# TrevorS/qwen3-tts-rs

Hardware: AMD Instinct MI355X
Metric: acoustic_frames_per_sec (higher is better)
Workload: dtype bf16

## Files before the change

include/q3tts.h:

```cpp
#ifndef Q3TTS_H
#define Q3TTS_H

#include <stddef.h>
#include <stdint.h>

#ifdef __cplusplus
extern "C" {
#endif

#define Q3_ABI_VERSION 1
#define Q3_MAX_BATCH 64

typedef enum q3_status {
    Q3_OK = 0,
    Q3_INVALID_ARG = 1,
    Q3_IO = 2,
    Q3_MISSING_WEIGHT = 3,
    Q3_KV_OVERFLOW = 4,
    Q3_HIP_ERROR = 5,
    Q3_RCCL_ERROR = 6,
    Q3_UNSUPPORTED = 7,
    Q3_OOM = 8
} q3_status;

// ... 209 lines not shown
int         q3_conv_path(int cout, int cin, int L, int k, int dil, int phases, int packed, int has_resid, int planes, int aligned16);
int         q3_resunit_path(int C, int L, int dil, int packed, int ya_is_xa, int planes);
const char* q3_conv_path_name(int code);
typedef struct q3_conv_ex_args {
    int kind, cin, cout, L, k, dil, stride;
    int act, planes, packed, resid_in_place, snake_raw, y2_is_x;
    int y_front, y_elems;
    int* path;
    const float* x; const float* w; const float* b;
    const float* snake_a; const float* snake_b; const float* resid; const float* scale;
    const float* post_a; const float* post_ib;
    const float* w2; const float* b2; const float* mid_a; const float* mid_ib;
    float* y; float* y2;
} q3_conv_ex_args;
q3_status q3_conv_ex(int device, const q3_conv_ex_args* args);
q3_status q3_test_conv_resident(int device, const q3_conv_ex_args* args, int resident, int* lds_bytes);
int q3_gemm_path(int M, int N, int K, int epi, int norm, int w2, int planes, int* path);
typedef struct q3_gemm_ex_args {
    int M, N, K, ldx, ldy, ldr, M_alloc;
    int epi, geometry, k_split, sup_m, sup_n;
    float eps;
    int* path;
    const float* x; const uint16_t* w; const uint16_t* w2;
    const float* bias; const float* norm_w; const float* resid;
    float* y;
} q3_gemm_ex_args;
q3_status q3_gemm_ex(int device, const q3_gemm_ex_args* args);
int q3_attn_prefill_path(int nh, int nkv, int use_planes, int halves, int* path);
typedef struct q3_attn_prefill_ex_args {
    int n_seq, rps, base_pos, nh, nkv, max_seq, ld_qkv, ld_out;
    int kernel, halves, use_planes;
    float eps;
    int* path;
    const float* qkv; const float* q_norm_w; const float* k_norm_w;
    const float* rope_cos; const float* rope_sin;
    float* kcache; float* vcache; float* out;
    int layout, n_layers, layer, n_slabs;
    const int* page_slots; int* rot_used; long long* stray;
} q3_attn_prefill_ex_args;
q3_status q3_attn_prefill_ex(int device, const q3_attn_prefill_ex_args* args);
typedef struct q3_attn_prefill_packed_ex_args {
    int n_seq, nh, nkv, max_seq, ld_qkv, ld_out;
    int kernel;
    float eps;
    const int* seq_len;
    int* path; long long* plane_tail;
    const float* qkv; const float* q_norm_w; const float* k_norm_w;
    const float* rope_cos; const float* rope_sin;
    float* kcache; float* vcache; float* out;
    int layout, n_layers, layer, n_slabs;
    const int* page_slots; int* rot_used; long long* stray;
} q3_attn_prefill_packed_ex_args;
q3_status q3_attn_prefill_packed_ex(int device, const q3_attn_prefill_packed_ex_args* args);
q3_status q3_prefill_pack_plan(const int32_t* lengths, const int32_t* hit_pages, int32_t n, int32_t row_budget, int32_t gemm_ok,
                               int32_t* pass, int32_t* row0, int32_t* n_passes);
q3_status q3_session_prefill_info(const q3_session* s, int32_t info[8]);
typedef struct q3_prompt_rows_ex_args {
    int mode, n, cols, n_table, n_rows, n_ref, cp_vocab, lds, ldd, reserved;
    const uint16_t* table; const uint32_t* ids; const float* src;
    const int* text_row; const int* codec_id; const float* xvec;
    const uint32_t* ref_codes; const uint16_t* cp_embs;
    const int* dst_row; const int* ent;
    float* out; int* trail_len; int* text_ready; int* limit;
} q3_prompt_rows_ex_args;
q3_status q3_prompt_rows_ex(int device, const q3_prompt_rows_ex_args* args);
int q3_attn_c_path(int hd, int kernel);
typedef struct q3_attn_c_ex_args {
    int mode, nh, hd, L, kernel, window;
    int N, n_rows, layers, layer, cap, n_blocks, n_tabs;
    float scale;
    const float* q; const float* k; const float* v;
    const int* rows; const float* caches;
    const int* tabs; const int* tab0; const int* tab_n;
    float* o;
} q3_attn_c_ex_args;
q3_status q3_attn_c_ex(int device, const q3_attn_c_ex_args* args);
q3_status q3_rope_c_ex(int device, float* q, float* k, const float* cs, const float* sn, const int* pos, int nh, int hd, int L, int n_pos);
q3_status q3_copy_cols_ex(int device, const float* src, size_t src_elems, float* dst, size_t dst_elems, int n, int C, const long long* s_off,
                          const long long* d_off, const int* sp, const int* dp, size_t src_off, size_t dst_off);
q3_status q3_copy_segs_ex(int device, const float* src, size_t src_elems, float* dst, size_t dst_elems, int n_segs, const unsigned long long* segs);
q3_status q3_gather_frames_ex(int device, const uint32_t* src, size_t src_elems, const long long* s_off, int n, uint32_t* dst, size_t dst_elems);
q3_status q3_rvq_embed_ex(int device, const uint32_t* frames, int n_frames, const float* first_cb, const float* rest_cbs, int cb_dim, int cb_size,
                          float* first_out, float* rest_out, int out_front, int out_elems);
q3_status q3_silu_mul_ex(int device, const float* g, const float* u, float* y, long long n, long long y_elems);
typedef struct q3_spk_op_ex_args {
    int op, C, T, pl, Tp, ld, off, reserved;
    long long a_elems, b_elems, out_front, out_elems;
    const float* a; const float* b; float* out;
} q3_spk_op_ex_args;
q3_status q3_spk_op_ex(int device, const q3_spk_op_ex_args* args);
typedef struct q3_mimi_op_ex_args {
    int op, C, L, r, Lf, elu, replicate, reserved;
    long long a_elems, b_elems, out_front, out_elems;
    const float* a; const float* b; float* out;
} q3_mimi_op_ex_args;
q3_status q3_mimi_op_ex(int device, const q3_mimi_op_ex_args* args);
q3_status q3_mimi_rvq_ex(int device, const float* proj, int T, const float* books, int n_layers, int CB, int CD, uint32_t* codes, int n_q,
                         int q0);
typedef struct q3_sample_rec {
    float inv_temp; int apply_temp, greedy;
    int top_k; float top_p; int use_top_p;
    float rep_pen, rep_inv; int use_rep;
    int eos_id, min_new_tokens, pad;
} q3_sample_rec;
q3_status q3_sample_row(const q3_options* opts, q3_sample_rec* out);
typedef struct q3_prompt_shape_rec {
    int32_t icl, n_ins, n_ref_text, n_icl, overlay;
    int32_t prefill_len, n_rows;
    int32_t trailing_len, n_trail;
    int32_t limit, open_need, prefix_pages;
    int32_t r_role, r_pad, r_bos, r_text, r_eos, trail_base;
} q3_prompt_shape_rec;
q3_status q3_prompt_shape(const q3_request* req, int n_text, q3_prompt_shape_rec* out, int* text_row, int* codec_id, int cap_positions);
typedef struct q3_sample_ex_args {
    int B, vocab, ld, u_stride, u_elems, advance, token_count_static, hist_stride_b, hist_cap, codec_eos, use_suppress, guard;
    q3_sample_rec scalar;
    const float* logits; const float* u; const int* draw_idx; const q3_sample_rec* rows;
    const int* limit; const int* text_ready;
    uint32_t* tok; uint8_t* seen; int* token_count; int* frame_idx; int* pos; float* logits_hist;
} q3_sample_ex_args;
q3_status q3_sample_ex(int device, const q3_sample_ex_args* args);
typedef struct q3_frame_embed_ex_args {
    int B, H, n_sem, cp_vocab, max_frames, n_text_rows, guard, reserved;
    const uint16_t* codec_emb; const uint16_t* cp_embs; const uint32_t* tok; const float* cp_logits_last;
    const int* frame_idx; const float* text_rows; const int* trail_base; const int* trail_len; const int* pad_row; const int* text_ready;
    uint32_t* codes; float* out;
} q3_frame_embed_ex_args;
q3_status q3_frame_embed_ex(int device, const q3_frame_embed_ex_args* args);
typedef struct q3_cp_gather_ex_args {
    int pass, B, H, n_sem, cp_vocab, max_frames, proj_dim, qkv_dim, ld_out, ld_qkv_out, guard, reserved;
    const float* last_hidden; const uint16_t* codec_emb; const uint32_t* tok; const uint16_t* cp_emb; const float* cp_logits;
    const float* proj_tab; const float* qkv_tab; const int* frame_idx;
    uint32_t* codes; float* out; float* qkv_out;
} q3_cp_gather_ex_args;
q3_status q3_cp_gather_ex(int device, const q3_cp_gather_ex_args* args);
q3_status q3_rmsnorm_ex(int device, const float* x, long long x_elems, long long x_off, int ldx, const float* w, float* y, long long y_elems,
                        long long y_front, int ldy, int rows, int cols, float eps, const int* frame_idx, const int* text_ready);
q3_status q3_norm_c(int device, int layernorm, const float* x, const float* w, const float* b, int C, int L, float eps,
                    float* y, int y_front, int y_elems);
q3_status q3_dwconv7(int device, const float* x, const float* w, const float* b, int C, int L, float* y, int y_front, int y_elems);
q3_status q3_row_move(int device, void* src_host, size_t src_bytes, void* dst_host, size_t dst_bytes, int n_segs, const size_t* src_off,
                      const size_t* dst_off, const size_t* seg_bytes, const int* mode);
enum { Q3_DEC_QUANT = 0, Q3_DEC_PRECONV = 1, Q3_DEC_PRETRANS = 2, Q3_DEC_UP0 = 3, Q3_DEC_UP1 = 4,
       Q3_DEC_INIT = 5, Q3_DEC_BLK0 = 6, Q3_DEC_BLK1 = 7, Q3_DEC_BLK2 = 8, Q3_DEC_BLK3 = 9, Q3_DEC_N = 10 };
q3_status q3_decode_codes(q3_model* m, const uint32_t* frames_host, int n_frames, float* pcm_host,
                          float** taps_host);
typedef struct q3_codec_stream q3_codec_stream;
q3_status q3_codec_stream_create(q3_model* m, int rows, int max_frames, q3_codec_stream** out);
void      q3_codec_stream_free(q3_codec_stream* cs);
q3_status q3_codec_stream_reset(q3_codec_stream* cs, int row);
q3_status q3_codec_stream_pos(q3_codec_stream* cs, int row, int* n_frames);
q3_status q3_codec_stream_push(q3_codec_stream* cs, int n_rows, const int* rows, const uint32_t* const* frames_host,
                               const int* n_frames, float* const* pcm_host, const size_t* cap);
q3_status q3_codec_stream_create_blocked(q3_model* m, int rows, int max_frames, int block_frames, int max_blocks, q3_codec_stream** out);
q3_status q3_codec_stream_info(q3_codec_stream* cs, int* block_frames, size_t* block_bytes, int* blocks_total, int* blocks_in_use,
                               int* blocks_peak);
q3_status q3_codec_stream_prime(q3_codec_stream* cs, int row, const uint32_t* frames_host, int n_frames);
enum { Q3_PCM_F32 = 0, Q3_PCM_S16 = 1, Q3_PCM_ULAW = 2, Q3_PCM_ALAW = 3 };
typedef struct q3_pcm_stage q3_pcm_stage;
q3_status q3_pcm_stage_create(int device, int rows, size_t max_push_samples, q3_pcm_stage** out);
void      q3_pcm_stage_free(q3_pcm_stage* ps);
q3_status q3_pcm_stage_set(q3_pcm_stage* ps, int row, uint32_t sample_rate, int format);
q3_status q3_pcm_stage_reset(q3_pcm_stage* ps, int row);
q3_status q3_pcm_stage_push(q3_pcm_stage* ps, int n_rows, const int* rows, const float* const* in_host, const size_t* n_in,
                            const int* last, void* const* out_host, const size_t* cap_samples, size_t* n_samples);
q3_status q3_pcm_stage_bound(uint32_t sample_rate, size_t n_in, size_t* n_out_max);
q3_status q3_pcm_stage_taps(uint32_t sample_rate, float* taps_host, size_t cap_floats, int* L, int* M);
q3_status q3_codec_stream_push_out(q3_codec_stream* cs, int n_rows, const int* rows, const uint32_t* const* frames_host, const int* n_frames,
                                   q3_pcm_stage* ps, const int* ps_rows, const int* last,
                                   void* const* out_host, const size_t* cap_samples, size_t* n_samples);
q3_status q3_session_set_output(q3_session* s, uint32_t sample_rate, int format);
q3_status q3_session_next_chunks_out(q3_session* s, void* const* out_host, const size_t* cap_samples, size_t* n_samples, int* done);
q3_status q3_batcher_ticket_output(q3_batcher* b, int64_t ticket, uint32_t sample_rate, int format);
q3_status q3_batcher_read_out(q3_batcher* b, int64_t ticket, void* out_host, size_t cap_samples, size_t* n_samples, int* done);
q3_status q3_pcm_stage_set_tempo(q3_pcm_stage* ps, int row, int tempo_permille);
q3_status q3_pcm_stage_tempo_count(int tempo_permille, size_t n_in_total, int ended, size_t* frames, size_t* samples_24k);
q3_status q3_pcm_stage_bound_tempo(uint32_t sample_rate, int tempo_permille, size_t n_in, size_t* n_out_max);
q3_status q3_pcm_stage_tempo_lags(q3_pcm_stage* ps, int row, int64_t* k0, int* lags, size_t cap, size_t* n);
q3_status q3_session_set_tempo(q3_session* s, int b, int tempo_permille);
q3_status q3_batcher_ticket_tempo(q3_batcher* b, int64_t ticket, int tempo_permille);
q3_status q3_pcm_stage_set_level(q3_pcm_stage* ps, int row, int gain_mB, int ceiling_mB);
q3_status q3_pcm_stage_level_coeffs(int gain_mB, int ceiling_mB, float* g, float* c);
q3_status q3_pcm_stage_level_count(size_t n_in_total, int ended, size_t* n_out);
q3_status q3_pcm_stage_bound_level(uint32_t sample_rate, int tempo_permille, size_t n_in, size_t* n_out_max);
q3_status q3_session_set_level(q3_session* s, int b, int gain_mB, int ceiling_mB);
q3_status q3_batcher_ticket_level(q3_batcher* b, int64_t ticket, int gain_mB, int ceiling_mB);
enum { Q3_LOUD_OFF = 0, Q3_LOUD_METER = 1, Q3_LOUD_NORMALIZE = 2 };
q3_status q3_loudness_kweight(uint32_t sample_rate, double* shelf_ba, double* highpass_ba);
q3_status q3_pcm_stage_loudness_consts(int target_mB, int prior_mB, float* T, float* P, float* gate_abs, float* a_lo, float* a_hi);
q3_status q3_pcm_stage_set_loudness(q3_pcm_stage* ps, int row, int mode, int target_mB, int prior_mB);
q3_status q3_pcm_stage_loudness(q3_pcm_stage* ps, int row, float* mean_square, float* gain, int* blocks, int* gated);
q3_status q3_pcm_stage_loudness_blocks(q3_pcm_stage* ps, int row, float* z, size_t cap, size_t* n);
q3_status q3_session_set_loudness(q3_session* s, int b, int mode, int target_mB, int prior_mB);
q3_status q3_session_loudness(q3_session* s, int b, float* mean_square, float* gain, int* blocks, int* gated);
q3_status q3_batcher_ticket_loudness(q3_batcher* b, int64_t ticket, int mode, int target_mB, int prior_mB);
q3_status q3_batcher_ticket_loudness_read(q3_batcher* b, int64_t ticket, float* mean_square, float* gain, int* blocks, int* gated);
q3_status q3_pcm_stage_set_pitch(q3_pcm_stage* ps, int row, int cents);
q3_status q3_pcm_stage_pitch_plan(int tempo_permille, int cents, int* tempo_eff, double* cents_realized);
q3_status q3_pcm_stage_pitch_tables(float* sinc, size_t cap1, float* win, size_t cap2, int* S1, int* S2);
q3_status q3_pcm_stage_pitch_count(int tempo_permille, int cents, size_t n_in_total, int ended, size_t* samples_24k);
q3_status q3_pcm_stage_bound_pitch(uint32_t sample_rate, int tempo_permille, int cents, int with_level, size_t n_in, size_t* n_out_max);
q3_status q3_session_set_pitch(q3_session* s, int b, int cents);
q3_status q3_batcher_ticket_pitch(q3_batcher* b, int64_t ticket, int cents);
q3_status q3_pcm_stage_set_silence(q3_pcm_stage* ps, int row, int threshold_mB, int edge_ms, int pause_ms);
q3_status q3_pcm_stage_silence(q3_pcm_stage* ps, int row, int64_t* n_in, int64_t* n_out, int64_t* lead_cut, int64_t* pause_cut, int64_t* trail_cut);
q3_status q3_pcm_stage_silence_hold(int edge_ms, int pause_ms, size_t* samples);
q3_status q3_pcm_stage_bound_silence(uint32_t sample_rate, int tempo_permille, int cents, int with_level, int edge_ms, int pause_ms, size_t n_in,
                                     size_t* n_out_max);
q3_status q3_silence_trim(const float* x, size_t n, int threshold_mB, int edge_ms, int pause_ms, float* y, size_t cap, size_t* n_y, int64_t* counts);
q3_status q3_session_set_silence(q3_session* s, int b, int threshold_mB, int edge_ms, int pause_ms);
q3_status q3_session_silence(q3_session* s, int b, int64_t* n_in, int64_t* n_out, int64_t* lead_cut, int64_t* pause_cut, int64_t* trail_cut);
q3_status q3_batcher_ticket_silence(q3_batcher* b, int64_t ticket, int threshold_mB, int edge_ms, int pause_ms);
q3_status q3_batcher_ticket_silence_read(q3_batcher* b, int64_t ticket, int64_t* n_in, int64_t* n_out, int64_t* lead_cut, int64_t* pause_cut, int64_t* trail_cut);
void      q3_codes_to_tensor(const uint32_t* frames, int n_frames, int64_t* out);

q3_status q3_session_set_profile(q3_session* s, int enable);
q3_status q3_session_profile_read(q3_session* s, double* ms, double* bytes, long* launches, int reset);
q3_status q3_session_profile_shapes(q3_session* s, int* rows, int cap_rows, int* n_rows, int reset);
q3_status q3_bench_linear(int device, int M, int N, int K, int epi, int rms, int tiled, int iters, int n_copies,
                          double* avg_us);
q3_status q3_session_stream(q3_session* s, void** stream);
q3_status q3_session_submit_info(q3_session* s, int* path, int* nodes);
q3_status q3_session_submit_fences(q3_session* s, int* acquire_free, int* release_free);
q3_status q3_session_frame_bytes(q3_session* s, int kv_len, double* weight_bytes, double* kv_bytes);

enum { Q3_MODEL_UNKNOWN = -1, Q3_MODEL_BASE = 0, Q3_MODEL_CUSTOM_VOICE = 1, Q3_MODEL_VOICE_DESIGN = 2 };
q3_status q3_config_default(int variant, q3_config* out);
q3_status q3_config_from_json(const char* path, q3_config* out, int* model_type);
q3_status q3_model_load(const char* model_dir, int device, q3_model** out, int* model_type);
q3_status q3_model_load_safetensors(q3_model* m, const char* path, int* n_loaded);
q3_status q3_safetensors_info(const char* path, const char* name, int* dtype, int64_t* shape, int cap_dims, int* n_dims);
q3_status q3_pcm16_from_f32(const float* samples_host, int64_t n, int16_t* out_host);
q3_status q3_wav_write_pcm16(const char* path, const float* samples_host, int64_t n, uint32_t sample_rate);
q3_status q3_g711_from_pcm16(const int16_t* in_host, int64_t n, int law, uint8_t* out_host);
q3_status q3_wav_write_g711(const char* path, const uint8_t* bytes_host, int64_t n, uint32_t sample_rate, int law);
q3_status q3_wav_read(const char* path, float* out_host, int64_t cap, int64_t* n_samples, uint32_t* sample_rate);
q3_status q3_codes_write_bin(const char* path, const uint32_t* codes_host, int n_frames, int n_groups);
q3_status q3_codes_read_bin(const char* path, uint32_t* codes_host, int cap_frames, int n_groups, int* n_frames);
q3_status q3_audio_write_bin(const char* path, const float* samples_host, int64_t n);
q3_status q3_audio_read_bin(const char* path, float* out_host, int64_t cap, int64_t* n_samples);
q3_status q3_resample(const float* in_host, int64_t n, uint32_t sr_in, uint32_t sr_out, float* out_host, int64_t cap, int64_t* n_out);

typedef struct q3_spk_config {
    int32_t mel_dim;
    int32_t enc_dim;
    int32_t channels[5];
    int32_t kernel_sizes[5];
    int32_t dilations[5];
    int32_t attention_channels;
    int32_t res2net_scale;
    int32_t se_channels;
    int32_t sample_rate;
} q3_spk_config;
typedef struct q3_speaker_encoder q3_speaker_encoder;
q3_status q3_spk_config_default(q3_spk_config* out);
q3_status q3_spk_config_from_json(const char* path, q3_spk_config* out, int* present);
q3_status q3_spk_create(const q3_spk_config* cfg, int device, q3_speaker_encoder** out);
void q3_spk_free(q3_speaker_encoder* e);
q3_status q3_spk_get_config(const q3_speaker_encoder* e, q3_spk_config* out);
int q3_spk_n_tensors(const q3_speaker_encoder* e);
q3_status q3_spk_tensor_info(const q3_speaker_encoder* e, int i, const char** name, int64_t* n);
q3_status q3_spk_set_tensor(q3_speaker_encoder* e, const char* name, const void* data_host, int src_dtype, int64_t n);
q3_status q3_spk_finalize(q3_speaker_encoder* e);
q3_status q3_spk_load_safetensors(q3_speaker_encoder* e, const char* path);
int q3_spk_mel_frames(int64_t n_samples);
q3_status q3_spk_mel(q3_speaker_encoder* e, const float* samples_host, int64_t n, float* mel_host, int64_t cap_floats, int* n_frames);
q3_status q3_spk_tables(q3_speaker_encoder* e, float* win_host, float* fb_host);
q3_status q3_spk_forward(q3_speaker_encoder* e, const float* mel_host, int T, float* out_host, float** taps_host);
q3_status q3_spk_encode(q3_speaker_encoder* e, const float* samples_host, int64_t n, uint32_t sample_rate, float* out_host);

typedef struct q3_mimi_config {
    int32_t n_filters;
    int32_t hidden;
    int32_t ratios[4];
    int32_t kernel;
    int32_t res_kernel;
    int32_t last_kernel;
    int32_t compress;
    int32_t n_layers;
    int32_t n_heads;
    int32_t head_dim;
    int32_t inter;
    int32_t window;
    int32_t cb_size;
    int32_t cb_dim;
    int32_t n_q;
    int32_t n_sem;
    float norm_eps;
    float rope_theta;
} q3_mimi_config;
typedef struct q3_speech_encoder q3_speech_encoder;
q3_status q3_mimi_config_default(q3_mimi_config* out);
q3_status q3_mimi_create(const q3_mimi_config* cfg, int device, q3_speech_encoder** out);
void q3_mimi_free(q3_speech_encoder* e);
q3_status q3_mimi_get_config(const q3_speech_encoder* e, q3_mimi_config* out);
int q3_mimi_n_tensors(const q3_speech_encoder* e);
q3_status q3_mimi_tensor_info(const q3_speech_encoder* e, int i, const char** name, int64_t* n);
q3_status q3_mimi_set_tensor(q3_speech_encoder* e, const char* name, const void* data_host, int src_dtype, int64_t n);
q3_status q3_mimi_finalize(q3_speech_encoder* e);
q3_status q3_mimi_load_safetensors(q3_speech_encoder* e, const char* path);
int q3_mimi_frames(const q3_mimi_config* cfg, int64_t n_samples);
q3_status q3_mimi_encode(q3_speech_encoder* e, const float* samples_host, int64_t n, uint32_t sample_rate, uint32_t* codes_host,
                         int cap_frames, int* n_frames, float** taps_host);

enum { Q3_SRC_U8 = 0, Q3_SRC_S16 = 1, Q3_SRC_S24 = 2, Q3_SRC_S32 = 3, Q3_SRC_F32 = 4, Q3_SRC_ULAW = 5, Q3_SRC_ALAW = 6 };
typedef struct q3_clip { const void* data; int64_t frames; int32_t channels; uint32_t sample_rate; int32_t format; } q3_clip;
// ... 37 lines not shown
```

qwen3_tts_rs_amd/_lib.py:

```python
import ctypes
import os

from .config import CConfig

_HERE = os.path.dirname(os.path.abspath(__file__))
LIB_PATH = os.environ.get("Q3TTS_LIB") or os.path.join(_HERE, "libq3tts.so")

if not os.path.exists(LIB_PATH):
    raise ImportError(
        f"{LIB_PATH} not found: the gfx950 HIP library is not built. Run "
        "`python -c 'import __graft_entry__ as g; g.build()'` (or qwen3_tts_rs_amd/csrc/build.sh).")

lib = ctypes.CDLL(LIB_PATH)


class COptions(ctypes.Structure):
    _fields_ = [
        ("temperature", ctypes.c_double), ("top_p", ctypes.c_double), ("repetition_penalty", ctypes.c_double),
        ("seed", ctypes.c_uint64), ("max_length", ctypes.c_int32), ("top_k", ctypes.c_int32),
        ("eos_token_id", ctypes.c_int32), ("chunk_frames", ctypes.c_int32), ("min_new_tokens", ctypes.c_int32),
        ("has_seed", ctypes.c_int32),
    ]


# ... 43 lines not shown
               [("eps", ctypes.c_float), ("qkv_eps", ctypes.c_float), ("reserved", ctypes.c_int32)] + \
               [(n, ctypes.c_void_p) for n in ("pos", "qkv", "q_norm_w", "k_norm_w", "rope_cos", "rope_sin", "kcache", "vcache", "out", "page_slots",
                                               "rot_used", "stray", "qkv_part", "qkv_ssq", "g_logits", "g_tok", "g_qkv_tab", "g_proj_tab", "g_x",
                                               "g_codes", "g_frame_idx", "zero_buf")]


class CConvEx(ctypes.Structure):
    _fields_ = [(n, ctypes.c_int32) for n in ("kind", "cin", "cout", "L", "k", "dil", "stride", "act", "planes", "packed", "resid_in_place",
                                              "snake_raw", "y2_is_x", "y_front", "y_elems")] + [("path", ctypes.POINTER(ctypes.c_int32))] + \
               [(n, ctypes.c_void_p) for n in ("x", "w", "b", "snake_a", "snake_b", "resid", "scale", "post_a", "post_ib", "w2", "b2", "mid_a",
                                               "mid_ib", "y", "y2")]


class CGemmEx(ctypes.Structure):
    _fields_ = [(n, ctypes.c_int32) for n in ("M", "N", "K", "ldx", "ldy", "ldr", "M_alloc", "epi", "geometry", "k_split", "sup_m",
                                              "sup_n")] + [("eps", ctypes.c_float), ("path", ctypes.POINTER(ctypes.c_int32))] + \
               [(n, ctypes.c_void_p) for n in ("x", "w", "w2", "bias", "norm_w", "resid", "y")]


class CAttnPrefillEx(ctypes.Structure):
    _fields_ = [(n, ctypes.c_int32) for n in ("n_seq", "rps", "base_pos", "nh", "nkv", "max_seq", "ld_qkv", "ld_out", "kernel", "halves",
                                              "use_planes")] + [("eps", ctypes.c_float), ("path", ctypes.POINTER(ctypes.c_int32))] + \
               [(n, ctypes.c_void_p) for n in ("qkv", "q_norm_w", "k_norm_w", "rope_cos", "rope_sin", "kcache", "vcache", "out")] + \
               [(n, ctypes.c_int32) for n in ("layout", "n_layers", "layer", "n_slabs")] + \
               [(n, ctypes.c_void_p) for n in ("page_slots", "rot_used", "stray")]


class CAttnPrefillPackedEx(ctypes.Structure):
    _fields_ = [(n, ctypes.c_int32) for n in ("n_seq", "nh", "nkv", "max_seq", "ld_qkv", "ld_out", "kernel")] + [("eps", ctypes.c_float)] + \
               [(n, ctypes.c_void_p) for n in ("seq_len", "path", "plane_tail", "qkv", "q_norm_w", "k_norm_w", "rope_cos", "rope_sin", "kcache", "vcache",
                                               "out")] + \
               [(n, ctypes.c_int32) for n in ("layout", "n_layers", "layer", "n_slabs")] + \
               [(n, ctypes.c_void_p) for n in ("page_slots", "rot_used", "stray")]


class CPromptRowsEx(ctypes.Structure):
    _fields_ = [(n, ctypes.c_int32) for n in ("mode", "n", "cols", "n_table", "n_rows", "n_ref", "cp_vocab", "lds", "ldd", "reserved")] + \
               [(n, ctypes.c_void_p) for n in ("table", "ids", "src", "text_row", "codec_id", "xvec", "ref_codes", "cp_embs", "dst_row", "ent", "out",
                                               "trail_len", "text_ready", "limit")]


class CAttnCEx(ctypes.Structure):
    _fields_ = [(n, ctypes.c_int32) for n in ("mode", "nh", "hd", "L", "kernel", "window", "N", "n_rows", "layers", "layer", "cap", "n_blocks",
                                              "n_tabs")] + [("scale", ctypes.c_float)] + \
               [(n, ctypes.c_void_p) for n in ("q", "k", "v", "rows", "caches", "tabs", "tab0", "tab_n", "o")]


class CSpkOpEx(ctypes.Structure):
    _fields_ = [(n, ctypes.c_int32) for n in ("op", "C", "T", "pl", "Tp", "ld", "off", "reserved")] + \
               [(n, ctypes.c_longlong) for n in ("a_elems", "b_elems", "out_front", "out_elems")] + \
               [(n, ctypes.c_void_p) for n in ("a", "b", "out")]


class CMimiOpEx(ctypes.Structure):
    _fields_ = [(n, ctypes.c_int32) for n in ("op", "C", "L", "r", "Lf", "elu", "replicate", "reserved")] + \
               [(n, ctypes.c_longlong) for n in ("a_elems", "b_elems", "out_front", "out_elems")] + \
               [(n, ctypes.c_void_p) for n in ("a", "b", "out")]


class CSampleRow(ctypes.Structure):
    _fields_ = [("inv_temp", ctypes.c_float), ("apply_temp", ctypes.c_int32), ("greedy", ctypes.c_int32), ("top_k", ctypes.c_int32),
                ("top_p", ctypes.c_float), ("use_top_p", ctypes.c_int32), ("rep_pen", ctypes.c_float), ("rep_inv", ctypes.c_float),
                ("use_rep", ctypes.c_int32), ("eos_id", ctypes.c_int32), ("min_new_tokens", ctypes.c_int32), ("pad", ctypes.c_int32)]


class CPromptShape(ctypes.Structure):
    _fields_ = [(n, ctypes.c_int32) for n in ("icl", "n_ins", "n_ref_text", "n_icl", "overlay", "prefill_len", "n_rows", "trailing_len", "n_trail",
                                              "limit", "open_need", "prefix_pages", "r_role", "r_pad", "r_bos", "r_text", "r_eos", "trail_base")]


class CSampleEx(ctypes.Structure):
    _fields_ = [(n, ctypes.c_int32) for n in ("B", "vocab", "ld", "u_stride", "u_elems", "advance", "token_count_static", "hist_stride_b",
                                              "hist_cap", "codec_eos", "use_suppress", "guard")] + [("scalar", CSampleRow)] + \
               [(n, ctypes.c_void_p) for n in ("logits", "u", "draw_idx", "rows", "limit", "text_ready", "tok", "seen", "token_count",
                                               "frame_idx", "pos", "logits_hist")]


class CFrameEmbedEx(ctypes.Structure):
    _fields_ = [(n, ctypes.c_int32) for n in ("B", "H", "n_sem", "cp_vocab", "max_frames", "n_text_rows", "guard", "reserved")] + \
               [(n, ctypes.c_void_p) for n in ("codec_emb", "cp_embs", "tok", "cp_logits_last", "frame_idx", "text_rows", "trail_base",
                                               "trail_len", "pad_row", "text_ready", "codes", "out")]


class CCpGatherEx(ctypes.Structure):
    _fields_ = [(n, ctypes.c_int32) for n in ("pass_", "B", "H", "n_sem", "cp_vocab", "max_frames", "proj_dim", "qkv_dim", "ld_out",
                                              "ld_qkv_out", "guard", "reserved")] + \
               [(n, ctypes.c_void_p) for n in ("last_hidden", "codec_emb", "tok", "cp_emb", "cp_logits", "proj_tab", "qkv_tab", "frame_idx",
                                               "codes", "out", "qkv_out")]


class CClip(ctypes.Structure):
    _fields_ = [("data", ctypes.c_void_p), ("frames", ctypes.c_int64), ("channels", ctypes.c_int32), ("sample_rate", ctypes.c_uint32),
                ("format", ctypes.c_int32)]


class CMimiPackClip(ctypes.Structure):
    _fields_ = [("frames", ctypes.c_int32), ("pass_", ctypes.c_int32), ("start", ctypes.c_int64)]


class CWavDesc(ctypes.Structure):
    _fields_ = [("format", ctypes.c_int32), ("channels", ctypes.c_int32), ("bits", ctypes.c_int32), ("sample_rate", ctypes.c_uint32),
                ("frames", ctypes.c_int64), ("data_offset", ctypes.c_int64), ("data_bytes", ctypes.c_int64)]


class CTiming(ctypes.Structure):
    _fields_ = [("prefill_ms", ctypes.c_double), ("generation_ms", ctypes.c_double), ("decode_ms", ctypes.c_double),
                ("generation_frames", ctypes.c_int32)]


c_void_p, c_int, c_char_p = ctypes.c_void_p, ctypes.c_int, ctypes.c_char_p
P = ctypes.POINTER

SYMBOLS = {
    "q3_abi_version": (c_int, []),
    "q3_last_error": (c_char_p, []),
    "q3_device_count": (c_int, []),
    "q3_model_create": (c_int, [P(CConfig), c_int, P(c_void_p)]),
    "q3_model_free": (None, [c_void_p]),
    "q3_model_set_tensor": (c_int, [c_void_p, c_char_p, c_int, c_void_p, ctypes.c_int64]),
    "q3_model_n_tensors": (c_int, [c_void_p]),
    "q3_model_tensor_info": (c_int, [c_void_p, c_int, P(c_char_p), P(ctypes.c_int64), P(c_int)]),
    "q3_model_arena": (c_int, [c_void_p, P(c_void_p), P(ctypes.c_size_t)]),
    "q3_model_kv_pool_limit": (c_int, [c_void_p, c_int]),
    "q3_model_set_codec_planes": (c_int, [c_void_p, c_int]),
    "q3_model_kv_pool_trim": (c_int, [c_void_p, P(ctypes.c_size_t)]),
    "q3_model_kv_pool_info": (c_int, [c_void_p, P(c_int), P(ctypes.c_size_t), P(c_int), P(c_int), P(c_int)]),
    "q3_model_prefix_cache": (c_int, [c_void_p, c_int]),
    "q3_model_prefix_cache_info": (c_int, [c_void_p, P(c_int), P(c_int), P(c_int), P(ctypes.c_longlong), P(ctypes.c_longlong), P(ctypes.c_longlong)]),
    "q3_session_prefix_info": (c_int, [c_void_p, c_int, P(c_int)]),
    "q3_model_mark_loaded": (c_int, [c_void_p]),
    "q3_model_finalize": (c_int, [c_void_p]),
    "q3_synth_fill": (c_int, [ctypes.c_uint64, c_char_p, c_int, ctypes.c_float, ctypes.c_float, ctypes.c_int64, c_void_p]),
    "q3_session_create": (c_int, [c_void_p, P(CRequest), c_int, P(c_void_p)]),
    "q3_session_create_reserved": (c_int, [c_void_p, P(CRequest), c_int, c_int, c_int, P(c_void_p)]),
    "q3_session_free": (None, [c_void_p]),
    "q3_session_prefill": (c_int, [c_void_p]),
    "q3_session_generate": (c_int, [c_void_p, c_int, c_int]),
    "q3_session_frames": (c_int, [c_void_p, c_int, P(c_int), P(c_int)]),
    "q3_session_codes": (c_int, [c_void_p, c_int, c_void_p, c_int, P(c_int)]),
    "q3_session_decode": (c_int, [c_void_p, c_int, c_int, c_int, c_void_p, ctypes.c_size_t, P(ctypes.c_size_t)]),
    "q3_session_set_kv_dtype": (c_int, [c_void_p, c_int]),
    "q3_session_run": (c_int, [c_void_p, c_int, P(c_void_p), P(ctypes.c_size_t), P(ctypes.c_size_t), P(CTiming)]),
    "q3_session_next_chunk": (c_int, [c_void_p, c_void_p, ctypes.c_size_t, P(ctypes.c_size_t), P(c_int)]),
    "q3_session_next_chunk_row": (c_int, [c_void_p, c_int, c_void_p, ctypes.c_size_t, P(ctypes.c_size_t), P(c_int)]),
    "q3_session_next_chunks": (c_int, [c_void_p, P(c_void_p), P(ctypes.c_size_t), P(ctypes.c_size_t), P(c_int)]),
    "q3_codec_stream_create": (c_int, [c_void_p, c_int, c_int, P(c_void_p)]),
    "q3_codec_stream_create_blocked": (c_int, [c_void_p, c_int, c_int, c_int, c_int, P(c_void_p)]),
    "q3_codec_stream_info": (c_int, [c_void_p, P(c_int), P(ctypes.c_size_t), P(c_int), P(c_int), P(c_int)]),
    "q3_codec_stream_prime": (c_int, [c_void_p, c_int, c_void_p, c_int]),
    "q3_codec_stream_free": (None, [c_void_p]),
    "q3_codec_stream_reset": (c_int, [c_void_p, c_int]),
    "q3_codec_stream_pos": (c_int, [c_void_p, c_int, P(c_int)]),
    "q3_codec_stream_push": (c_int, [c_void_p, c_int, P(c_int), P(c_void_p), P(c_int), P(c_void_p), P(ctypes.c_size_t)]),
    "q3_pcm_stage_create": (c_int, [c_int, c_int, ctypes.c_size_t, P(c_void_p)]),
    "q3_pcm_stage_free": (None, [c_void_p]),
    "q3_pcm_stage_set": (c_int, [c_void_p, c_int, ctypes.c_uint32, c_int]),
    "q3_pcm_stage_reset": (c_int, [c_void_p, c_int]),
    "q3_pcm_stage_push": (c_int, [c_void_p, c_int, P(c_int), P(c_void_p), P(ctypes.c_size_t), P(c_int), P(c_void_p), P(ctypes.c_size_t),
                                  P(ctypes.c_size_t)]),
    "q3_pcm_stage_bound": (c_int, [ctypes.c_uint32, ctypes.c_size_t, P(ctypes.c_size_t)]),
    "q3_pcm_stage_taps": (c_int, [ctypes.c_uint32, c_void_p, ctypes.c_size_t, P(c_int), P(c_int)]),
    "q3_pcm_stage_set_tempo": (c_int, [c_void_p, c_int, c_int]),
    "q3_pcm_stage_tempo_count": (c_int, [c_int, ctypes.c_size_t, c_int, P(ctypes.c_size_t), P(ctypes.c_size_t)]),
    "q3_pcm_stage_bound_tempo": (c_int, [ctypes.c_uint32, c_int, ctypes.c_size_t, P(ctypes.c_size_t)]),
    "q3_pcm_stage_tempo_lags": (c_int, [c_void_p, c_int, P(ctypes.c_int64), c_void_p, ctypes.c_size_t, P(ctypes.c_size_t)]),
    "q3_session_set_tempo": (c_int, [c_void_p, c_int, c_int]),
    "q3_batcher_ticket_tempo": (c_int, [c_void_p, ctypes.c_int64, c_int]),
    "q3_pcm_stage_set_pitch": (c_int, [c_void_p, c_int, c_int]),
    "q3_pcm_stage_pitch_plan": (c_int, [c_int, c_int, P(c_int), P(ctypes.c_double)]),
    "q3_pcm_stage_pitch_tables": (c_int, [c_void_p, ctypes.c_size_t, c_void_p, ctypes.c_size_t, P(c_int), P(c_int)]),
    "q3_pcm_stage_pitch_count": (c_int, [c_int, c_int, ctypes.c_size_t, c_int, P(ctypes.c_size_t)]),
    "q3_pcm_stage_bound_pitch": (c_int, [ctypes.c_uint32, c_int, c_int, c_int, ctypes.c_size_t, P(ctypes.c_size_t)]),
    "q3_session_set_pitch": (c_int, [c_void_p, c_int, c_int]),
    "q3_batcher_ticket_pitch": (c_int, [c_void_p, ctypes.c_int64, c_int]),
    "q3_pcm_stage_set_silence": (c_int, [c_void_p, c_int, c_int, c_int, c_int]),
    "q3_pcm_stage_silence": (c_int, [c_void_p, c_int] + [P(ctypes.c_int64)] * 5),
    "q3_pcm_stage_silence_hold": (c_int, [c_int, c_int, P(ctypes.c_size_t)]),
    "q3_pcm_stage_bound_silence": (c_int, [ctypes.c_uint32, c_int, c_int, c_int, c_int, c_int, ctypes.c_size_t, P(ctypes.c_size_t)]),
    "q3_silence_trim": (c_int, [c_void_p, ctypes.c_size_t, c_int, c_int, c_int, c_void_p, ctypes.c_size_t, P(ctypes.c_size_t), P(ctypes.c_int64)]),
    "q3_session_set_silence": (c_int, [c_void_p, c_int, c_int, c_int, c_int]),
    "q3_session_silence": (c_int, [c_void_p, c_int] + [P(ctypes.c_int64)] * 5),
    "q3_batcher_ticket_silence": (c_int, [c_void_p, ctypes.c_int64, c_int, c_int, c_int]),
    "q3_batcher_ticket_silence_read": (c_int, [c_void_p, ctypes.c_int64] + [P(ctypes.c_int64)] * 5),
    "q3_pcm_stage_set_level": (c_int, [c_void_p, c_int, c_int, c_int]),
    "q3_pcm_stage_level_coeffs": (c_int, [c_int, c_int, P(ctypes.c_float), P(ctypes.c_float)]),
    "q3_pcm_stage_level_count": (c_int, [ctypes.c_size_t, c_int, P(ctypes.c_size_t)]),
    "q3_pcm_stage_bound_level": (c_int, [ctypes.c_uint32, c_int, ctypes.c_size_t, P(ctypes.c_size_t)]),
    "q3_session_set_level": (c_int, [c_void_p, c_int, c_int, c_int]),
    "q3_batcher_ticket_level": (c_int, [c_void_p, ctypes.c_int64, c_int, c_int]),
    "q3_loudness_kweight": (c_int, [ctypes.c_uint32, P(ctypes.c_double), P(ctypes.c_double)]),
    "q3_pcm_stage_loudness_consts": (c_int, [c_int, c_int, P(ctypes.c_float), P(ctypes.c_float), P(ctypes.c_float), P(ctypes.c_float), P(ctypes.c_float)]),
    "q3_pcm_stage_set_loudness": (c_int, [c_void_p, c_int, c_int, c_int, c_int]),
    "q3_pcm_stage_loudness": (c_int, [c_void_p, c_int, P(ctypes.c_float), P(ctypes.c_float), P(c_int), P(c_int)]),
    "q3_pcm_stage_loudness_blocks": (c_int, [c_void_p, c_int, c_void_p, ctypes.c_size_t, P(ctypes.c_size_t)]),
    "q3_session_set_loudness": (c_int, [c_void_p, c_int, c_int, c_int, c_int]),
    "q3_session_loudness": (c_int, [c_void_p, c_int, P(ctypes.c_float), P(ctypes.c_float), P(c_int), P(c_int)]),
    "q3_batcher_ticket_loudness": (c_int, [c_void_p, ctypes.c_int64, c_int, c_int, c_int]),
    "q3_batcher_ticket_loudness_read": (c_int, [c_void_p, ctypes.c_int64, P(ctypes.c_float), P(ctypes.c_float), P(c_int), P(c_int)]),
    "q3_codec_stream_push_out": (c_int, [c_void_p, c_int, P(c_int), P(c_void_p), P(c_int), c_void_p, P(c_int), P(c_int), P(c_void_p),
                                         P(ctypes.c_size_t), P(ctypes.c_size_t)]),
    "q3_session_set_output": (c_int, [c_void_p, ctypes.c_uint32, c_int]),
    "q3_session_next_chunks_out": (c_int, [c_void_p, P(c_void_p), P(ctypes.c_size_t), P(ctypes.c_size_t), P(c_int)]),
    "q3_batcher_ticket_output": (c_int, [c_void_p, ctypes.c_int64, ctypes.c_uint32, c_int]),
    "q3_batcher_read_out": (c_int, [c_void_p, ctypes.c_int64, c_void_p, ctypes.c_size_t, P(ctypes.c_size_t), P(c_int)]),
    "q3_session_replace": (c_int, [c_void_p, c_int, c_void_p]),
    "q3_session_park_row": (c_int, [c_void_p, c_int, P(c_void_p)]),
    "q3_session_resume_row": (c_int, [c_void_p, c_int, c_void_p]),
    "q3_parked_free": (None, [c_void_p]),
    "q3_parked_info": (c_int, [c_void_p, P(c_int), P(c_int), P(c_int), P(c_int), P(ctypes.c_size_t)]),
    "q3_row_move": (c_int, [c_int, c_void_p, ctypes.c_size_t, c_void_p, ctypes.c_size_t, c_int, P(ctypes.c_size_t), P(ctypes.c_size_t),
                            P(ctypes.c_size_t), P(c_int)]),
    "q3_batcher_create": (c_int, [c_void_p, c_int, c_int, c_int, P(c_void_p)]),
    "q3_batcher_free": (None, [c_void_p]),
    "q3_batcher_submit": (c_int, [c_void_p, c_void_p, c_int, P(ctypes.c_int64)]),
    "q3_batcher_submit_streamed": (c_int, [c_void_p, c_void_p, P(ctypes.c_int64)]),
    "q3_batcher_read": (c_int, [c_void_p, ctypes.c_int64, c_void_p, ctypes.c_size_t, P(ctypes.c_size_t), P(c_int)]),
    "q3_batcher_stream_info": (c_int, [c_void_p, P(c_int), P(ctypes.c_size_t), P(c_int), P(c_int), P(c_int)]),
    "q3_batcher_submit_open": (c_int, [c_void_p, c_void_p, c_int, P(ctypes.c_int64)]),
    "q3_batcher_append_text": (c_int, [c_void_p, ctypes.c_int64, c_void_p, c_int, c_int]),
    "q3_batcher_text_state": (c_int, [c_void_p, ctypes.c_int64, P(c_int), P(c_int), P(c_int), P(c_int)]),
    "q3_batcher_cancel": (c_int, [c_void_p, ctypes.c_int64]),
    "q3_batcher_set_parking": (c_int, [c_void_p, c_int, c_int, c_int]),
    "q3_batcher_park": (c_int, [c_void_p, ctypes.c_int64]),
    "q3_batcher_unpark": (c_int, [c_void_p, ctypes.c_int64]),
    "q3_batcher_park_info": (c_int, [c_void_p, P(c_int), P(c_int), P(ctypes.c_longlong), P(ctypes.c_longlong), P(ctypes.c_longlong), P(c_int)]),
    "q3_batcher_step": (c_int, [c_void_p, c_int, c_int, P(c_int), P(c_int), P(c_int)]),
    "q3_batcher_poll": (c_int, [c_void_p, ctypes.c_int64, P(c_int), P(c_int), P(ctypes.c_size_t)]),
    "q3_batcher_fetch": (c_int, [c_void_p, ctypes.c_int64, c_void_p, c_int, c_void_p, ctypes.c_size_t]),
    "q3_session_set_debug": (c_int, [c_void_p, c_int]),
    "q3_session_prefill_len": (c_int, [c_void_p, c_int, P(c_int), P(c_int)]),
    "q3_session_get": (c_int, [c_void_p, c_int, c_int, c_void_p, ctypes.c_size_t]),
    "q3_talker_step": (c_int, [c_void_p, c_void_p, c_void_p, c_void_p]),
    "q3_cp_generate": (c_int, [c_void_p, c_void_p, c_void_p, c_void_p, c_void_p]),
    "q3_frame_embed": (c_int, [c_void_p, ctypes.c_uint32, c_void_p, c_void_p, c_void_p]),
    "q3_sample": (c_int, [c_int, c_void_p, c_void_p, c_void_p, c_int, c_int, P(COptions), c_int, c_void_p]),
    "q3_rng_seed": (None, [ctypes.c_uint64, P(ctypes.c_uint64)]),
    "q3_rng_next": (ctypes.c_float, [P(ctypes.c_uint64)]),
    "q3_fused_residual_rmsnorm": (c_int, [c_int, c_int, c_void_p, c_void_p, c_void_p, c_int, c_int, ctypes.c_float, c_void_p, c_void_p]),
    "q3_linear": (c_int, [c_int, c_void_p, c_void_p, c_void_p, c_int, c_int, c_int, c_void_p]),
    "q3_linear_ex": (c_int, [c_int, P(CLinearEx)]),
    "q3_attn_step": (c_int, [c_int, P(CAttnStep)]),
    "q3_attn_step_ex": (c_int, [c_int, P(CAttnStepEx)]),
    "q3_kv_pages_to_bf16_ex": (c_int, [c_int] * 4 + [c_void_p] * 6),
    "q3_conv_path": (c_int, [c_int] * 10),
    "q3_resunit_path": (c_int, [c_int] * 6),
    "q3_conv_path_name": (c_char_p, [c_int]),
    "q3_conv_ex": (c_int, [c_int, P(CConvEx)]),
    "q3_test_conv_resident": (c_int, [c_int, P(CConvEx), c_int, P(ctypes.c_int32)]),
    "q3_gemm_path": (c_int, [c_int] * 7 + [P(ctypes.c_int32)]),
    "q3_gemm_ex": (c_int, [c_int, P(CGemmEx)]),
    "q3_attn_prefill_path": (c_int, [c_int] * 4 + [P(ctypes.c_int32)]),
    "q3_attn_prefill_ex": (c_int, [c_int, P(CAttnPrefillEx)]),
    "q3_attn_prefill_packed_ex": (c_int, [c_int, P(CAttnPrefillPackedEx)]),
    "q3_prefill_pack_plan": (c_int, [P(ctypes.c_int32), P(ctypes.c_int32), ctypes.c_int32, ctypes.c_int32, ctypes.c_int32, P(ctypes.c_int32),
                                     P(ctypes.c_int32), P(ctypes.c_int32)]),
    "q3_session_prefill_info": (c_int, [c_void_p, P(ctypes.c_int32)]),
    "q3_prompt_rows_ex": (c_int, [c_int, P(CPromptRowsEx)]),
    "q3_attn_c_path": (c_int, [c_int, c_int]),
    "q3_attn_c_ex": (c_int, [c_int, P(CAttnCEx)]),
    "q3_rope_c_ex": (c_int, [c_int, c_void_p, c_void_p, c_void_p, c_void_p, c_void_p, c_int, c_int, c_int, c_int]),
    "q3_copy_cols_ex": (c_int, [c_int, c_void_p, ctypes.c_size_t, c_void_p, ctypes.c_size_t, c_int, c_int, c_void_p, c_void_p, c_void_p, c_void_p,
                                ctypes.c_size_t, ctypes.c_size_t]),
    "q3_copy_segs_ex": (c_int, [c_int, c_void_p, ctypes.c_size_t, c_void_p, ctypes.c_size_t, c_int, c_void_p]),
    "q3_gather_frames_ex": (c_int, [c_int, c_void_p, ctypes.c_size_t, c_void_p, c_int, c_void_p, ctypes.c_size_t]),
    "q3_rvq_embed_ex": (c_int, [c_int, c_void_p, c_int, c_void_p, c_void_p, c_int, c_int, c_void_p, c_void_p, c_int, c_int]),
    "q3_silu_mul_ex": (c_int, [c_int, c_void_p, c_void_p, c_void_p, ctypes.c_longlong, ctypes.c_longlong]),
    "q3_spk_op_ex": (c_int, [c_int, P(CSpkOpEx)]),
    "q3_mimi_op_ex": (c_int, [c_int, P(CMimiOpEx)]),
    "q3_mimi_rvq_ex": (c_int, [c_int, c_void_p, c_int, c_void_p, c_int, c_int, c_int, c_void_p, c_int, c_int]),
    "q3_spk_tables": (c_int, [c_void_p, c_void_p, c_void_p]),
    "q3_sample_row": (c_int, [P(COptions), P(CSampleRow)]),
    "q3_prompt_shape": (c_int, [P(CRequest), c_int, P(CPromptShape), c_void_p, c_void_p, c_int]),
    "q3_sample_ex": (c_int, [c_int, P(CSampleEx)]),
    "q3_frame_embed_ex": (c_int, [c_int, P(CFrameEmbedEx)]),
    "q3_cp_gather_ex": (c_int, [c_int, P(CCpGatherEx)]),
    "q3_rmsnorm_ex": (c_int, [c_int, c_void_p, ctypes.c_longlong, ctypes.c_longlong, c_int, c_void_p, c_void_p, ctypes.c_longlong,
                              ctypes.c_longlong, c_int, c_int, c_int, ctypes.c_float, c_void_p, c_void_p]),
    "q3_norm_c": (c_int, [c_int, c_int, c_void_p, c_void_p, c_void_p, c_int, c_int, ctypes.c_float, c_void_p, c_int, c_int]),
    "q3_dwconv7": (c_int, [c_int, c_void_p, c_void_p, c_void_p, c_int, c_int, c_void_p, c_int, c_int]),
    "q3_decode_codes": (c_int, [c_void_p, c_void_p, c_int, c_void_p, P(c_void_p)]),
    "q3_codes_to_tensor": (None, [c_void_p, c_int, c_void_p]),
    "q3_session_set_profile": (c_int, [c_void_p, c_int]),
    "q3_session_profile_read": (c_int, [c_void_p, P(ctypes.c_double), P(ctypes.c_double), P(ctypes.c_long), c_int]),
    "q3_session_profile_shapes": (c_int, [c_void_p, P(c_int), c_int, P(c_int), c_int]),
    "q3_bench_linear": (c_int, [c_int] * 9 + [P(ctypes.c_double)]),
    "q3_session_stream": (c_int, [c_void_p, P(c_void_p)]),
    "q3_session_frame_bytes": (c_int, [c_void_p, c_int, P(ctypes.c_double), P(ctypes.c_double)]),
    "q3_session_submit_info": (c_int, [c_void_p, P(c_int), P(c_int)]),
    "q3_session_submit_fences": (c_int, [c_void_p, P(c_int), P(c_int)]),
    "q3_session_set_stream_mode": (c_int, [c_void_p, c_int]),
    "q3_session_open_text": (c_int, [c_void_p, c_int]),
    "q3_session_append_text": (c_int, [c_void_p, c_int, c_void_p, c_int, c_int]),
    "q3_session_text_state": (c_int, [c_void_p, c_int, P(c_int), P(c_int), P(c_int), P(c_int), P(c_int)]),
    "q3_model_config": (c_int, [c_void_p, P(CConfig)]),
    "q3_config_default": (c_int, [c_int, P(CConfig)]),
    "q3_config_from_json": (c_int, [c_char_p, P(CConfig), P(c_int)]),
    "q3_model_load": (c_int, [c_char_p, c_int, P(c_void_p), P(c_int)]),
    "q3_model_load_safetensors": (c_int, [c_void_p, c_char_p, P(c_int)]),
    "q3_safetensors_info": (c_int, [c_char_p, c_char_p, P(c_int), P(ctypes.c_int64), c_int, P(c_int)]),
    "q3_pcm16_from_f32": (c_int, [c_void_p, ctypes.c_int64, c_void_p]),
    "q3_wav_write_pcm16": (c_int, [c_char_p, c_void_p, ctypes.c_int64, ctypes.c_uint32]),
    "q3_g711_from_pcm16": (c_int, [c_void_p, ctypes.c_int64, c_int, c_void_p]),
    "q3_wav_write_g711": (c_int, [c_char_p, c_void_p, ctypes.c_int64, ctypes.c_uint32, c_int]),
    "q3_wav_read": (c_int, [c_char_p, c_void_p, ctypes.c_int64, P(ctypes.c_int64), P(ctypes.c_uint32)]),
    "q3_codes_write_bin": (c_int, [c_char_p, c_void_p, c_int, c_int]),
    "q3_codes_read_bin": (c_int, [c_char_p, c_void_p, c_int, c_int, P(c_int)]),
# ... 67 lines not shown
```

qwen3_tts_rs_amd/api.py:

```python
import ctypes
import enum
from dataclasses import dataclass
from typing import List, NamedTuple, Optional, Sequence, Tuple

import numpy as np

from . import _lib
from ._lib import lib, check, COptions, CRequest, CTiming
from .config import Q3Config
from . import synth

MAX_BATCH = 64
CODEC_EOS_TOKEN_ID = 2150
SAMPLES_PER_FRAME = 1920


class Language(enum.Enum):
    Chinese = 2055
    English = 2050
    Japanese = 2058
    Korean = 2064
    German = 2053
    French = 2061
    Russian = 2069
# ... 992 lines not shown
        s = Session(self, utts[:n0], o, frame_budget=budget, prompt_budget=prompt)
        owner = list(range(n0)); nxt = n0
        codes: List[Optional[np.ndarray]] = [None] * len(utts); pcm: List[Optional[np.ndarray]] = [None] * len(utts)
        frames = 0
        t0 = _time.perf_counter()
        try:
            s.prefill()
            while any(i is not None for i in owner):
                s.generate(poll_frames, use_graph=use_graph)
                for b in range(n0):
                    i = owner[b]
                    if i is None:
                        continue
                    n, done = s.frames(b)
                    if not done:
                        continue
                    codes[i] = s.codes(b); frames += int(codes[i].shape[0])
                    if decode:
                        pcm[i] = s.decode(b)
                    if nxt < len(utts):
                        s.replace(b, utts[nxt]); owner[b] = nxt; nxt += 1
                    else:
                        owner[b] = None
            wall = _time.perf_counter() - t0
        finally:
            s.close()
        return codes, pcm, frames, wall

    def synthesize_continuous_streaming(self, utts: Sequence[Utterance], options=None, slots: int = 8, poll_frames: int = 10,
                                        on_audio=None, use_graph: bool = True):
        o = options or SynthesisOptions()
        utts = list(utts)
        budget = max((u.max_length if u.max_length is not None else (u.options or o).max_length) for u in utts)
        prompt = max((0 if u.instruct_ids is None else len(u.instruct_ids)) + (0 if u.ref_codes is None else int(np.asarray(u.ref_codes).reshape(-1, 16).shape[0])) + 16 for u in utts)
        bt = Batcher(self, slots=min(slots, max(len(utts), 1)), frame_budget=budget, prompt_budget=prompt, options=o)
        try:
            tickets = [bt.submit_streamed(u) for u in utts]
            open_ = set(range(len(utts)))

            def drain():
                for i in sorted(open_):
                    samples, done = bt.read(tickets[i])
                    if samples.size or done:
                        if on_audio is not None:
                            on_audio(i, samples, done)
                    if done:
                        open_.discard(i)
            while True:
                running, queued, _ = bt.step(poll_frames, use_graph)
                drain()
                if running == 0 and queued == 0:
                    break
            drain()
            return [bt.fetch(t)[0] for t in tickets]
        finally:
            bt.close()

    def synthesize_streaming(self, text_ids, speaker: Speaker, language: Language, options=None,
                             continuous: bool = False) -> StreamingSession:
        return StreamingSession(self, Utterance(text_ids, speaker, language), options or SynthesisOptions(), continuous)

    def synthesize_voice_design_streaming(self, text_ids, instruct_ids, language: Language, options=None,
                                          continuous: bool = False) -> StreamingSession:
        return StreamingSession(self, Utterance(text_ids, language=language, instruct_ids=instruct_ids), options or SynthesisOptions(), continuous)

    def synthesize_streaming_text(self, first_ids, speaker: Speaker, language: Language, options=None,
                                  continuous: bool = False) -> "TextStreamingSession":
        return TextStreamingSession(self, Utterance(list(first_ids), speaker, language), options or SynthesisOptions(), continuous)

    def synthesize_voice_clone_debug(self, text_ids, prompt, language: Language, options=None):
        return self.synthesize_voice_clone(text_ids, prompt.speaker_embedding, language, options,
                                           ref_codes=prompt.ref_codes, ref_text_ids=prompt.ref_text_ids)

    def device(self) -> str:
        return f"hip:{self.device_index}"

    @classmethod
    def from_pretrained_with_tokenizer(cls, model_dir: str, tokenizer_dir: Optional[str], device: int = 0):
        from .text import TextTokenizer
        return cls.from_pretrained(model_dir, device), TextTokenizer.from_pretrained(model_dir, tokenizer_dir)

    def decode_codes(self, codes: np.ndarray, taps=None) -> AudioBuffer:
        c = np.ascontiguousarray(codes, dtype=np.uint32).reshape(-1, 16)
        out = np.zeros(c.shape[0] * self.config.samples_per_frame, dtype=np.float32)
        tp = None
        if taps is not None:
            tp = (ctypes.c_void_p * 10)(*[t.ctypes.data_as(ctypes.c_void_p) if t is not None else None for t in taps])
        check(lib.q3_decode_codes(self._h, c.ctypes.data_as(ctypes.c_void_p), c.shape[0], out.ctypes.data_as(ctypes.c_void_p), tp))
        return AudioBuffer(out)

    def codec_stream(self, rows: int, max_frames: int, block_frames: int = 0, max_blocks: int = 0) -> "CodecStream":
        return CodecStream(self, rows, max_frames, block_frames, max_blocks)

    def pcm_stage(self, rows: int, max_push_samples: int) -> "PcmStage":
        return PcmStage(self, rows, max_push_samples)

    def frame_embed(self, sem_token: int, codes15, text_add: np.ndarray) -> np.ndarray:
        c = np.ascontiguousarray(codes15, dtype=np.uint32); t = np.ascontiguousarray(text_add, dtype=np.float32)
        out = np.zeros(self.config.hidden, dtype=np.float32)
        check(lib.q3_frame_embed(self._h, int(sem_token), c.ctypes.data_as(ctypes.c_void_p), t.ctypes.data_as(ctypes.c_void_p),
                                 out.ctypes.data_as(ctypes.c_void_p)))
        return out


class CodecStream:
    def __init__(self, model: "Qwen3TTS", rows: int, max_frames: int, block_frames: int = 0, max_blocks: int = 0):
        self.model = model; self.rows = int(rows); self.max_frames = int(max_frames)
        self._h = ctypes.c_void_p()
        if block_frames or max_blocks:
            check(lib.q3_codec_stream_create_blocked(model._h, self.rows, self.max_frames, int(block_frames), int(max_blocks),
                                                     ctypes.byref(self._h)))
        else:
            check(lib.q3_codec_stream_create(model._h, self.rows, self.max_frames, ctypes.byref(self._h)))

    def prime(self, row: int, codes: np.ndarray):
        c = np.ascontiguousarray(codes, dtype=np.uint32).reshape(-1, 16)
        check(lib.q3_codec_stream_prime(self._h, int(row), c.ctypes.data_as(ctypes.c_void_p), c.shape[0]))

    def info(self) -> dict:
        bf = ctypes.c_int(); bb = ctypes.c_size_t(); tot = ctypes.c_int(); use = ctypes.c_int(); peak = ctypes.c_int()
        check(lib.q3_codec_stream_info(self._h, ctypes.byref(bf), ctypes.byref(bb), ctypes.byref(tot), ctypes.byref(use), ctypes.byref(peak)))
        return {"block_frames": bf.value, "block_bytes": bb.value, "blocks_total": tot.value, "blocks_in_use": use.value,
                "blocks_peak": peak.value}

    def push(self, frames: dict, stage: Optional["PcmStage"] = None, stage_rows: Optional[dict] = None, last=()) -> dict:
        if stage is None:
            return self._push_lists(list(frames.keys()), list(frames.values()))
        rows = list(frames.keys()); n = len(rows); spf = self.model.config.samples_per_frame
        cs = [np.ascontiguousarray(frames[r], dtype=np.uint32).reshape(-1, 16) for r in rows]
        srows = [int((stage_rows or {}).get(r, r)) for r in rows]
        outs = [np.zeros(stage.bound(sr, c.shape[0] * spf), dtype=stage.dtype(sr)) for sr, c in zip(srows, cs)]
        r_ = (ctypes.c_int * n)(*[int(x) for x in rows])
        fp = (ctypes.c_void_p * n)(*[c.ctypes.data_as(ctypes.c_void_p) for c in cs])
        nf = (ctypes.c_int * n)(*[c.shape[0] for c in cs])
        sr_ = (ctypes.c_int * n)(*srows)
        ls = (ctypes.c_int * n)(*[1 if r in last else 0 for r in rows])
        op = (ctypes.c_void_p * n)(*[o.ctypes.data_as(ctypes.c_void_p) for o in outs])
        cp = (ctypes.c_size_t * n)(*[o.size for o in outs])
        ns = (ctypes.c_size_t * n)()
        check(lib.q3_codec_stream_push_out(self._h, n, r_, fp, nf, stage._h, sr_, ls, op, cp, ns))
        return {int(rows[i]): outs[i][:ns[i]].copy() for i in range(n)}

    def _push_lists(self, rows: Sequence[int], codes: Sequence[np.ndarray], cap: Optional[Sequence[int]] = None) -> dict:
        n = len(rows); spf = self.model.config.samples_per_frame
        cs = [np.ascontiguousarray(c, dtype=np.uint32).reshape(-1, 16) for c in codes]
        outs = [np.zeros(c.shape[0] * spf, dtype=np.float32) for c in cs]
        r = (ctypes.c_int * n)(*[int(x) for x in rows])
        fp = (ctypes.c_void_p * n)(*[c.ctypes.data_as(ctypes.c_void_p) for c in cs])
        nf = (ctypes.c_int * n)(*[c.shape[0] for c in cs])
        op = (ctypes.c_void_p * n)(*[o.ctypes.data_as(ctypes.c_void_p) for o in outs])
        cp = (ctypes.c_size_t * n)(*[int(x) for x in (cap if cap is not None else [o.size for o in outs])])
        check(lib.q3_codec_stream_push(self._h, n, r, fp, nf, op, cp))
        return {int(rows[i]): outs[i] for i in range(n)}

    def reset(self, row: int):
        check(lib.q3_codec_stream_reset(self._h, int(row)))

    def pos(self, row: int) -> int:
        n = ctypes.c_int()
        check(lib.q3_codec_stream_pos(self._h, int(row), ctypes.byref(n)))
        return n.value

    def close(self):
        if getattr(self, "_h", None):
            lib.q3_codec_stream_free(self._h); self._h = None

    __del__ = close


PCM_F32, PCM_S16, PCM_ULAW, PCM_ALAW = 0, 1, 2, 3
PCM_NAMES = ("f32", "s16", "ulaw", "alaw")
PCM_DTYPE = (np.float32, np.int16, np.uint8, np.uint8)


def pcm_format(pcm16: bool = False, fmt: Optional[str] = None) -> int:
    if fmt is None:
        return PCM_S16 if pcm16 else PCM_F32
    if pcm16:
        raise ValueError("give pcm16= or fmt=, not both")
    if fmt not in PCM_NAMES:
        raise ValueError(f"fmt must be one of {list(PCM_NAMES)}, not {fmt!r}")
    return PCM_NAMES.index(fmt)


def pcm_stage_taps(rate: int) -> Tuple[np.ndarray, int, int]:
    L = ctypes.c_int(); M = ctypes.c_int()
    check(lib.q3_pcm_stage_taps(int(rate), None, 0, ctypes.byref(L), ctypes.byref(M)))
    t = np.zeros((L.value, 128), np.float32)
    check(lib.q3_pcm_stage_taps(int(rate), t.ctypes.data_as(ctypes.c_void_p), t.size, ctypes.byref(L), ctypes.byref(M)))
    return t, L.value, M.value


def pcm_stage_bound(rate: int, n_in: int, tempo_permille: int = 1000, level: bool = False, pitch_cents: int = 0, silence=None) -> int:
    n = ctypes.c_size_t()
    if silence is not None:
        check(lib.q3_pcm_stage_bound_silence(int(rate), int(tempo_permille), int(pitch_cents), 1 if level else 0, int(silence[0]), int(silence[1]),
                                             int(n_in), ctypes.byref(n)))
    elif int(pitch_cents):
        check(lib.q3_pcm_stage_bound_pitch(int(rate), int(tempo_permille), int(pitch_cents), 1 if level else 0, int(n_in), ctypes.byref(n)))
    elif level:
        check(lib.q3_pcm_stage_bound_level(int(rate), int(tempo_permille), int(n_in), ctypes.byref(n)))
    elif int(tempo_permille) == 1000:
        check(lib.q3_pcm_stage_bound(int(rate), int(n_in), ctypes.byref(n)))
    else:
        check(lib.q3_pcm_stage_bound_tempo(int(rate), int(tempo_permille), int(n_in), ctypes.byref(n)))
    return int(n.value)


def pcm_stage_tempo_count(tempo_permille: int, n_in_total: int, ended: bool = False) -> Tuple[int, int]:
    f = ctypes.c_size_t(); y = ctypes.c_size_t()
    check(lib.q3_pcm_stage_tempo_count(int(tempo_permille), int(n_in_total), 1 if ended else 0, ctypes.byref(f), ctypes.byref(y)))
    return int(f.value), int(y.value)


def pcm_stage_pitch_plan(tempo_permille: int, cents: int) -> Tuple[int, float]:
    te = ctypes.c_int(); c = ctypes.c_double()
    check(lib.q3_pcm_stage_pitch_plan(int(tempo_permille), int(cents), ctypes.byref(te), ctypes.byref(c)))
    return int(te.value), float(c.value)


def pcm_stage_pitch_tables() -> Tuple[np.ndarray, np.ndarray, int, int]:
    s1 = ctypes.c_int(); s2 = ctypes.c_int()
    check(lib.q3_pcm_stage_pitch_tables(None, 0, None, 0, ctypes.byref(s1), ctypes.byref(s2)))
    sc = np.zeros(61 * s1.value + 2, np.float32); w2 = np.zeros(64 * s2.value + 2, np.float32)
    check(lib.q3_pcm_stage_pitch_tables(sc.ctypes.data_as(ctypes.c_void_p), sc.size, w2.ctypes.data_as(ctypes.c_void_p), w2.size,
                                        ctypes.byref(s1), ctypes.byref(s2)))
    return sc, w2, s1.value, s2.value


def pcm_stage_pitch_count(tempo_permille: int, cents: int, n_in_total: int, ended: bool = False) -> int:
    n = ctypes.c_size_t()
    check(lib.q3_pcm_stage_pitch_count(int(tempo_permille), int(cents), int(n_in_total), 1 if ended else 0, ctypes.byref(n)))
    return int(n.value)


def pcm_stage_level_coeffs(gain_mb: int, ceiling_mb: int) -> Tuple[np.float32, np.float32]:
    g = ctypes.c_float(); c = ctypes.c_float()
    check(lib.q3_pcm_stage_level_coeffs(int(gain_mb), int(ceiling_mb), ctypes.byref(g), ctypes.byref(c)))
    return np.float32(g.value), np.float32(c.value)


def pcm_stage_level_count(n_in_total: int, ended: bool = False) -> int:
    n = ctypes.c_size_t()
    check(lib.q3_pcm_stage_level_count(int(n_in_total), 1 if ended else 0, ctypes.byref(n)))
    return int(n.value)


LOUD_OFF, LOUD_METER, LOUD_NORMALIZE = 0, 1, 2


class Loudness(NamedTuple):
    lufs: float
    mean_square: float
    gain: float
    gain_db: float
    blocks: int
    gated: int

    @classmethod
    def of(cls, m, g, blocks, gated):
        m = float(np.float32(m)); g = float(np.float32(g))
        return cls(-0.691 + 10.0 * float(np.log10(m)) if m > 0.0 else float("-inf"), m, g, 20.0 * float(np.log10(g)) if g > 0.0 else float("-inf"),
                   int(blocks), int(gated))


def loudness_kweight(rate: int) -> Tuple[np.ndarray, np.ndarray]:
    sh = np.zeros(6, np.float64); hp = np.zeros(6, np.float64)
    check(lib.q3_loudness_kweight(int(rate), sh.ctypes.data_as(ctypes.POINTER(ctypes.c_double)), hp.ctypes.data_as(ctypes.POINTER(ctypes.c_double))))
    return sh, hp


def pcm_stage_loudness_consts(target_mb: int = -1900, prior_mb: int = 0) -> Tuple[np.float32, ...]:
    v = [ctypes.c_float() for _ in range(5)]
    check(lib.q3_pcm_stage_loudness_consts(int(target_mb), int(prior_mb), *[ctypes.byref(x) for x in v]))
    return tuple(np.float32(x.value) for x in v)


class Silence(NamedTuple):
    n_in: int
    n_out: int
    lead_cut: int
    pause_cut: int
    trail_cut: int


def silence_mb(threshold_db) -> int:
    return 0 if threshold_db is None else int(round(float(threshold_db) * 100.0))


def pcm_stage_silence_hold(edge_ms: int, pause_ms: int) -> int:
    n = ctypes.c_size_t()
    check(lib.q3_pcm_stage_silence_hold(int(edge_ms), int(pause_ms), ctypes.byref(n)))
    return int(n.value)


def trim_silence(samples, threshold_db: float, edge_ms: int = 50, pause_ms: int = 400, counts: bool = False):
    x = np.ascontiguousarray(samples.samples if isinstance(samples, AudioBuffer) else samples, dtype=np.float32).reshape(-1)
    if isinstance(samples, AudioBuffer) and samples.sample_rate != 24000:
        raise ValueError(f"trim_silence takes 24 kHz audio, not {samples.sample_rate} Hz")
    y = np.zeros(max(x.size, 1), np.float32)
    n = ctypes.c_size_t(); c = (ctypes.c_int64 * 5)()
    check(lib.q3_silence_trim(x.ctypes.data_as(ctypes.c_void_p), x.size, silence_mb(threshold_db), int(edge_ms), int(pause_ms),
                              y.ctypes.data_as(ctypes.c_void_p), y.size, ctypes.byref(n), c))
    y = y[:int(n.value)].copy()
    out = AudioBuffer(y, 24000) if isinstance(samples, AudioBuffer) else y
    return (out, Silence(*[int(v) for v in c])) if counts else out
# ... 1070 lines not shown
```

qwen3_tts_rs_amd/csrc/q3_codec_stream.hip:

```cpp
#include "q3_engine.h"

struct CsRow { int pos = 0; float* kv = nullptr; float* lat = nullptr; float* hist = nullptr; std::vector<float*> blocks; };
struct q3_codec_stream {
    q3_model* m = nullptr; int R = 0, cap = 0;
    int bf = 0, max_blocks = 0;
    std::vector<float*> free_blocks; int blocks_total = 0, blocks_in_use = 0, blocks_peak = 0;
    hipStream_t st = nullptr; bool owns_stream = false;
    std::vector<CsRow> rows;
    CodecWS ws;
    float *cs = nullptr, *sn = nullptr;
    char* desc = nullptr; size_t desc_cap = 0;
    float* stage = nullptr; float* stage_host = nullptr; size_t stage_cap = 0;
};

static size_t kv_floats(const q3_codec_stream* cs) {
    const q3_config& c = cs->m->cfg;
    return (size_t)c.dec_layers * 2 * c.dec_heads * c.dec_head_dim * cs->cap;
}

static size_t block_floats(const q3_codec_stream* cs) {
    const q3_config& c = cs->m->cfg;
    return ((size_t)c.dec_layers * 2 * c.dec_heads * c.dec_head_dim + c.dec_latent) * cs->bf;
}

q3_status codec_stream_create(q3_model* m, int rows, int max_frames, hipStream_t st, q3_codec_stream** out, int block_frames, int max_blocks) {
    if (!m || !m->finalized) return set_err(Q3_INVALID_ARG, "model not finalized");
    if (!out || rows < 1 || max_frames < 1) return set_err(Q3_INVALID_ARG, "q3_codec_stream_create: rows and max_frames must be positive");
    if (m->device < 0) return set_err(Q3_INVALID_ARG, "q3_codec_stream_create: the model has no device (manifest-only): the vocoder runs on the GPU");
    if (m->cfg.dec_head_dim != 64) return set_err(Q3_INVALID_ARG, "q3_codec_stream_create: decoder head dim must be 64");
    HIPC(hipSetDevice(m->device));
    std::unique_ptr<q3_codec_stream> cs(new q3_codec_stream());
    cs->m = m; cs->R = rows; cs->cap = max_frames; cs->rows.resize(rows);
    cs->bf = block_frames; cs->max_blocks = max_blocks;
    m->refs.fetch_add(1);
    auto fail = [&](q3_status s) { q3_codec_stream_free(cs.release()); return s; };
    if (st) cs->st = st;
    else {
        q3_relax_capture_mode();
        const hipError_t e = hipStreamCreateWithFlags(&cs->st, hipStreamNonBlocking);
        if (e != hipSuccess) { cs->st = nullptr; return fail(set_err(Q3_HIP_ERROR, "hipStreamCreateWithFlags: %s", hipGetErrorString(e))); }
        cs->owns_stream = true;
    }
    if (dev_malloc((void**)&cs->cs, (size_t)max_frames * 32 * 4) != hipSuccess || dev_malloc((void**)&cs->sn, (size_t)max_frames * 32 * 4) != hipSuccess)
        return fail(set_err(Q3_OOM, "q3_codec_stream_create: RoPE table of %d frames", max_frames));
    const q3_status s = codec_rope_table(m->cfg, max_frames, cs->cs, cs->sn);
    if (s != Q3_OK) return fail(s);
    *out = cs.release();
    return Q3_OK;
}

extern "C" q3_status q3_codec_stream_create(q3_model* m, int rows, int max_frames, q3_codec_stream** out) {
    return codec_stream_create(m, rows, max_frames, nullptr, out);
}

extern "C" q3_status q3_codec_stream_create_blocked(q3_model* m, int rows, int max_frames, int block_frames, int max_blocks, q3_codec_stream** out) {
    if (block_frames < 32 || block_frames % 32 != 0)
        return set_err(Q3_INVALID_ARG, "q3_codec_stream_create_blocked: block_frames %d is not a positive multiple of 32 (a 32-key attention tile must lie inside one block)", block_frames);
    if (max_blocks < 0) return set_err(Q3_INVALID_ARG, "q3_codec_stream_create_blocked: negative max_blocks");
    return codec_stream_create(m, rows, max_frames, nullptr, out, block_frames, max_blocks);
}
extern "C" q3_status q3_codec_stream_info(q3_codec_stream* cs, int* block_frames, size_t* block_bytes, int* blocks_total, int* blocks_in_use, int* blocks_peak) {
    if (!cs) return set_err(Q3_INVALID_ARG, "q3_codec_stream_info: null stream");
    if (block_frames) *block_frames = cs->bf;
    if (block_bytes) *block_bytes = block_floats(cs) * 4;
    if (blocks_total) *blocks_total = cs->blocks_total;
    if (blocks_in_use) *blocks_in_use = cs->blocks_in_use;
    if (blocks_peak) *blocks_peak = cs->blocks_peak;
    return Q3_OK;
}

extern "C" void q3_codec_stream_free(q3_codec_stream* cs) {
    if (!cs) return;
    q3_model* m = cs->m;
    (void)hipSetDevice(m->device);
    if (cs->st) (void)hipStreamSynchronize(cs->st);
    for (CsRow& r : cs->rows) { dev_free(r.kv); dev_free(r.lat); dev_free(r.hist); for (float* b : r.blocks) dev_free(b); }
    for (float* b : cs->free_blocks) dev_free(b);
    cs->ws.release();
    dev_free(cs->cs); dev_free(cs->sn); dev_free(cs->desc); dev_free(cs->stage);
    if (cs->stage_host) (void)hipHostFree(cs->stage_host);
    if (cs->owns_stream && cs->st) (void)hipStreamDestroy(cs->st);
    delete cs;
    if (m->refs.fetch_sub(1) == 1) model_destroy(m);
}

int codec_stream_pos(const q3_codec_stream* cs, int row) { return cs->rows[row].pos; }
void codec_stream_blocks(const q3_codec_stream* cs, int row, int upto, int* held, int* need) {
    const CsRow& r = cs->rows[row];
    *held = (int)r.blocks.size();
    *need = cs->bf ? std::max(0, (upto + cs->bf - 1) / cs->bf - *held) : 0;
}
void codec_stream_reset(q3_codec_stream* cs, int row) {
    CsRow& r = cs->rows[row];
    r.pos = 0;
    cs->blocks_in_use -= (int)r.blocks.size();
    cs->free_blocks.insert(cs->free_blocks.end(), r.blocks.begin(), r.blocks.end());
    r.blocks.clear();
}

extern "C" q3_status q3_codec_stream_reset(q3_codec_stream* cs, int row) {
    if (!cs || row < 0 || row >= cs->R) return set_err(Q3_INVALID_ARG, "q3_codec_stream_reset: bad row");
    codec_stream_reset(cs, row);
    return Q3_OK;
}
extern "C" q3_status q3_codec_stream_pos(q3_codec_stream* cs, int row, int* n_frames) {
    if (!cs || row < 0 || row >= cs->R || !n_frames) return set_err(Q3_INVALID_ARG, "q3_codec_stream_pos: bad row");
    *n_frames = cs->rows[row].pos;
    return Q3_OK;
}

namespace {
struct DescBlock {
    std::vector<char> host;
    template <typename T> size_t add(const std::vector<T>& v) {
        const size_t off = (host.size() + 15) & ~(size_t)15;
        host.resize(off + v.size() * sizeof(T));
        if (!v.empty()) memcpy(host.data() + off, v.data(), v.size() * sizeof(T));
        return off;
    }
};
}

q3_status codec_stream_push(q3_codec_stream* cs, const std::vector<CsPush>& all) {
    q3_model* m = cs->m;
    const q3_config& c = m->cfg;
    std::vector<CsPush> P;
    for (const CsPush& p : all) if (p.n > 0) P.push_back(p);
    q3_pcm_stage* ps = nullptr;
    std::vector<const CsPush*> flush;
    for (const CsPush& p : all) {
        if (p.ps) ps = p.ps;
        if (p.n_out) *p.n_out = 0;
        if (p.n <= 0 && p.ps && p.last) flush.push_back(&p);
    }
    if (P.empty()) {
        if (flush.empty()) return Q3_OK;
        std::vector<PsSeg> segs; std::vector<void*> outs; std::vector<size_t> cnt(flush.size(), 0);
        for (const CsPush* f : flush) { segs.push_back({f->ps_row, nullptr, 0, 1}); outs.push_back(f->out_host); }
        Q3C(pcm_stage_push_dev(ps, segs, cs->st, outs.data(), cnt.data()));
        for (size_t k = 0; k < flush.size(); ++k) if (flush[k]->n_out) *flush[k]->n_out = cnt[k];
        return Q3_OK;
    }
    HIPC(hipSetDevice(m->device));
    hipStream_t st = cs->st;
    const int Q = c.dec_q_dim, LAT = c.dec_latent, QD = c.dec_heads * c.dec_head_dim, cap = cs->cap, spf = samples_per_frame(c);
    const int nP = (int)P.size();
    const bool on_dev = P[0].dev != nullptr;
    const int bf = cs->bf, kp = bf ? bf : cap;
    const size_t lat_off = (size_t)c.dec_layers * 2 * QD * bf;
    struct Untake {
        q3_codec_stream* cs; const std::vector<CsPush>& P; bool armed = true;
        ~Untake() {
            if (!armed || !cs->bf) return;
            for (const CsPush& p : P) {
                CsRow& r = cs->rows[p.row];
                while ((int)r.blocks.size() > (r.pos + cs->bf - 1) / cs->bf) { cs->free_blocks.push_back(r.blocks.back()); r.blocks.pop_back(); cs->blocks_in_use--; }
            }
        }
    } untake{cs, P};
    if (bf) {
        int need = 0;
        for (const CsPush& p : P) {
            const CsRow& r = cs->rows[p.row];
            need += std::max(0, (r.pos + p.n + bf - 1) / bf - (int)r.blocks.size());
        }
        if (cs->max_blocks > 0 && cs->blocks_in_use + need > cs->max_blocks)
            return set_err(Q3_OOM, "codec stream: block pool exhausted: the push needs %d more block(s) of %d frames, %d of %d are in use",
                           need, bf, cs->blocks_in_use, cs->max_blocks);
        while ((int)cs->free_blocks.size() < need) {
            float* b = nullptr;
            if (dev_malloc((void**)&b, block_floats(cs) * 4) != hipSuccess) {
                (void)hipGetLastError();
                return set_err(Q3_OOM, "codec stream: block %d (%zu KB each)", cs->blocks_total, block_floats(cs) * 4 >> 10);
            }
            cs->free_blocks.push_back(b); cs->blocks_total++;
        }
        for (const CsPush& p : P) {
            CsRow& r = cs->rows[p.row];
            if (!r.hist && dev_malloc((void**)&r.hist, (size_t)Q * 2 * 4) != hipSuccess) {
                (void)hipGetLastError(); r.hist = nullptr;
                return set_err(Q3_OOM, "codec stream: history columns of row %d", p.row);
            }
        }
        for (const CsPush& p : P) {
            CsRow& r = cs->rows[p.row];
            while ((int)r.blocks.size() * bf < r.pos + p.n) { r.blocks.push_back(cs->free_blocks.back()); cs->free_blocks.pop_back(); cs->blocks_in_use++; }
        }
    }
    for (const CsPush& p : P) {
        CsRow& r = cs->rows[p.row];
        if (bf || r.kv) continue;
        if (dev_malloc((void**)&r.kv, kv_floats(cs) * 4) != hipSuccess || dev_malloc((void**)&r.lat, (size_t)LAT * cap * 4) != hipSuccess ||
            dev_malloc((void**)&r.hist, (size_t)Q * 2 * 4) != hipSuccess) {
            (void)hipGetLastError();
            dev_free(r.kv); dev_free(r.lat); dev_free(r.hist); r.kv = r.lat = r.hist = nullptr;
            return set_err(Q3_OOM, "codec stream: state of row %d (%zu MB)", p.row, (kv_floats(cs) + (size_t)LAT * cap) * 4 >> 20);
        }
    }
    int N = 0, W = 0, Lc = 0, solo_max = 0, max_tiles = 0;
    std::vector<int> col0(nP), out0(nP), conc, solo;
    for (int i = 0; i < nP; ++i) {
        const int f0 = cs->rows[P[i].row].pos, a0 = f0 + P[i].skip, e = f0 + P[i].n;
        col0[i] = N; N += P[i].n;
        out0[i] = W; W += e - a0;
        if (e > a0) {
            if (a0 > CODEC_CTX_FRAMES) { conc.push_back(i); Lc += e - a0 + CODEC_CTX_FRAMES; }
            else { solo.push_back(i); solo_max = std::max(solo_max, e); }
        }
        max_tiles = std::max(max_tiles, ((e - 1) >> 5) - (f0 >> 5) + 1);
    }
    const int Np = N + 2 * nP;
    {
        const int CS_WIDE = 2048;
        int max_n = 0; for (const CsPush& p : P) max_n = std::max(max_n, p.n);
        const int T = std::max(1, std::max(Lc, solo_max));
        const long long Tw = (long long)cs->R * (max_n + CODEC_CTX_FRAMES), Fw = (long long)cs->R * (max_n + 2);
        Q3C(codec_reserve(m, cs->ws, (int)std::max<long long>(T, std::min<long long>(Tw, CS_WIDE)),
                          (int)std::max<long long>(Np, std::min<long long>(Fw, CS_WIDE))));
    }
    CodecWS& ws = cs->ws;
    if ((size_t)W * spf > cs->stage_cap) {
        HIPC(hipStreamSynchronize(st));
        dev_free(cs->stage); cs->stage = nullptr;
        if (cs->stage_host) { (void)hipHostFree(cs->stage_host); cs->stage_host = nullptr; }
        cs->stage_cap = 0;
        HIPC(dev_malloc((void**)&cs->stage, (size_t)W * spf * 4));
        HIPC(hipHostMalloc((void**)&cs->stage_host, (size_t)W * spf * 4, hipHostMallocDefault));
        cs->stage_cap = (size_t)W * spf;
    }
    std::vector<PsSeg> psegs; std::vector<const CsPush*> pseg_of; std::vector<void*> pouts; PsPlan plan;
    if (ps) {
        for (int i = 0; i < nP; ++i)
            if (P[i].ps) { psegs.push_back({P[i].ps_row, cs->stage + (size_t)out0[i] * spf, (size_t)(P[i].n - P[i].skip) * spf, P[i].last}); pseg_of.push_back(&P[i]); }
        for (const CsPush* f : flush) { psegs.push_back({f->ps_row, nullptr, 0, 1}); pseg_of.push_back(f); }
        for (const CsPush* p : pseg_of) pouts.push_back(p->out_host);
        Q3C(pcm_stage_begin(ps, psegs, plan));
    }
    float *A = ws.bufA, *B = ws.bufB, *C = ws.bufC, *F = ws.bufF;
    float* knew = A + (size_t)QD * N;
    std::vector<int> pos(N);
    std::vector<AttnCsRow> arows(nP);
    std::vector<ColCopy> xin(Np), hist(2 * nP), compact(N), kvsc(N), latsc(N), latg(Lc), solog;
    std::vector<SegCopy> segs;
    std::vector<AttnCbRow> brows(bf ? nP : 0);
    std::vector<const float*> tabs;
    auto kv_col = [&](const CsRow& r, int f) { return bf ? r.blocks[f / bf] + f % bf : r.kv + f; };
    auto lat_col = [&](const CsRow& r, int f) { return bf ? r.blocks[f / bf] + lat_off + f % bf : r.lat + f; };
    std::vector<const uint32_t*> fsrc(on_dev ? N : 0);
    std::vector<uint32_t> fhost(on_dev ? 0 : (size_t)N * 16);
    for (int i = 0; i < nP; ++i) {
        const CsRow& r = cs->rows[P[i].row];
        const int f0 = r.pos, n = P[i].n, x0 = col0[i] + 2 * i;
        arows[i] = {r.kv, f0, f0 + n, col0[i]};
        if (bf) { brows[i] = {(int)tabs.size(), f0, f0 + n, col0[i]}; tabs.insert(tabs.end(), r.blocks.begin(), r.blocks.end()); }
        for (int h = 0; h < 2; ++h) xin[x0 + h] = {f0 - 2 + h >= 0 ? r.hist + h : nullptr, A + x0 + h, 2, Np};
        for (int h = 0; h < 2; ++h) hist[2 * i + h] = {A + x0 + n + h, r.hist + h, Np, 2};
        for (int j = 0; j < n; ++j) {
            const int col = col0[i] + j;
            pos[col] = f0 + j;
            xin[x0 + 2 + j] = {B + col, A + x0 + 2 + j, N, Np};
            compact[col] = {B + x0 + 2 + j, C + col, Np, N};
            kvsc[col] = {knew + col, kv_col(r, f0 + j), N, kp};
            latsc[col] = {C + col, lat_col(r, f0 + j), N, kp};
            if (on_dev) fsrc[col] = P[i].dev + (size_t)j * 16;
            else memcpy(&fhost[(size_t)col * 16], P[i].host + (size_t)j * 16, 64);
        }
    }
    {
        int l0 = 0;
        for (int i : conc) {
            const CsRow& r = cs->rows[P[i].row];
            const int a0 = r.pos + P[i].skip, c0 = a0 - CODEC_CTX_FRAMES, len = P[i].n - P[i].skip + CODEC_CTX_FRAMES;
            for (int j = 0; j < len; ++j) latg[l0 + j] = {lat_col(r, c0 + j), F + l0 + j, kp, Lc};
            segs.push_back({(unsigned long long)(l0 + CODEC_CTX_FRAMES) * spf, (unsigned long long)out0[i] * spf, (unsigned long long)(P[i].n - P[i].skip) * spf});
            l0 += len;
        }
        for (int i : solo) {
            const CsRow& r = cs->rows[P[i].row];
            const int e = r.pos + P[i].n;
            if (bf) for (int f = 0; f < e; ++f) solog.push_back({lat_col(r, f), F + f, kp, e});
            segs.push_back({(unsigned long long)(cs->rows[P[i].row].pos + P[i].skip) * spf, (unsigned long long)out0[i] * spf,
                            (unsigned long long)(P[i].n - P[i].skip) * spf});
        }
    }
    DescBlock db;
    const size_t o_pos = db.add(pos), o_arows = db.add(arows), o_xin = db.add(xin), o_hist = db.add(hist), o_compact = db.add(compact),
                 o_kvsc = db.add(kvsc), o_latsc = db.add(latsc), o_latg = db.add(latg), o_segs = db.add(segs), o_fsrc = db.add(fsrc),
                 o_brows = db.add(brows), o_tabs = db.add(tabs), o_solog = db.add(solog), o_ps = db.add(plan.desc);
    if (db.host.size() > cs->desc_cap) {
        HIPC(hipStreamSynchronize(st));
        dev_free(cs->desc); cs->desc = nullptr; cs->desc_cap = 0;
        HIPC(dev_malloc((void**)&cs->desc, db.host.size() * 2));
        cs->desc_cap = db.host.size() * 2;
    }
    struct Failed {
        q3_codec_stream* cs; const std::vector<CsPush>& P; bool armed = true;
        ~Failed() {
            if (!armed) return;
            (void)hipStreamSynchronize(cs->st);
            for (const CsPush& p : P) codec_stream_reset(cs, p.row);
        }
    } failed{cs, P};
    HIPC(q3_hipMemcpy(cs->desc, db.host.data(), db.host.size(), hipMemcpyHostToDevice));
    auto D = [&](size_t off) { return (const void*)(cs->desc + off); };
    if (on_dev) HIPC(launch_gather_frames((const uint32_t* const*)D(o_fsrc), ws.frames, N, st));
    else HIPC(q3_hipMemcpy(ws.frames, fhost.data(), fhost.size() * 4, hipMemcpyHostToDevice));

    const CodecScope scope(m);
    Q3C(codec_front_quant(m, ws, N, st));
    HIPC(launch_copy_cols((const ColCopy*)D(o_xin), Np, Q, 0, 0, st));
    HIPC(launch_copy_cols((const ColCopy*)D(o_hist), 2 * nP, Q, 0, 0, st));
    Q3C(codec_front_preconv(m, A, B, Np, st));
    HIPC(launch_copy_cols((const ColCopy*)D(o_compact), N, LAT, 0, 0, st));
    const float scale = (float)pow((double)c.dec_head_dim, -0.5);
    Q3C(codec_front_transformer(m, ws, N, st, [&](int l, float* q, float* k, float*, float* ao) -> q3_status {
        const size_t layer_off = (size_t)l * 2 * QD * kp;
        HIPC(launch_rope_c_pos(q, k, cs->cs, cs->sn, (const int*)D(o_pos), c.dec_heads, c.dec_head_dim, N, st));
        HIPC(launch_copy_cols((const ColCopy*)D(o_kvsc), N, 2 * QD, 0, layer_off, st));
        if (bf) HIPC(launch_attn_cb(q, ao, (const AttnCbRow*)D(o_brows), (const float* const*)D(o_tabs), nP, max_tiles, layer_off, c.dec_heads, c.dec_head_dim, N, bf, scale, st));
        else HIPC(launch_attn_cs(q, ao, (const AttnCsRow*)D(o_arows), nP, max_tiles, layer_off, c.dec_heads, c.dec_head_dim, N, cap, scale, st));
        return Q3_OK;
    }));
    HIPC(launch_copy_cols((const ColCopy*)D(o_latsc), N, LAT, 0, 0, st));
    const SegCopy* dsegs = (const SegCopy*)D(o_segs);
    if (!conc.empty()) {
        size_t max_n = 0; for (int i : conc) max_n = std::max(max_n, (size_t)(P[i].n - P[i].skip) * spf);
        HIPC(launch_copy_cols((const ColCopy*)D(o_latg), Lc, LAT, 0, 0, st));
        Q3C(codec_stack_dev(m, ws, F, Lc, st, nullptr, scope));
        HIPC(launch_copy_segs(ws.pcm, cs->stage, dsegs, (int)conc.size(), max_n, st));
    }
    for (size_t k = 0, g0 = 0; k < solo.size(); ++k) {
        const int i = solo[k]; const CsRow& r = cs->rows[P[i].row];
        const int e = r.pos + P[i].n;
        if (bf) { HIPC(launch_copy_cols((const ColCopy*)D(o_solog) + g0, e, LAT, 0, 0, st)); g0 += (size_t)e; }
        else HIPC(launch_copy_rows(r.lat, cap, F, e, LAT, e, st));
        Q3C(codec_stack_dev(m, ws, F, e, st, nullptr, scope));
        HIPC(launch_copy_segs(ws.pcm, cs->stage, dsegs + conc.size() + k, 1, (size_t)(P[i].n - P[i].skip) * spf, st));
    }
    bool raw = false;
    for (int i = 0; i < nP; ++i) raw = raw || !P[i].ps;
    if (W > 0 && raw) HIPC(hipMemcpyAsync(cs->stage_host, cs->stage, (size_t)W * spf * 4, hipMemcpyDeviceToHost, st));
    if (ps) Q3C(pcm_stage_run(ps, psegs, plan, (const PsDesc*)D(o_ps), st));
    HIPC(hipStreamSynchronize(st));
    if (ps) pcm_stage_finish(ps, psegs, plan, pouts.data(), nullptr);
    for (size_t k = 0; k < psegs.size(); ++k) if (pseg_of[k]->n_out) *pseg_of[k]->n_out = plan.count[k];
    for (int i = 0; i < nP; ++i) {
        if (P[i].pcm_host && !P[i].ps) memcpy(P[i].pcm_host, cs->stage_host + (size_t)out0[i] * spf, (size_t)(P[i].n - P[i].skip) * spf * 4);
        cs->rows[P[i].row].pos += P[i].n;
    }
    failed.armed = false; untake.armed = false;
    cs->blocks_peak = std::max(cs->blocks_peak, cs->blocks_in_use);
    return Q3_OK;
}

extern "C" q3_status q3_codec_stream_push(q3_codec_stream* cs, int n_rows, const int* rows, const uint32_t* const* frames_host,
                                          const int* n_frames, float* const* pcm_host, const size_t* cap) {
    if (!cs) return set_err(Q3_INVALID_ARG, "q3_codec_stream_push: null stream");
    if (n_rows < 0 || (n_rows > 0 && (!rows || !frames_host || !n_frames || !pcm_host || !cap)))
        return set_err(Q3_INVALID_ARG, "q3_codec_stream_push: null argument");
    const int spf = samples_per_frame(cs->m->cfg);
    std::vector<char> seen(cs->R, 0);
    std::vector<CsPush> P;
    for (int i = 0; i < n_rows; ++i) {
        const int r = rows[i], n = n_frames[i];
        if (r < 0 || r >= cs->R) return set_err(Q3_INVALID_ARG, "q3_codec_stream_push: row %d out of range (%d rows)", r, cs->R);
        if (seen[r]) return set_err(Q3_INVALID_ARG, "q3_codec_stream_push: row %d listed twice", r);
        seen[r] = 1;
        if (n < 0) return set_err(Q3_INVALID_ARG, "q3_codec_stream_push: negative frame count for row %d", r);
        if (n == 0) continue;
        if (cs->rows[r].pos + n > cs->cap)
            return set_err(Q3_INVALID_ARG, "q3_codec_stream_push: row %d would reach %d frames, the stream holds %d", r, cs->rows[r].pos + n, cs->cap);
        if (!frames_host[i] || !pcm_host[i]) return set_err(Q3_INVALID_ARG, "q3_codec_stream_push: null frames or pcm pointer for row %d", r);
        if (cap[i] < (size_t)n * spf) return set_err(Q3_INVALID_ARG, "q3_codec_stream_push: pcm buffer of row %d too small (%zu < %zu samples)", r, cap[i], (size_t)n * spf);
        for (int f = 0; f < n; ++f)
            for (int g = 1; g < 16; ++g)
                if (frames_host[i][(size_t)f * 16 + g] >= (uint32_t)cs->m->cfg.dec_cb_size)
                    return set_err(Q3_INVALID_ARG, "code %u out of range for codebook %d (row %d, frame %d)", frames_host[i][(size_t)f * 16 + g], g, r, f);
        P.push_back({r, n, 0, frames_host[i], nullptr, pcm_host[i]});
    }
    return codec_stream_push(cs, P);
}

extern "C" q3_status q3_codec_stream_push_out(q3_codec_stream* cs, int n_rows, const int* rows, const uint32_t* const* frames_host, const int* n_frames,
                                              q3_pcm_stage* ps, const int* ps_rows, const int* last,
                                              void* const* out_host, const size_t* cap_samples, size_t* n_samples) {
    if (!cs) return set_err(Q3_INVALID_ARG, "q3_codec_stream_push_out: null stream");
    if (!ps) return set_err(Q3_INVALID_ARG, "q3_codec_stream_push_out: null stage");
    if (n_rows < 0 || (n_rows > 0 && (!rows || !frames_host || !n_frames || !ps_rows || !out_host || !cap_samples || !n_samples)))
        return set_err(Q3_INVALID_ARG, "q3_codec_stream_push_out: null argument");
    Q3C(pcm_stage_check_rows(ps, "q3_codec_stream_push_out", n_rows, ps_rows));
    const int spf = samples_per_frame(cs->m->cfg);
    std::vector<char> seen(cs->R, 0);
    std::vector<CsPush> P;
    for (int i = 0; i < n_rows; ++i) {
        const int r = rows[i], n = n_frames[i], lst = last ? last[i] : 0;
        if (r < 0 || r >= cs->R) return set_err(Q3_INVALID_ARG, "q3_codec_stream_push_out: row %d out of range (%d rows)", r, cs->R);
        if (seen[r]) return set_err(Q3_INVALID_ARG, "q3_codec_stream_push_out: row %d listed twice", r);
        seen[r] = 1;
        n_samples[i] = 0;
        if (n < 0) return set_err(Q3_INVALID_ARG, "q3_codec_stream_push_out: negative frame count for row %d", r);
        if (n == 0 && !lst) continue;
        if (cs->rows[r].pos + n > cs->cap)
            return set_err(Q3_INVALID_ARG, "q3_codec_stream_push_out: row %d would reach %d frames, the stream holds %d", r, cs->rows[r].pos + n, cs->cap);
        if (n > 0 && !frames_host[i]) return set_err(Q3_INVALID_ARG, "q3_codec_stream_push_out: null frames pointer for row %d", r);
        const size_t cnt = pcm_stage_count(ps, ps_rows[i], (size_t)n * spf, lst);
        if (cap_samples[i] < cnt) return set_err(Q3_INVALID_ARG, "q3_codec_stream_push_out: output buffer of row %d too small (%zu < %zu samples)", r, cap_samples[i], cnt);
        if (cnt > 0 && !out_host[i]) return set_err(Q3_INVALID_ARG, "q3_codec_stream_push_out: null output pointer for row %d", r);
        for (int f = 0; f < n; ++f)
            for (int g = 1; g < 16; ++g)
                if (frames_host[i][(size_t)f * 16 + g] >= (uint32_t)cs->m->cfg.dec_cb_size)
                    return set_err(Q3_INVALID_ARG, "code %u out of range for codebook %d (row %d, frame %d)", frames_host[i][(size_t)f * 16 + g], g, r, f);
        CsPush p{r, n, 0, frames_host[i], nullptr, nullptr};
        p.ps = ps; p.ps_row = ps_rows[i]; p.last = lst; p.out_host = out_host[i]; p.n_out = &n_samples[i];
        P.push_back(p);
    }
    return codec_stream_push(cs, P);
}

extern "C" q3_status q3_codec_stream_prime(q3_codec_stream* cs, int row, const uint32_t* frames_host, int n_frames) {
    if (!cs) return set_err(Q3_INVALID_ARG, "q3_codec_stream_prime: null stream");
    if (row < 0 || row >= cs->R) return set_err(Q3_INVALID_ARG, "q3_codec_stream_prime: row %d out of range (%d rows)", row, cs->R);
    if (cs->rows[row].pos != 0) return set_err(Q3_INVALID_ARG, "q3_codec_stream_prime: row %d is at frame %d, state-only frames come first", row, cs->rows[row].pos);
    if (n_frames < 0 || (n_frames > 0 && !frames_host)) return set_err(Q3_INVALID_ARG, "q3_codec_stream_prime: bad frames argument");
    if (n_frames > cs->cap) return set_err(Q3_INVALID_ARG, "q3_codec_stream_prime: %d frames, the stream holds %d", n_frames, cs->cap);
    for (int f = 0; f < n_frames; ++f)
        for (int g = 1; g < 16; ++g)
            if (frames_host[(size_t)f * 16 + g] >= (uint32_t)cs->m->cfg.dec_cb_size)
                return set_err(Q3_INVALID_ARG, "code %u out of range for codebook %d (row %d, frame %d)", frames_host[(size_t)f * 16 + g], g, row, f);
    return codec_stream_push(cs, {CsPush{row, n_frames, n_frames, frames_host, nullptr, nullptr}});
}
```

qwen3_tts_rs_amd/csrc/q3_engine.h:

```cpp
#pragma once
#include "../../include/q3tts.h"
#include "q3_kernels.h"

#include <math.h>
#include <stdarg.h>
#include <stdio.h>
#include <string.h>

#include <algorithm>
#include <atomic>
#include <chrono>
#include <functional>
#include <memory>
#include <string>
#include <thread>
#include <mutex>
#include <unordered_map>
#include <vector>

#include "q3_internal.h"
#include "q3_aql.h"

using namespace q3;
#define Q3_HIDDEN __attribute__((visibility("hidden")))
// ... 185 lines not shown
    if (no4 && w.t1 && M > 2) return 1;
    if (w.t2 && !short_k_wide(N, K) && (M <= 2 || (N <= 1024 && M <= 8))) return 2;
    return 1;
}
static inline void set_w(LinArgs& a, const TW& w, int M, int N, int K) {
    a.tiled = pick_mode(w, M, N, K); a.W = a.tiled == 2 ? w.t2 : w.t1; a.Kpad = kpad_for(a.tiled, K);
}
static inline void set_w2(LinArgs& a, const TW& w, const TW& w2, int M, int N, int K) {
    set_w(a, w, M, N, K); a.W2 = a.tiled == 2 ? w2.t2 : w2.t1;
}
Q3_HIDDEN hipError_t dev_malloc(void** p, size_t bytes);
Q3_HIDDEN void dev_free(void* p);

struct DevPool {
    std::vector<void*> ptrs;
    bool lazy = false;
    hipError_t settle() { return q3_null_stream_sync(); }
    template <typename T> hipError_t alloc(T** p, size_t count) {
        void* q = nullptr;
        hipError_t e = dev_malloc(&q, (count ? count : 1) * sizeof(T));
        if (e != hipSuccess) return e;
        ptrs.push_back(q); *p = (T*)q;
        return q3_null_stream_memset(q, (count ? count : 1) * sizeof(T), !lazy);
    }
    void release_all() {
        if (lazy) (void)q3_null_stream_sync();
        for (void* p : ptrs) dev_free(p);
        ptrs.clear(); lazy = false;
    }
    ~DevPool() { release_all(); }
};

constexpr int CODEC_CTX_FRAMES = 12;

struct CodecWS {
    int cap_frames = 0;
    int cap_front = 0;
    float *bufA = nullptr, *bufB = nullptr, *bufC = nullptr, *bufF = nullptr, *bufD = nullptr, *bufE = nullptr;
    float *cs = nullptr, *sn = nullptr;
    uint32_t* frames = nullptr; float* pcm = nullptr;
    void release() {
        dev_free(bufA); dev_free(bufB); dev_free(bufC); dev_free(bufF); dev_free(bufD); dev_free(bufE); dev_free(cs); dev_free(sn); dev_free(frames); dev_free(pcm);
        bufA = bufB = bufC = bufF = bufD = bufE = cs = sn = pcm = nullptr; frames = nullptr; cap_frames = 0; cap_front = 0;
    }
};

struct LmBuf { float *X, *SUM, *QKV, *Q, *ATT, *ACT, *PART; };
struct LmDims { int H, I, nh, nkv, layers; float eps; };

struct BatReq {
    q3_request r{}; std::vector<uint32_t> text, instruct, ref_codes, ref_text; std::vector<float> xvec;
    void own(const q3_request& q, int hidden) {
        r = q;
        text.assign(q.text_ids, q.text_ids + (q.text_ids ? q.n_text : 0));
        instruct.assign(q.instruct_ids, q.instruct_ids + (q.instruct_ids ? q.n_instruct : 0));
        ref_codes.assign(q.ref_codes, q.ref_codes + (q.ref_codes ? (size_t)q.n_ref * 16 : 0));
        ref_text.assign(q.ref_text_ids, q.ref_text_ids + (q.ref_text_ids ? q.n_ref_text : 0));
        if (q.xvector) xvec.assign(q.xvector, q.xvector + hidden);
        fix();
    }
    void fix() {
        r.text_ids = text.empty() ? nullptr : text.data(); r.n_text = (int32_t)text.size();
        r.instruct_ids = instruct.empty() ? nullptr : instruct.data(); r.n_instruct = (int32_t)instruct.size();
        r.ref_codes = ref_codes.empty() ? nullptr : ref_codes.data(); r.n_ref = (int32_t)(ref_codes.size() / 16);
        r.ref_text_ids = ref_text.empty() ? nullptr : ref_text.data(); r.n_ref_text = (int32_t)ref_text.size();
        r.xvector = xvec.empty() ? nullptr : xvec.data();
    }
};
struct SeqInfo {
    q3_request req; std::vector<uint32_t> text, instruct, ref_codes, ref_text; std::vector<float> xvec; bool icl = false;
    int prefill_len = 0, trailing_len = 0, row_base = 0, n_rows = 0, trail_base = 0, pad_row = 0;
    int n_frames = 0; bool done = false;
    int start_run = 0, limit = 0, stream_pos = 0;
    int reused = 0;
    bool idle = false;
    int max_length_req = 0;
    bool opened = false, text_closed = true;
    std::vector<uint32_t> text_all;
    int n_trail = 0, ready = 0x7fffffff, committed = 0;
    q3_request request() const {
        static const uint32_t none[1] = {0};
        q3_request r = req;
        r.text_ids = text.data(); r.n_text = (int32_t)text.size();
        r.instruct_ids = instruct.empty() ? nullptr : instruct.data(); r.n_instruct = (int32_t)instruct.size();
        r.ref_codes = ref_codes.empty() ? nullptr : ref_codes.data(); r.n_ref = (int32_t)(ref_codes.size() / 16);
        r.ref_text_ids = !ref_text.empty() ? ref_text.data() : icl ? none : nullptr; r.n_ref_text = (int32_t)ref_text.size();
        r.xvector = xvec.empty() ? nullptr : xvec.data();
        return r;
    }
};

struct ProfAcc { double ms = 0; double bytes = 0; long launches = 0; };
struct ParkShelf { std::mutex mu; bool alive = true; std::vector<std::pair<void*, size_t>> blocks; };
enum { PARK_MAX_SEGS = 24, PARK_PAYLOAD_INTS = 8 };
constexpr size_t PARK_DESC_BYTES = (size_t)PARK_MAX_SEGS * 32 + (size_t)PARK_PAYLOAD_INTS * 16;
struct ProfShape { int M, N, K, epi, rms, produce, tiled, count; };

struct OutSettings {
    uint32_t rate = 24000; int fmt = Q3_PCM_F32;
    int tempo = 1000, cents = 0;
    int gain_mB = 0, ceil_mB = 0;
    int loud = Q3_LOUD_OFF, target_mB = -1900, prior_mB = 0;
    int sil_mB = 0, edge_ms = 0, pause_ms = 20;
    bool plain() const {
        return rate == 24000 && fmt == Q3_PCM_F32 && tempo == 1000 && cents == 0 && gain_mB == 0 && ceil_mB == 0 && loud == Q3_LOUD_OFF && sil_mB == 0;
    }
    size_t sample_bytes() const { return fmt == Q3_PCM_F32 ? 4 : fmt == Q3_PCM_S16 ? 2 : 1; }
};

struct q3_session {
    q3_model* m = nullptr; int B = 0;
    hipStream_t stream = nullptr; bool owns_stream = true;
    DevPool pool;
    std::vector<SeqInfo> seq;
    q3_options opts{};
    int max_frames = 0, max_seq = 0, prefill_len = 0, n_splits = 1;
    int* limit = nullptr;
    SampleRow* sample_rows = nullptr;
    int row_cap = 0, repl_base = 0;
    LmBuf tb{}, cb{};
    float *LASTH = nullptr, *LOGITS = nullptr, *CP_IN = nullptr, *CP_LOGITS = nullptr;
    float* wide_ws = nullptr; size_t wide_ws_bytes = 0;
    float *kcache = nullptr, *vcache = nullptr, *ckcache = nullptr, *cvcache = nullptr;
    size_t kv_layer_stride = 0, ckv_layer_stride = 0;
    bool paged = false; unsigned long long* kv_table = nullptr; std::vector<std::vector<float*>> kv_rows;
    std::vector<BatReq> ragged;
    int prefill_info[8] = {0, 0, 0, 0, 0, 0, 0, 0};
    bool regrouped = false;
    bool prefix_common = false;
    int kv_overflow_row = -1;
    bool kv_bf16 = false, kv_in_bf16 = false; unsigned long long* kv_conv = nullptr;
    float *rows = nullptr, *embeds = nullptr, *xvec = nullptr; int n_rows_total = 0;
    uint32_t* ids_dev = nullptr; int *tr_dev = nullptr, *ci_dev = nullptr; float *proj_e = nullptr, *proj_h = nullptr;
    uint32_t* ref_codes_dev = nullptr;
    int *trail_base = nullptr, *trail_len = nullptr, *pad_row = nullptr;
    int* text_ready = nullptr;
    uint32_t* app_ids = nullptr; float *app_e = nullptr, *app_h = nullptr, *app_out = nullptr;
    int* flush_buf = nullptr; size_t flush_cap = 0;
    uint32_t* tok = nullptr; uint8_t* seen = nullptr; int *frame_idx = nullptr, *pos = nullptr, *token_count = nullptr;
    float* U = nullptr; uint32_t* codes = nullptr;
    float* logits_hist = nullptr; float* cp_logits_hist = nullptr; bool debug = false;
    bool prefilled = false; int frames_run = 0;
    uint64_t uid = 0; char* park_desc = nullptr; std::shared_ptr<ParkShelf> shelf;
    hipGraphExec_t graph_exec = nullptr; hipGraph_t graph = nullptr;
    q3::AqlProgram* aql = nullptr; int aql_mode = 0; bool aql_tried = false, aql_failed = false;
    bool precapture = false;
    CodecWS cws;
    q3_codec_stream* cstream = nullptr;
    q3_pcm_stage* ostage = nullptr; bool out_started = false;
    std::vector<OutSettings> out;
    hipStream_t dec_stream = nullptr; hipEvent_t dec_ev = nullptr;
    std::vector<CodecWS> par_ws; std::vector<hipStream_t> par_streams;
    CodecWS seg_ws;
    std::vector<uint32_t> codes_host; bool codes_host_valid = false;
    int stream_pos = 0;
    int stream_mode = 0;
    bool profile = false; ProfAcc prof_linear;
    bool legacy_attn = getenv("Q3_LEGACY_ATTN") != nullptr;
    bool proj_tables = getenv("Q3_NO_PROJ_TABLES") == nullptr;
    bool qkv_tables = getenv("Q3_NO_QKV_TABLES") == nullptr;
    bool ksplit = getenv("Q3_NO_KSPLIT") == nullptr;
    bool cp_attn = getenv("Q3_NO_CP_ATTN") == nullptr;
    bool no_chunk = getenv("Q3_NO_CHUNK") != nullptr;
    std::vector<std::pair<hipEvent_t, hipEvent_t>> prof_events; std::vector<double> prof_event_bytes;
    std::vector<hipEvent_t> prof_pool; size_t prof_pool_next = 0;
    std::vector<ProfShape> prof_shapes;
#ifdef Q3_TRACE
    unsigned long long* trace_buf = nullptr; int trace_node = 0, trace_cap = 0;
    struct TraceMeta { int kind, a, b, c, d, e, f; };
    std::vector<TraceMeta> trace_meta;
    unsigned long long* trace_next(int kind, int a, int b, int c, int d = 0, int e = 0, int f = 0) {
        if (!trace_buf || trace_node >= trace_cap) return nullptr;
        trace_meta.push_back({kind, a, b, c, d, e, f});
        return trace_buf + (size_t)(trace_node++) * TRACE_NODE;
    }
#endif
    ~q3_session();
};


Q3_HIDDEN void model_destroy(q3_model* m);
Q3_HIDDEN void retile_bf16(const uint16_t* src, int N, int K, uint16_t* dst, int mode);
Q3_HIDDEN q3_status codec_reserve(const q3_model* m, CodecWS& ws, int T, int Tf = 0);
Q3_HIDDEN int samples_per_frame(const q3_config& c);
Q3_HIDDEN q3_status codec_decode_dev(const q3_model* m, CodecWS& ws, int T, hipStream_t st, float** taps, int c0 = 0, int resident = 0);
struct Q3_HIDDEN CodecScope { int planes, resident; explicit CodecScope(const q3_model* m, int resident = 0); ~CodecScope(); CodecScope(const CodecScope&) = delete; };
using CodecAttnFn = std::function<q3_status(int layer, float* q, float* k, float* v, float* ao)>;
Q3_HIDDEN q3_status codec_rope_table(const q3_config& c, int n, float* cs_dev, float* sn_dev);
Q3_HIDDEN q3_status codec_front_quant(const q3_model* m, CodecWS& ws, int T, hipStream_t st);
Q3_HIDDEN q3_status codec_front_preconv(const q3_model* m, const float* x, float* y, int L, hipStream_t st);
Q3_HIDDEN q3_status codec_front_transformer(const q3_model* m, CodecWS& ws, int T, hipStream_t st, const CodecAttnFn& rope_attn);
Q3_HIDDEN q3_status codec_stack_dev(const q3_model* m, CodecWS& ws, float* cur, int L, hipStream_t st, float** taps, const CodecScope& scope);
struct CsPush {
    int row; int n; int skip; const uint32_t* host; const uint32_t* dev; float* pcm_host;
    q3_pcm_stage* ps = nullptr; int ps_row = -1; int last = 0; void* out_host = nullptr; size_t* n_out = nullptr;
};
Q3_HIDDEN q3_status codec_stream_create(q3_model* m, int rows, int max_frames, hipStream_t st, q3_codec_stream** out, int block_frames = 0,
                                        int max_blocks = 0);
Q3_HIDDEN q3_status codec_stream_push(q3_codec_stream* cs, const std::vector<CsPush>& pushes);
Q3_HIDDEN int codec_stream_pos(const q3_codec_stream* cs, int row);
Q3_HIDDEN void codec_stream_blocks(const q3_codec_stream* cs, int row, int upto, int* held, int* need);
Q3_HIDDEN void codec_stream_reset(q3_codec_stream* cs, int row);
struct PsSeg { int row; const float* dev; size_t n; int last; };
struct PsDesc {
    const float* src; const float* tail_in; float* tail_out; const float* taps; void* out;
    long long base, i0;
    int n_new, n_out, L, M, fmt, pad;
};
struct PsPlan { std::vector<PsDesc> desc; std::vector<size_t> off, count; size_t bytes = 0; bool late = false; };
Q3_HIDDEN void resampler_taps(int L, int M, std::vector<float>& out);
Q3_HIDDEN int pcm_stage_rows(const q3_pcm_stage* ps);
Q3_HIDDEN void pcm_stage_reset(q3_pcm_stage* ps, int row);
Q3_HIDDEN q3_status pcm_stage_check_rows(const q3_pcm_stage* ps, const char* who, int n_rows, const int* rows);
Q3_HIDDEN size_t pcm_stage_count(const q3_pcm_stage* ps, int row, size_t n, int last);
Q3_HIDDEN q3_status out_set_output(const char* who, OutSettings& o, uint32_t sample_rate, int format);
Q3_HIDDEN q3_status out_set_tempo(const char* who, OutSettings& o, int tempo_permille);
Q3_HIDDEN q3_status out_set_pitch(const char* who, OutSettings& o, int cents);
Q3_HIDDEN q3_status out_set_level(const char* who, OutSettings& o, int gain_mB, int ceiling_mB);
Q3_HIDDEN q3_status out_set_loudness(const char* who, OutSettings& o, int mode, int target_mB, int prior_mB);
Q3_HIDDEN q3_status out_set_silence(const char* who, OutSettings& o, int threshold_mB, int edge_ms, int pause_ms);
Q3_HIDDEN q3_status pcm_stage_apply(q3_pcm_stage* ps, int row, const char* who, const OutSettings& o);
Q3_HIDDEN const OutSettings& pcm_stage_settings(const q3_pcm_stage* ps, int row);
Q3_HIDDEN void out_loudness_at_rest(const OutSettings& o, float* mean_square, float* gain, int* blocks, int* gated);
Q3_HIDDEN void out_silence_at_rest(int64_t* n_in, int64_t* n_out, int64_t* lead_cut, int64_t* pause_cut, int64_t* trail_cut);
Q3_HIDDEN q3_status pcm_stage_begin(q3_pcm_stage* ps, const std::vector<PsSeg>& segs, PsPlan& plan);
Q3_HIDDEN q3_status pcm_stage_run(q3_pcm_stage* ps, const std::vector<PsSeg>& segs, PsPlan& plan, const PsDesc* desc_dev, hipStream_t st);
Q3_HIDDEN void pcm_stage_finish(q3_pcm_stage* ps, const std::vector<PsSeg>& segs, const PsPlan& plan, void* const* out_host, size_t* n_samples);
Q3_HIDDEN q3_status pcm_stage_push_dev(q3_pcm_stage* ps, const std::vector<PsSeg>& segs, hipStream_t st, void* const* out_host, size_t* n_samples);
Q3_HIDDEN hipError_t sync_frames(q3_session* s);
Q3_HIDDEN q3_status kv_reserve_row(q3_session* s, int b, int n_pos);
Q3_HIDDEN q3_status kv_reserve_frames(q3_session* s, int frames);
Q3_HIDDEN void kv_release_row(q3_session* s, int b);
Q3_HIDDEN LmDims talker_dims(const q3_config& c);
Q3_HIDDEN LmDims cp_dims(const q3_config& c);
Q3_HIDDEN q3_status talker_step(q3_session* s, const int* pos_dev, int pos_static, bool with_head, int rows_per_seq = 1,
                                const int* text_ready = nullptr);
Q3_HIDDEN SampleRow sample_row(const q3_options& o);
using PromptShape = q3_prompt_shape_rec;
Q3_HIDDEN int icl_frame_cap(int n_text);
Q3_HIDDEN PromptShape prompt_shape(const q3_request& r, int n_text);
static inline PromptShape prompt_shape(const q3_request& r) { return prompt_shape(r, r.n_text); }
Q3_HIDDEN void prompt_positions(const PromptShape& sh, const q3_request& r, int row_base, int* text_row, int* codec_id);
Q3_HIDDEN long row_worst_units(int prefill_len, int limit, bool bf16);
Q3_HIDDEN q3_request idle_request(int chunk_frames);
Q3_HIDDEN q3_status session_create(q3_model* m, const q3_request* reqs, int batch, int frame_budget, int prompt_budget, q3_session** out,
                                   hipStream_t borrow = nullptr);
Q3_HIDDEN q3_status lm_layer(q3_session* s, const LmDims& d, const LayerW& w, LmBuf& b, float* kc, float* vc, int max_seq,
                             const int* pos_dev, int pos_static, int n_splits, int rows_per_seq = 1, bool skip_qkv = false,
                             const CpGatherArgs* fold = nullptr, int paged_layer = -1);
struct TextPiece { int b; const uint32_t* ids; int n; bool last; };
Q3_HIDDEN q3_status session_text_enable(q3_session* s);
Q3_HIDDEN q3_status session_append_many(q3_session* s, const std::vector<TextPiece>& pieces);
Q3_HIDDEN int session_row_remaining(const q3_session* s, int b);
Q3_HIDDEN int session_row_committed(const q3_session* s, int b);
Q3_HIDDEN q3_status session_refresh_codes(q3_session* s);
enum { ROW_MOVE_COPY = 0, ROW_MOVE_EXCHANGE = 1 };
struct RowSeg { void* src; void* dst; unsigned long long bytes; int mode; int pad; };
Q3_HIDDEN hipError_t launch_row_move(const RowSeg* segs_dev, int n_segs, size_t max_bytes, hipStream_t st);
Q3_HIDDEN int parked_frames(const q3_parked* p, const uint32_t** codes);
Q3_HIDDEN int parked_committed(const q3_parked* p);
Q3_HIDDEN int parked_pages(const q3_parked* p);
Q3_HIDDEN bool parked_done(const q3_parked* p);
Q3_HIDDEN const SeqInfo& parked_seq(const q3_parked* p);
Q3_HIDDEN q3_status transplant_row(q3_session* s, int b, q3_session* side, int j, int limit);
Q3_HIDDEN q3_status side_prefill(q3_session* host, const q3_request* reqs, const int* limit_req, int n, bool open_text, bool closed,
                                 bool prefix_common, hipStream_t borrow, std::unique_ptr<q3_session>* side_out, int* limit_out,
                                 const std::function<void()>& created = nullptr, bool staged_only = false);
```

qwen3_tts_rs_amd/csrc/q3_session.hip:

```cpp
#include "q3_engine.h"
#include "q3_prefix_cache.h"

hipError_t sync_frames(q3_session* s) {
    if (s->aql) {
        std::string why;
        if (!q3::aql_wait(s->aql, &why)) { s->aql_failed = true; set_err(Q3_HIP_ERROR, "AQL frame submission: %s", why.c_str()); return hipErrorUnknown; }
    }
    return hipStreamSynchronize(s->stream);
}

static hipError_t run_linear(q3_session* s, const LinArgs& a_in) {
    LinArgs a = a_in;
    a.ws = s->wide_ws; a.ws_bytes = s->wide_ws_bytes;
#ifdef Q3_TRACE
    a.trace = s->trace_next(0, a.M, a.N, a.K, a.epi, a.norm_w ? 1 : 0, a.tiled);
#endif
    if (!s->profile) return launch_linear(a, s->stream);
    hipEvent_t e0, e1;
    if (s->prof_pool_next + 2 <= s->prof_pool.size()) { e0 = s->prof_pool[s->prof_pool_next++]; e1 = s->prof_pool[s->prof_pool_next++]; }
    else {
        hipError_t e = hipEventCreate(&e0); if (e != hipSuccess) return e;
        e = hipEventCreate(&e1); if (e != hipSuccess) return e;
        s->prof_pool.push_back(e0); s->prof_pool.push_back(e1); s->prof_pool_next = s->prof_pool.size();
    }
// ... 461 lines not shown
        }
        if (q.icl) {
            if (r.n_ref_text < 0) return set_err(Q3_INVALID_ARG, "bad reference text");
            q.ref_text.assign(r.ref_text_ids, r.ref_text_ids + r.n_ref_text);
            for (uint32_t id : q.ref_text) if (id >= (uint32_t)c.text_vocab) return set_err(Q3_INVALID_ARG, "reference text id %u out of range", id);
            q.req.opts.repetition_penalty = r.opts.repetition_penalty < 1.5 ? 1.5 : r.opts.repetition_penalty;
            q.req.opts.max_length = sh.limit;
            if (b == 0) s->opts = q.req.opts;
        }
        q.prefill_len = sh.prefill_len; q.trailing_len = sh.trailing_len;
        q.row_base = rows; q.n_rows = sh.n_rows;
        rows += q.n_rows;
        if (q.prefill_len != s->seq[0].prefill_len)
            return set_err(Q3_UNSUPPORTED, "all sequences of a batch must have the same prefill length (%d vs %d)", q.prefill_len, s->seq[0].prefill_len);
    }
    s->prefill_len = s->seq[0].prefill_len;
    s->n_rows_total = rows;
    s->max_frames = frame_budget > 1 ? frame_budget : 1;
    for (auto& q : s->seq) {
        if (q.req.opts.max_length < 1) return set_err(Q3_INVALID_ARG, "max_length must be at least 1");
        q.limit = q.req.opts.max_length; q.start_run = 0;
        if (q.limit > s->max_frames) s->max_frames = q.limit;
        if (q.n_rows > s->row_cap) s->row_cap = q.n_rows;
    }
    s->opts.max_length = s->max_frames;
    if (s->row_cap < 1024) s->row_cap = 1024;
    if (prompt_budget > 0 && s->row_cap < prompt_budget + 1024) s->row_cap = prompt_budget + 1024;
    s->repl_base = rows;
    s->max_seq = (prompt_budget > s->prefill_len ? prompt_budget : s->prefill_len) + s->max_frames + 1;
    if (s->max_seq > m->rope_len) return set_err(Q3_KV_OVERFLOW, "sequence length %d exceeds the RoPE table (%d)", s->max_seq, m->rope_len);
    {
        static const int ns_env = [] { const char* e = getenv("Q3_ATTN_SPLITS"); return e ? atoi(e) : 0; }();
        int ns = ns_env > 0 ? ns_env : (batch <= 2 ? 1024 : 512) / (batch * c.n_kv_heads);
        const int cap = ns_env > 0 ? MAX_SPLITS : (s->max_seq > 2048 ? MAX_SPLITS : 16);
        if (ns < 1) ns = 1; if (ns > cap) ns = cap; s->n_splits = ns;
    }
    {
        if (borrow) { s->stream = borrow; s->owns_stream = false; }
        else {
            {
                std::lock_guard<std::mutex> g(m->stream_mu);
                if (!m->idle_streams.empty()) { s->stream = m->idle_streams.back(); m->idle_streams.pop_back(); }
            }
            if (!s->stream) {
                int least = 0, greatest = 0;
                HIPC(hipDeviceGetStreamPriorityRange(&least, &greatest));
                HIPC(hipStreamCreateWithPriority(&s->stream, hipStreamNonBlocking, greatest));
            }
        }
    }
    const int B = batch, H = c.hidden, CH = c.cp_hidden;
    s->pool.lazy = true;
    auto alloc_lm = [&](LmBuf& b, const LmDims& d, int nsplit) -> hipError_t {
        const int QD = d.nh * HEAD_DIM, KD = d.nkv * HEAD_DIM;
        const size_t R = batch > 16 ? (size_t)up16(batch) : 16;
        hipError_t e;
        if ((e = s->pool.alloc(&b.X, R * d.H)) != hipSuccess) return e;
        if ((e = s->pool.alloc(&b.SUM, R * d.H)) != hipSuccess) return e;
        if ((e = s->pool.alloc(&b.QKV, R * (QD + 2 * KD))) != hipSuccess) return e;
        if ((e = s->pool.alloc(&b.Q, R * QD)) != hipSuccess) return e;
        if ((e = s->pool.alloc(&b.ATT, R * QD)) != hipSuccess) return e;
        if ((e = s->pool.alloc(&b.ACT, R * d.I)) != hipSuccess) return e;
        return s->pool.alloc(&b.PART, R * d.nh * nsplit * PART_STRIDE);
    };
    HIPC(alloc_lm(s->tb, talker_dims(c), s->n_splits));
    HIPC(alloc_lm(s->cb, cp_dims(c), 1));
    if (B > 16) {
        size_t need = 0;
        auto upd = [&](int N, int K, int epi) { if (N % 128 == 0 && K % 128 == 0) { const size_t b = gemm_wide_ws_bytes(B, N, K, epi); if (b > need) need = b; } };
        const int QDt = c.n_heads * HEAD_DIM, KDt = c.n_kv_heads * HEAD_DIM, QDc = c.cp_heads * HEAD_DIM, KDc = c.cp_kv_heads * HEAD_DIM;
        upd(QDt + 2 * KDt, H, EPI_NONE); upd(H, QDt, EPI_RESID); upd(c.inter, H, EPI_SWIGLU); upd(H, c.inter, EPI_RESID); upd(c.codec_vocab, H, EPI_NONE);
        upd(QDc + 2 * KDc, c.cp_hidden, EPI_NONE); upd(c.cp_hidden, QDc, EPI_RESID); upd(c.cp_inter, c.cp_hidden, EPI_SWIGLU); upd(c.cp_hidden, c.cp_inter, EPI_RESID);
        upd(c.cp_vocab, c.cp_hidden, EPI_NONE); upd(c.cp_hidden, H, EPI_NONE);
        if (need) { HIPC(s->pool.alloc(&s->wide_ws, need / 4)); s->wide_ws_bytes = need; }
    }
    HIPC(s->pool.alloc(&s->LASTH, (size_t)B * H));
    HIPC(s->pool.alloc(&s->LOGITS, (size_t)B * c.codec_vocab));
    HIPC(s->pool.alloc(&s->CP_IN, (size_t)(B > 16 ? up16(B) : 16) * H));
    HIPC(s->pool.alloc(&s->CP_LOGITS, (size_t)15 * B * c.cp_vocab));
    s->kv_layer_stride = (size_t)B * c.n_kv_heads * s->max_seq * HEAD_DIM;
    {
        const char* e = getenv("Q3_KV_CONTIGUOUS");
        s->paged = !(e && atoi(e) != 0);
        if (s->paged) {
            if (s->max_seq > KV_MAX_PAGES * KV_PAGE_POS) return set_err(Q3_KV_OVERFLOW, "sequence length %d exceeds a row's page table (%d)", s->max_seq, KV_MAX_PAGES * KV_PAGE_POS);
            HIPC(s->pool.alloc(&s->kv_table, (size_t)B * KV_MAX_PAGES));
            HIPC(s->pool.alloc(&s->kv_conv, (size_t)2 * B * KV_MAX_PAGES));
            HIPC(s->pool.alloc(&s->park_desc, PARK_DESC_BYTES));
            s->shelf = std::make_shared<ParkShelf>();
            s->kv_rows.resize((size_t)B);
            for (auto& r : s->kv_rows) r.reserve(KV_MAX_PAGES);
        } else {
            HIPC(s->pool.alloc(&s->kcache, s->kv_layer_stride * c.n_layers));
            HIPC(s->pool.alloc(&s->vcache, s->kv_layer_stride * c.n_layers));
        }
    }
    s->ckv_layer_stride = (size_t)B * c.cp_kv_heads * (c.n_groups + 1) * HEAD_DIM;
    HIPC(s->pool.alloc(&s->ckcache, 2 * s->ckv_layer_stride * c.cp_layers + 64));
    s->cvcache = s->ckcache + s->ckv_layer_stride * c.cp_layers + 64;
    HIPC(s->pool.alloc(&s->rows, ((size_t)rows + (size_t)B * s->row_cap) * H));
    HIPC(s->pool.alloc(&s->limit, B));
    HIPC(s->pool.alloc(&s->sample_rows, B));
    {
        std::vector<int> lim(B); std::vector<SampleRow> sr(B);
        for (int b = 0; b < B; ++b) { lim[b] = s->seq[b].limit; sr[b] = sample_row(s->seq[b].req.opts); }
        HIPC(q3_hipMemcpy(s->limit, lim.data(), B * 4, hipMemcpyHostToDevice));
        HIPC(q3_hipMemcpy(s->sample_rows, sr.data(), B * sizeof(SampleRow), hipMemcpyHostToDevice));
    }
    HIPC(s->pool.alloc(&s->embeds, (size_t)B * s->prefill_len * H));
    HIPC(s->pool.alloc(&s->xvec, (size_t)B * H));
    HIPC(s->pool.alloc(&s->ids_dev, (size_t)rows)); HIPC(s->pool.alloc(&s->tr_dev, (size_t)B * s->prefill_len)); HIPC(s->pool.alloc(&s->ci_dev, (size_t)B * s->prefill_len));
    HIPC(s->pool.alloc(&s->proj_e, (size_t)rows * c.text_dim)); HIPC(s->pool.alloc(&s->proj_h, (size_t)rows * c.text_dim));
    HIPC(s->pool.alloc(&s->trail_base, B)); HIPC(s->pool.alloc(&s->trail_len, B)); HIPC(s->pool.alloc(&s->pad_row, B));
    HIPC(s->pool.alloc(&s->tok, B)); HIPC(s->pool.alloc(&s->seen, (size_t)B * c.codec_vocab));
    HIPC(s->pool.alloc(&s->frame_idx, B)); HIPC(s->pool.alloc(&s->pos, B)); HIPC(s->pool.alloc(&s->token_count, B));
    HIPC(s->pool.alloc(&s->U, (size_t)B * (s->max_frames + 2)));
    HIPC(s->pool.alloc(&s->codes, (size_t)B * s->max_frames * 16));
    std::vector<float> U((size_t)B * (s->max_frames + 2), 0.0f);
    for (int b = 0; b < B; ++b) {
        uint64_t st;
        const q3_options& o = reqs[b].opts;
        uint64_t seed = o.seed;
        if (!o.has_seed) seed = (uint64_t)std::chrono::high_resolution_clock::now().time_since_epoch().count() + 0x9E37ULL * b;
        q3_rng_seed(seed, &st);
        for (int i = 0; i <= s->max_frames; ++i) U[(size_t)b * (s->max_frames + 2) + i] = q3_rng_next(&st);
    }
    HIPC(q3_hipMemcpy(s->U, U.data(), U.size() * 4, hipMemcpyHostToDevice));
    HIPC(s->pool.settle());
    s->pool.lazy = false;
    *out = s.release();
    return Q3_OK;
}

q3_session::~q3_session() {
    if (!m) return;
    (void)hipSetDevice(m->device);
    if (stream) (void)hipStreamSynchronize(stream);
    if (dec_stream) (void)hipStreamSynchronize(dec_stream);
    for (auto st : par_streams) (void)hipStreamSynchronize(st);
    if (aql) q3::aql_program_destroy(aql);
    for (int b = 0; b < (int)kv_rows.size(); ++b) kv_release_row(this, b);
    if (shelf) {
        std::lock_guard<std::mutex> g(shelf->mu);
        shelf->alive = false;
        for (auto& blk : shelf->blocks) dev_free(blk.first);
        shelf->blocks.clear();
    }
    if (graph_exec) (void)hipGraphExecDestroy(graph_exec);
    if (graph) (void)hipGraphDestroy(graph);
    for (auto& ev : prof_pool) (void)hipEventDestroy(ev);
    for (auto st : par_streams) (void)hipStreamDestroy(st);
    if (ostage) q3_pcm_stage_free(ostage);
    if (cstream) q3_codec_stream_free(cstream);
    cws.release(); seg_ws.release();
    for (auto& w : par_ws) w.release();
    if (dec_ev) (void)hipEventDestroy(dec_ev);
    if (dec_stream) (void)hipStreamDestroy(dec_stream);
    if (stream && owns_stream) {
        std::lock_guard<std::mutex> g(m->stream_mu);
        if (m->idle_streams.size() < 16) { m->idle_streams.push_back(stream); stream = nullptr; }
    }
    if (stream && owns_stream) (void)hipStreamDestroy(stream);
    pool.release_all();
    if (m->refs.fetch_sub(1) == 1) model_destroy(m);
}

extern "C" void q3_session_free(q3_session* s) { delete s; }

extern "C" q3_status q3_session_set_kv_dtype(q3_session* s, int dtype) {
    if (!s) return set_err(Q3_INVALID_ARG, "null session");
    if (s->prefilled) return set_err(Q3_INVALID_ARG, "q3_session_set_kv_dtype must be called before prefill");
    if (dtype != Q3_DTYPE_F32 && dtype != Q3_DTYPE_BF16) return set_err(Q3_INVALID_ARG, "q3_session_set_kv_dtype: unknown dtype %d", dtype);
    if (dtype == Q3_DTYPE_BF16 && !s->paged) return set_err(Q3_UNSUPPORTED, "bf16 K/V needs the paged cache (Q3_KV_CONTIGUOUS is set)");
    s->kv_bf16 = dtype == Q3_DTYPE_BF16;
    return Q3_OK;
}

extern "C" q3_status q3_session_set_debug(q3_session* s, int capture) {
    if (!s) return set_err(Q3_INVALID_ARG, "null session");
    if (s->prefilled) return set_err(Q3_INVALID_ARG, "set_debug must be called before prefill");
    if (capture && s->text_ready) return set_err(Q3_UNSUPPORTED, "set_debug: the session has open text rows");
    s->debug = capture != 0;
    if (s->debug && !s->logits_hist) {
        const q3_config& c = s->m->cfg;
        HIPC(hipSetDevice(s->m->device));
        HIPC(s->pool.alloc(&s->logits_hist, (size_t)s->B * (s->max_frames + 1) * c.codec_vocab));
        HIPC(s->pool.alloc(&s->cp_logits_hist, (size_t)s->max_frames * 15 * s->B * c.cp_vocab));
    }
    return Q3_OK;
}
extern "C" q3_status q3_session_set_profile(q3_session* s, int enable) {
    if (!s) return set_err(Q3_INVALID_ARG, "null session");
    if (enable && s->text_ready) return set_err(Q3_UNSUPPORTED, "set_profile: the session has open text rows");
    s->profile = enable != 0;
    return Q3_OK;
}
extern "C" q3_status q3_session_stream(q3_session* s, void** stream) {
    if (!s || !stream) return set_err(Q3_INVALID_ARG, "null argument");
    *stream = (void*)s->stream;
    return Q3_OK;
}
extern "C" q3_status q3_session_prefill_len(q3_session* s, int b, int* prefill_len, int* trailing_len) {
    if (!s || b < 0 || b >= s->B) return set_err(Q3_INVALID_ARG, "bad sequence index");
    if (!s->ragged.empty()) {
        if (prefill_len) *prefill_len = prompt_shape(s->ragged[(size_t)b].r).prefill_len;
        if (trailing_len) *trailing_len = -1;
        return Q3_OK;
    }
    if (prefill_len) *prefill_len = s->seq[b].prefill_len;
    if (trailing_len) *trailing_len = s->seq[b].trailing_len;
    return Q3_OK;
}

static q3_status text_project(q3_session* s, const uint32_t* ids_dev, int n, float* out_rows) {
    const q3_model* m = s->m; const q3_config& c = m->cfg;
    const int TD = c.text_dim, H = c.hidden;
    if (n > s->n_rows_total) return set_err(Q3_INVALID_ARG, "text_project: %d rows exceed the session's %d", n, s->n_rows_total);
    float *e = s->proj_e, *h = s->proj_h;
    q3_status st = Q3_OK;
    hipError_t er = launch_gather_rows_bf16(m->text_emb, ids_dev, e, n, TD, s->stream);
    if (er == hipSuccess && n >= 48 && TD % 64 == 0 && H % 64 == 0 && !s->no_chunk) {
        GemmArgs g1; g1.W = m->fc1w.t1; g1.x = e; g1.ldx = TD; g1.bias = m->fc1b; g1.y = h; g1.ldy = TD;
        g1.M = n; g1.N = TD; g1.K = TD; g1.Kpad = (TD + 31) / 32 * 32; g1.epi = EPI_SILU;
        er = launch_lm_gemm(g1, s->stream);
        if (er == hipSuccess) {
            GemmArgs g2; g2.W = m->fc2w.t1; g2.x = h; g2.ldx = TD; g2.bias = m->fc2b; g2.y = out_rows; g2.ldy = H;
            g2.M = n; g2.N = H; g2.K = TD; g2.Kpad = (TD + 31) / 32 * 32; g2.epi = EPI_NONE;
            er = launch_lm_gemm(g2, s->stream);
        }
    } else
    for (int r0 = 0; r0 < n && er == hipSuccess; r0 += 8) {
        const int M = (n - r0) < 8 ? (n - r0) : 8;
        LinArgs a;
        a.N = TD; a.K = TD; set_w(a, m->fc1w, M, TD, TD); a.x = e + (size_t)r0 * TD; a.ldx = TD; a.bias = m->fc1b; a.y = h + (size_t)r0 * TD; a.ldy = TD; a.M = M; a.epi = EPI_SILU;
        er = launch_linear(a, s->stream);
        if (er != hipSuccess) break;
        LinArgs b2;
        b2.N = H; b2.K = TD; set_w(b2, m->fc2w, M, H, TD); b2.x = h + (size_t)r0 * TD; b2.ldx = TD; b2.bias = m->fc2b; b2.y = out_rows + (size_t)r0 * H; b2.ldy = H; b2.M = M; b2.epi = EPI_NONE;
        er = launch_linear(b2, s->stream);
    }
    if (er != hipSuccess) st = set_err(Q3_HIP_ERROR, "text projection: %s", hipGetErrorString(er));
    return st;
}

static int slot_row0(const q3_session* s, int b) { return s->repl_base + b * s->row_cap; }
static int open_n_trail(const SeqInfo& q) { return prompt_shape(q.request(), (int)q.text_all.size()).n_trail; }
static void open_trailing_ids(const SeqInfo& q, std::vector<uint32_t>& out) {
    std::vector<uint32_t> all(q.ref_text);
    all.insert(all.end(), q.text_all.begin(), q.text_all.end());
    out.assign(all.end() - open_n_trail(q), all.end());
}
static void open_counts(SeqInfo& q) {
    q.n_trail = open_n_trail(q);
    q.trailing_len = q.n_trail + (q.text_closed ? 1 : 0);
    q.ready = q.text_closed ? 0x7fffffff : q.n_trail;
    if (q.icl && q.text_closed) q.limit = std::min(q.max_length_req, icl_frame_cap((int)q.text_all.size()));
}
static hipError_t project_group(q3_session* s, const uint32_t* ids_dev) {
    const q3_model* m = s->m; const q3_config& c = m->cfg;
    const int TD = c.text_dim, H = c.hidden;
    hipError_t er = launch_gather_rows_bf16(m->text_emb, ids_dev, s->app_e, 8, TD, s->stream);
    if (er != hipSuccess) return er;
    LinArgs a;
    a.N = TD; a.K = TD; set_w(a, m->fc1w, 8, TD, TD); a.x = s->app_e; a.ldx = TD; a.bias = m->fc1b; a.y = s->app_h; a.ldy = TD; a.M = 8; a.epi = EPI_SILU;
    er = launch_linear(a, s->stream);
    if (er != hipSuccess) return er;
    LinArgs b2;
    b2.N = H; b2.K = TD; set_w(b2, m->fc2w, 8, H, TD); b2.x = s->app_h; b2.ldx = TD; b2.bias = m->fc2b; b2.y = s->app_out; b2.ldy = H; b2.M = 8; b2.epi = EPI_NONE;
    return launch_linear(b2, s->stream);
}
static q3_status project_appended(q3_session* s, int b, const std::vector<uint32_t>& ids, int dst) {
    const int H = s->m->cfg.hidden, n = (int)ids.size(), row0 = slot_row0(s, b);
    if (n <= 0) return Q3_OK;
    std::vector<uint32_t> padded((size_t)(n + 7) / 8 * 8);
    for (size_t i = 0; i < padded.size(); ++i) padded[i] = ids[i < (size_t)n ? i : (size_t)n - 1];
    hipError_t er = hipSuccess;
    for (int r0 = 0; r0 < n && er == hipSuccess; r0 += 8) {
        const int k = (n - r0) < 8 ? (n - r0) : 8;
        er = hipMemcpyAsync(s->app_ids, padded.data() + r0, 8 * 4, hipMemcpyHostToDevice, s->stream);
        if (er == hipSuccess) er = project_group(s, s->app_ids);
        if (er == hipSuccess)
            er = hipMemcpyAsync(s->rows + (size_t)(row0 + dst + r0) * H, s->app_out, (size_t)k * H * 4, hipMemcpyDeviceToDevice, s->stream);
    }
    const hipError_t es = sync_frames(s);
    if (er == hipSuccess) er = es;
    if (er != hipSuccess) return set_err(Q3_HIP_ERROR, "appended text projection: %s", hipGetErrorString(er));
    return Q3_OK;
}
static q3_status publish_text(q3_session* s, int b) {
    const SeqInfo& q = s->seq[(size_t)b];
    const int v[3] = {q.trailing_len, q.ready, q.limit};
    HIPC(hipMemcpyAsync(s->trail_len + b, &v[0], 4, hipMemcpyHostToDevice, s->stream));
    HIPC(hipMemcpyAsync(s->text_ready + b, &v[1], 4, hipMemcpyHostToDevice, s->stream));
    HIPC(hipMemcpyAsync(s->limit + b, &v[2], 4, hipMemcpyHostToDevice, s->stream));
    HIPC(sync_frames(s));
    return Q3_OK;
}
static bool any_open_text(const q3_session* s) { for (const auto& q : s->seq) if (q.opened && !q.text_closed) return true; return false; }

static q3_status alloc_text_state(q3_session* s) {
    if (s->text_ready) return Q3_OK;
    const q3_config& c = s->m->cfg;
    HIPC(s->pool.alloc(&s->text_ready, (size_t)s->B));
    HIPC(s->pool.alloc(&s->app_ids, 8)); HIPC(s->pool.alloc(&s->app_e, (size_t)8 * c.text_dim));
    HIPC(s->pool.alloc(&s->app_h, (size_t)8 * c.text_dim)); HIPC(s->pool.alloc(&s->app_out, (size_t)8 * c.hidden));
    const std::vector<int> closed((size_t)s->B, 0x7fffffff);
// ... 963 lines not shown
}
extern "C" q3_status q3_session_next_chunks_out(q3_session* s, void* const* out_host, const size_t* cap_samples, size_t* n_samples, int* done) {
    if (!s) return set_err(Q3_INVALID_ARG, "q3_session_next_chunks_out: null session");
    if (!n_samples || !done || !out_host || !cap_samples) return set_err(Q3_INVALID_ARG, "q3_session_next_chunks_out: null argument");
    if (s->m->device < 0) return set_err(Q3_INVALID_ARG, "q3_session_next_chunks_out: the model has no device");
    if (!s->ostage) {
        const int chunk = s->opts.chunk_frames > 0 ? s->opts.chunk_frames : 10;
        Q3C(q3_pcm_stage_create(s->m->device, s->B, (size_t)chunk * samples_per_frame(s->m->cfg), &s->ostage));
        for (int b = 0; b < s->B; ++b) Q3C(pcm_stage_apply(s->ostage, b, "q3_session_next_chunks_out", s->out[(size_t)b]));
    }
    s->out_started = true;
    return next_chunks(s, nullptr, cap_samples, n_samples, done, true, out_host);
}
static q3_status next_chunks(q3_session* s, float* const* pcm_host, const size_t* cap, size_t* n_samples, int* done, bool out, void* const* out_host) {
    HIPC(hipSetDevice(s->m->device));
    if (!s->prefilled) Q3C(q3_session_prefill(s));
    Q3C(refresh_codes(s));
    const int chunk = s->opts.chunk_frames > 0 ? s->opts.chunk_frames : 10;
    const int spf = samples_per_frame(s->m->cfg);
    for (int b = 0; b < s->B; ++b) {
        SeqInfo& q = s->seq[b];
        while (!q.done && q.n_frames - q.stream_pos < chunk && (q.opened ? row_capacity(s, q) : session_remaining(s)) > 0) {
            Q3C(q3_session_generate(s, chunk - (q.n_frames - q.stream_pos), 1));
            Q3C(refresh_codes(s));
        }
    }
    std::vector<int> avail((size_t)s->B, 0);
    std::vector<char> held((size_t)s->B, 0), ends((size_t)s->B, 0);
    for (int b = 0; b < s->B; ++b) {
        const SeqInfo& q = s->seq[b];
        int a = std::min(q.n_frames - q.stream_pos, chunk);
        held[(size_t)b] = q.opened && !q.done && a < chunk;
        if (a < 0 || held[(size_t)b]) a = 0;
        avail[(size_t)b] = a;
        ends[(size_t)b] = held[(size_t)b] ? 0 : (a <= 0 || (q.done && q.stream_pos + a >= q.n_frames)) ? 1 : 0;
        if (out) {
            const size_t cnt = pcm_stage_count(s->ostage, b, (size_t)a * spf, ends[(size_t)b]);
            if (cnt > 0 && (!out_host[b] || cap[b] < cnt))
                return set_err(Q3_INVALID_ARG, "q3_session_next_chunks_out: output buffer of row %d too small (%zu samples needed)", b, cnt);
        } else if (a > 0 && pcm_host && pcm_host[b] && (!cap || cap[b] < (size_t)a * spf))
            return set_err(Q3_INVALID_ARG, "q3_session_next_chunks: pcm buffer of row %d too small", b);
    }
    std::vector<CsPush> pushes;
    std::vector<float> tmp;
    for (int b = 0; b < s->B; ++b) {
        SeqInfo& q = s->seq[b];
        const int a = avail[(size_t)b];
        n_samples[b] = out ? 0 : (size_t)a * spf;
        if (out) {
            const int last = ends[(size_t)b];
            if (a <= 0 && !last) continue;
            if (s->stream_mode == 1 && !q.icl) {
                if (!s->cstream) Q3C(codec_stream_create(s->m, s->B, s->max_frames, s->stream, &s->cstream));
                int n = 0, skip = 0, sp = 0;
                if (a > 0) {
                    if (codec_stream_pos(s->cstream, b) > q.stream_pos) codec_stream_reset(s->cstream, b);
                    sp = codec_stream_pos(s->cstream, b);
                    n = q.stream_pos + a - sp; skip = q.stream_pos - sp;
                }
                CsPush p{b, n, skip, nullptr, s->codes + ((size_t)b * s->max_frames + sp) * 16, nullptr};
                p.ps = s->ostage; p.ps_row = b; p.last = last; p.out_host = out_host[b]; p.n_out = &n_samples[b];
                pushes.push_back(p);
            } else {
                tmp.resize((size_t)a * spf);
                if (a > 0) Q3C(chunk_decode_row(s, b, a, tmp.data(), tmp.size(), nullptr));
                const float* in = tmp.data(); const size_t n_in = tmp.size();
                Q3C(q3_pcm_stage_push(s->ostage, 1, &b, &in, &n_in, &last, &out_host[b], &cap[b], &n_samples[b]));
            }
            continue;
        }
        if (a <= 0) continue;
        if (s->stream_mode == 1 && !q.icl) {
            if (!s->cstream) Q3C(codec_stream_create(s->m, s->B, s->max_frames, s->stream, &s->cstream));
            if (codec_stream_pos(s->cstream, b) > q.stream_pos) codec_stream_reset(s->cstream, b);
            const int sp = codec_stream_pos(s->cstream, b);
            pushes.push_back({b, q.stream_pos + a - sp, q.stream_pos - sp, nullptr, s->codes + ((size_t)b * s->max_frames + sp) * 16,
                              pcm_host ? pcm_host[b] : nullptr});
        } else {
            Q3C(chunk_decode_row(s, b, a, pcm_host ? pcm_host[b] : nullptr, cap ? cap[b] : 0, nullptr));
        }
    }
    if (!pushes.empty()) Q3C(codec_stream_push(s->cstream, pushes));
    for (int b = 0; b < s->B; ++b) {
        SeqInfo& q = s->seq[b];
        q.stream_pos += avail[(size_t)b];
        done[b] = held[(size_t)b] ? 0 : (avail[(size_t)b] <= 0 || (q.done && q.stream_pos >= q.n_frames)) ? 1 : 0;
    }
    return Q3_OK;
}

extern "C" q3_status q3_session_frames(q3_session* s, int b, int* n_frames, int* done) {
    if (!s || b < 0 || b >= s->B) return set_err(Q3_INVALID_ARG, "bad sequence index");
    HIPC(hipSetDevice(s->m->device));
    Q3C(refresh_codes(s));
    if (n_frames) *n_frames = s->seq[b].n_frames;
    if (done) *done = s->seq[b].done ? 1 : 0;
    return Q3_OK;
}

extern "C" q3_status q3_session_codes(q3_session* s, int b, uint32_t* codes_host, int cap_frames, int* n_frames) {
    if (!s || b < 0 || b >= s->B) return set_err(Q3_INVALID_ARG, "bad sequence index");
    HIPC(hipSetDevice(s->m->device));
    Q3C(refresh_codes(s));
    const int n = s->seq[b].n_frames;
    if (n_frames) *n_frames = n;
    if (codes_host) {
        if (cap_frames < n) return set_err(Q3_INVALID_ARG, "codes buffer too small (%d < %d frames)", cap_frames, n);
        memcpy(codes_host, &s->codes_host[(size_t)b * s->max_frames * 16], (size_t)n * 16 * 4);
    }
    return Q3_OK;
}

static q3_status decode_range_on(q3_session* s, int b, int f0, int f1, hipStream_t st, float* pcm_host, size_t cap, size_t* n_samples) {
    const int T = f1 - f0, spf = samples_per_frame(s->m->cfg);
    if (n_samples) *n_samples = (size_t)T * spf;
    if (T == 0) return Q3_OK;
    Q3C(codec_reserve(s->m, s->cws, T));
    HIPC(hipMemcpyAsync(s->cws.frames, s->codes + ((size_t)b * s->max_frames + f0) * 16, (size_t)T * 16 * 4, hipMemcpyDeviceToDevice, st));
    Q3C(codec_decode_dev(s->m, s->cws, T, st, nullptr));
    HIPC(hipStreamSynchronize(st));
    if (pcm_host) {
        if (cap < (size_t)T * spf) return set_err(Q3_INVALID_ARG, "pcm buffer too small");
        HIPC(q3_hipMemcpy(pcm_host, s->cws.pcm, (size_t)T * spf * 4, hipMemcpyDeviceToHost));
    }
    return Q3_OK;
}

extern "C" q3_status q3_session_decode(q3_session* s, int b, int f0, int f1, float* pcm_host, size_t cap, size_t* n_samples) {
    if (!s || b < 0 || b >= s->B) return set_err(Q3_INVALID_ARG, "bad sequence index");
    HIPC(hipSetDevice(s->m->device));
    Q3C(refresh_codes(s));
    if (f0 < 0 || f1 < f0 || f1 > s->seq[b].n_frames) return set_err(Q3_INVALID_ARG, "bad frame range [%d,%d) of %d", f0, f1, s->seq[b].n_frames);
    const int T = f1 - f0, spf = samples_per_frame(s->m->cfg);
    const SeqInfo& q = s->seq[b];
    if (!q.ref_codes.empty() && s->prefilled && f0 == 0 && f1 == q.n_frames) {
        const int n_ref = (int)(q.ref_codes.size() / 16), total = n_ref + T;
        const size_t all = (size_t)total * spf, cut = (size_t)n_ref * all / (size_t)(total > 0 ? total : 1);
        if (n_samples) *n_samples = all - cut;
        Q3C(codec_reserve(s->m, s->cws, total));
        HIPC(hipMemcpyAsync(s->cws.frames, q.ref_codes.data(), (size_t)n_ref * 16 * 4, hipMemcpyHostToDevice, s->stream));
        if (T > 0) HIPC(hipMemcpyAsync(s->cws.frames + (size_t)n_ref * 16, s->codes + (size_t)b * s->max_frames * 16, (size_t)T * 16 * 4, hipMemcpyDeviceToDevice, s->stream));
        Q3C(codec_decode_dev(s->m, s->cws, total, s->stream, nullptr));
        HIPC(sync_frames(s));
        if (pcm_host) {
            if (cap < all - cut) return set_err(Q3_INVALID_ARG, "pcm buffer too small");
            HIPC(q3_hipMemcpy(pcm_host, s->cws.pcm + cut, (all - cut) * 4, hipMemcpyDeviceToHost));
        }
        return Q3_OK;
    }
    return decode_range_on(s, b, f0, f1, s->stream, pcm_host, cap, n_samples);
}

static constexpr bool DECODE_OVERLAP_DEFAULT = true;
extern "C" q3_status q3_session_run(q3_session* s, int use_graph, float** pcm_host, const size_t* cap, size_t* n_samples, q3_timing* timing) {
    if (!s) return set_err(Q3_INVALID_ARG, "null session");
    if (any_open_text(s)) return set_err(Q3_UNSUPPORTED, "q3_session_run: a row's text is still open (q3_session_append_text with last != 0 closes it; or drive the session with q3_session_generate)");
    using clk = std::chrono::steady_clock;
    auto ms = [](clk::time_point a, clk::time_point b) { return std::chrono::duration<double, std::milli>(b - a).count(); };
    const auto t0 = clk::now();
    s->precapture = use_graph != 0;
    Q3C(q3_session_prefill(s));
    const auto t1 = clk::now();
    const int overlap_env = [] { const char* e = getenv("Q3_DECODE_OVERLAP"); return e ? (atoi(e) != 0 ? 1 : 0) : -1; }();
    const int resident_env = [] { const char* e = getenv("Q3_DECODE_RESIDENT"); const int v = e ? atoi(e) : 1; return v < 0 ? 0 : (v > 2 ? 2 : v); }();
    const int seg_env = [] { const char* e = getenv("Q3_DECODE_SEG"); const int v = e ? atoi(e) : 256; return v < 16 ? 16 : v; }();
    const bool overlap_wanted = overlap_env >= 0 ? overlap_env != 0 : (DECODE_OVERLAP_DEFAULT && s->B >= 2 && s->B <= 16);
    bool overlap = overlap_wanted && !s->debug && !s->profile && s->max_frames > seg_env;
    for (auto& q : s->seq) if (!q.ref_codes.empty()) overlap = false;
    const int spf = samples_per_frame(s->m->cfg);
    if (!overlap) {
        Q3C(q3_session_generate(s, s->max_frames, use_graph));
        Q3C(refresh_codes(s));
        const auto t2 = clk::now();
        int total = 0;
        static const int conc = [] { const char* e = getenv("Q3_DECODE_PAIRS"); const int v = e ? atoi(e) : 2; return v < 1 ? 1 : (v > 8 ? 8 : v); }();
        bool any_icl = false;
        for (auto& q : s->seq) any_icl = any_icl || !q.ref_codes.empty();
        if (conc > 1 && s->B > 1 && !any_icl) {
            while ((int)s->par_ws.size() < conc - 1) {
                s->par_ws.emplace_back();
                hipStream_t st = nullptr;
                HIPC(hipStreamCreateWithFlags(&st, hipStreamNonBlocking));
                s->par_streams.push_back(st);
            }
            auto ws_of = [&](int k) -> CodecWS& { return k == 0 ? s->cws : s->par_ws[(size_t)k - 1]; };
            auto st_of = [&](int k) { return k == 0 ? s->stream : s->par_streams[(size_t)k - 1]; };
            if (pcm_host)
                for (int b = 0; b < s->B; ++b)
                    if (pcm_host[b] && s->seq[b].n_frames && (!cap || cap[b] < (size_t)s->seq[b].n_frames * spf)) return set_err(Q3_INVALID_ARG, "pcm buffer too small");
            for (int b0 = 0; b0 < s->B; b0 += conc) {
                const int nb = (s->B - b0) < conc ? (s->B - b0) : conc;
                for (int k = 0; k < nb; ++k) {
                    const int b = b0 + k, T = s->seq[b].n_frames;
                    if (n_samples) n_samples[b] = (size_t)T * spf;
                    total += T;
                    if (T == 0) continue;
                    Q3C(codec_reserve(s->m, ws_of(k), T));
                    HIPC(hipMemcpyAsync(ws_of(k).frames, s->codes + (size_t)b * s->max_frames * 16, (size_t)T * 16 * 4, hipMemcpyDeviceToDevice, st_of(k)));
                    Q3C(codec_decode_dev(s->m, ws_of(k), T, st_of(k), nullptr));
                    if (pcm_host && pcm_host[b])
                        HIPC(hipMemcpyAsync(pcm_host[b], ws_of(k).pcm, (size_t)T * spf * 4, hipMemcpyDeviceToHost, st_of(k)));
                }
                for (int k = 0; k < nb; ++k) HIPC(hipStreamSynchronize(st_of(k)));
            }
        } else
        for (int b = 0; b < s->B; ++b) {
            size_t n = 0;
            Q3C(q3_session_decode(s, b, 0, s->seq[b].n_frames, pcm_host ? pcm_host[b] : nullptr, cap ? cap[b] : 0, &n));
            if (n_samples) n_samples[b] = n;
            total += s->seq[b].n_frames;
        }
        const auto t3 = clk::now();
        if (timing) { timing->prefill_ms = ms(t0, t1); timing->generation_ms = ms(t1, t2); timing->decode_ms = ms(t2, t3); timing->generation_frames = total; }
        return Q3_OK;
    }
    HIPC(hipSetDevice(s->m->device));
    static const int cus = [] { const char* e = getenv("Q3_DECODE_CUS"); const int v = e ? atoi(e) : 0; return v <= 0 ? 0 : (v < 8 ? 8 : (v > 248 ? 248 : v & ~7)); }();
    if (!s->dec_stream) {
        if (cus) {
            uint32_t mask[8] = {0, 0, 0, 0, 0, 0, 0, 0};
            for (int i = 256 - cus; i < 256; ++i) mask[i >> 5] |= 1u << (i & 31);
            HIPC(hipExtStreamCreateWithCUMask(&s->dec_stream, 8, mask));
        } else {
            int least = 0, greatest = 0;
            HIPC(hipDeviceGetStreamPriorityRange(&least, &greatest));
            HIPC(hipStreamCreateWithPriority(&s->dec_stream, hipStreamNonBlocking, least));
        }
    }
    Q3C(codec_reserve(s->m, s->seg_ws, seg_env + CODEC_CTX_FRAMES, s->max_frames));
    struct Split {
        q3::AqlProgram* p = nullptr;
        void release() { if (p) { std::string why; q3::aql_restrict_cus(p, 0, &why); p = nullptr; } }
        ~Split() { release(); }
    } split;
    if (cus && s->aql && !s->aql_failed) { std::string why; if (q3::aql_restrict_cus(s->aql, 256 - cus, &why)) split.p = s->aql; }
    std::vector<int> dec_pos((size_t)s->B, 0);
    std::thread worker; q3_status wst = Q3_OK; std::string werr;
    double join_wait_ms = 0.0; int n_dispatch = 0;
    auto join = [&]() -> q3_status {
        if (worker.joinable()) worker.join();
        if (wst != Q3_OK) return set_err(wst, "%s", werr.c_str());
        return Q3_OK;
    };
    struct Job { int b, a, e; };
    auto seg_enqueue = [s, spf, pcm_host, cap](const Job& j, CodecWS& ws, hipStream_t st, int resident) -> q3_status {
        const int c0 = j.a > CODEC_CTX_FRAMES ? j.a - CODEC_CTX_FRAMES : 0;
        if (pcm_host && pcm_host[j.b] && (!cap || cap[j.b] < (size_t)j.e * spf)) return set_err(Q3_INVALID_ARG, "pcm buffer too small");
        HIPC(hipMemcpyAsync(ws.frames, s->codes + (size_t)j.b * s->max_frames * 16, (size_t)j.e * 16 * 4, hipMemcpyDeviceToDevice, st));
        Q3C(codec_decode_dev(s->m, ws, j.e, st, nullptr, c0, resident));
        if (pcm_host && pcm_host[j.b])
            HIPC(hipMemcpyAsync(pcm_host[j.b] + (size_t)j.a * spf, ws.pcm + (size_t)(j.a - c0) * spf, (size_t)(j.e - j.a) * spf * 4, hipMemcpyDeviceToHost, st));
        return Q3_OK;
    };
    auto collect = [&](bool final_pass) {
        std::vector<Job> jobs;
        for (int b = 0; b < s->B; ++b) {
            const SeqInfo& q = s->seq[b];
            const int e = (q.done || final_pass) ? q.n_frames : (q.n_frames < s->frames_run ? q.n_frames : s->frames_run);
            if (e > dec_pos[(size_t)b] && (final_pass || q.done || e - dec_pos[(size_t)b] >= 16)) {
                for (int a = dec_pos[(size_t)b]; a < e; a += seg_env) jobs.push_back({b, a, a + seg_env < e ? a + seg_env : e});
                dec_pos[(size_t)b] = e;
            }
        }
        return jobs;
    };
    auto dispatch = [&]() -> q3_status {
        std::vector<Job> jobs = collect(false);
        if (jobs.empty()) return Q3_OK;
        {
            const auto j0 = clk::now();
            Q3C(join());
            join_wait_ms += ms(j0, clk::now()); ++n_dispatch;
        }
        worker = std::thread([s, jobs, seg_enqueue, resident_env, &wst, &werr]() {
            if (hipSetDevice(s->m->device) != hipSuccess) { wst = Q3_HIP_ERROR; werr = "hipSetDevice failed in the decode thread"; return; }
            for (const Job& j : jobs) {
                const q3_status st = seg_enqueue(j, s->seg_ws, s->dec_stream, resident_env);
                if (st != Q3_OK) { wst = st; werr = q3_last_error(); return; }
            }
        });
        return Q3_OK;
    };
    const int tail_env = [] { const char* e = getenv("Q3_DECODE_TAIL"); const int v = e ? atoi(e) : 32; return v < 16 ? 16 : v; }();
    q3_status st = Q3_OK;
    while (st == Q3_OK && session_remaining(s) > 0 && !all_done(s)) {
        int n = seg_env;
        const int left = session_remaining(s);
        if (left > tail_env && left - n < tail_env) n = left - tail_env;
        st = q3_session_generate(s, n, use_graph);
        if (st == Q3_OK) st = refresh_codes(s);
        if (st == Q3_OK && session_remaining(s) > 0 && !all_done(s)) st = dispatch();
    }
    const auto t2 = clk::now();
    split.release();
    { const q3_status js = join(); if (st == Q3_OK) st = js; }
    if (st != Q3_OK) { hipStreamSynchronize(s->dec_stream); return st; }
    {
        const int conc = 2;
        auto ws_of = [&](int k) -> CodecWS& { return k == 0 ? s->cws : s->par_ws[(size_t)k - 1]; };
        auto st_of = [&](int k) { return k == 0 ? s->stream : s->par_streams[(size_t)k - 1]; };
        auto tail = [&]() -> q3_status {
            std::vector<Job> jobs = collect(true);
            while ((int)s->par_ws.size() < conc - 1) {
                hipStream_t pst = nullptr;
                HIPC(hipStreamCreateWithFlags(&pst, hipStreamNonBlocking));
                s->par_ws.emplace_back(); s->par_streams.push_back(pst);
            }
            for (int k = 0; k < conc; ++k) Q3C(codec_reserve(s->m, ws_of(k), seg_env + CODEC_CTX_FRAMES, s->max_frames));
            for (size_t i = 0; i < jobs.size(); ++i) Q3C(seg_enqueue(jobs[i], ws_of((int)(i % conc)), st_of((int)(i % conc)), 0));
            return Q3_OK;
        };
        st = tail();
        hipError_t he = hipStreamSynchronize(s->dec_stream);
        for (int k = 0; k < conc && k <= (int)s->par_streams.size(); ++k) { const hipError_t e2 = hipStreamSynchronize(st_of(k)); if (he == hipSuccess) he = e2; }
        if (st != Q3_OK) return st;
        HIPC(he);
    }
    int total = 0;
    for (int b = 0; b < s->B; ++b) {
        if (n_samples) n_samples[b] = (size_t)s->seq[b].n_frames * spf;
        total += s->seq[b].n_frames;
    }
    const auto t3 = clk::now();
    if (timing) { timing->prefill_ms = ms(t0, t1); timing->generation_ms = ms(t1, t2); timing->decode_ms = ms(t2, t3); timing->generation_frames = total; }
    const bool log_env = getenv("Q3_DECODE_LOG") != nullptr;
    if (log_env)
        fprintf(stderr, "q3_session_run overlap: resident %d seg %d tail %d, %d dispatches, frame loop waited %.3f ms for the enqueue thread, frames %.1f ms, exposed decode %.1f ms\n",
                resident_env, seg_env, tail_env, n_dispatch, join_wait_ms, ms(t1, t2), ms(t2, t3));
    return Q3_OK;
}

extern "C" q3_status q3_session_set_stream_mode(q3_session* s, int mode) {
    if (!s || (mode != 0 && mode != 1)) return set_err(Q3_INVALID_ARG, "q3_session_set_stream_mode: mode must be 0 (context-free) or 1 (continuous)");
    s->stream_mode = mode;
    return Q3_OK;
}

extern "C" q3_status q3_session_next_chunk(q3_session* s, float* pcm_host, size_t cap, size_t* n_samples, int* done) {
    if (!s) return set_err(Q3_INVALID_ARG, "null session");
    if (s->B != 1) return set_err(Q3_UNSUPPORTED, "streaming sessions are batch 1 (StreamingSession, lib.rs:1484)");
    if (!s->prefilled) { s->precapture = true; Q3C(q3_session_prefill(s)); }
    Q3C(refresh_codes(s));
    SeqInfo& q = s->seq[0];
    const int chunk = s->opts.chunk_frames > 0 ? s->opts.chunk_frames : 10;
    while (!q.done && q.n_frames - s->stream_pos < chunk && session_remaining(s) > 0) {
        int need = chunk - (q.n_frames - s->stream_pos);
        Q3C(q3_session_generate(s, need, 1));
        Q3C(refresh_codes(s));
    }
    int avail = q.n_frames - s->stream_pos;
    if (avail > chunk) avail = chunk;
    if (q.opened && !q.done && avail < chunk) { if (n_samples) *n_samples = 0; if (done) *done = 0; return Q3_OK; }
    if (avail <= 0) { if (n_samples) *n_samples = 0; if (done) *done = 1; return Q3_OK; }
    const bool chunk_done = q.done && s->stream_pos + avail >= q.n_frames;
    static const bool no_ahead = getenv("Q3_STREAM_NO_AHEAD") != nullptr;
    int ahead = 0;
    if (!no_ahead && !q.done && (s->aql || s->graph_exec) && !s->aql_failed && !s->debug && !s->profile) {
        ahead = chunk - (q.n_frames - (s->stream_pos + avail));
        if (ahead > session_remaining(s)) ahead = session_remaining(s);
        if (ahead < 0) ahead = 0;
    }
    const bool first = s->stream_pos == 0;
    auto launch_ahead = [&]() -> q3_status {
        Q3C(kv_reserve_frames(s, ahead));
        if (s->aql) HIPC(hipStreamSynchronize(s->stream));
        return frames_enqueue(s, ahead);
    };
    hipStream_t dst = s->stream;
    if (ahead > 0 && !first) {
        if (!s->dec_stream) HIPC(hipStreamCreateWithFlags(&s->dec_stream, hipStreamNonBlocking));
        Q3C(launch_ahead());
        dst = s->dec_stream;
    }
    const int spf = samples_per_frame(s->m->cfg);
    const float* src = nullptr;
    if (s->stream_mode == 1 && !q.icl) {
        const int a0 = s->stream_pos, e = s->stream_pos + avail;
        const int c0 = a0 > CODEC_CTX_FRAMES ? a0 - CODEC_CTX_FRAMES : 0;
        Q3C(codec_reserve(s->m, s->cws, chunk + CODEC_CTX_FRAMES, s->max_frames));
        HIPC(hipMemcpyAsync(s->cws.frames, s->codes, (size_t)e * 16 * 4, hipMemcpyDeviceToDevice, dst));
        Q3C(codec_decode_dev(s->m, s->cws, e, dst, nullptr, c0));
        src = s->cws.pcm + (size_t)(a0 - c0) * spf;
    } else {
        Q3C(codec_reserve(s->m, s->cws, avail));
        HIPC(hipMemcpyAsync(s->cws.frames, s->codes + (size_t)s->stream_pos * 16, (size_t)avail * 16 * 4, hipMemcpyDeviceToDevice, dst));
        Q3C(codec_decode_dev(s->m, s->cws, avail, dst, nullptr));
        src = s->cws.pcm;
    }
    if (ahead > 0 && first) {
        if (!s->dec_ev) HIPC(hipEventCreateWithFlags(&s->dec_ev, hipEventDisableTiming));
        HIPC(hipEventRecord(s->dec_ev, s->stream));
        Q3C(launch_ahead());
        HIPC(hipEventSynchronize(s->dec_ev));
    } else {
        HIPC(hipStreamSynchronize(dst));
    }
    if (n_samples) *n_samples = (size_t)avail * spf;
    if (pcm_host) {
        if (cap < (size_t)avail * spf) return set_err(Q3_INVALID_ARG, "pcm buffer too small");
        HIPC(q3_hipMemcpy(pcm_host, src, (size_t)avail * spf * 4, hipMemcpyDeviceToHost));
    }
    s->stream_pos += avail;
    if (done) *done = chunk_done ? 1 : 0;
    return Q3_OK;
}

extern "C" q3_status q3_session_get(q3_session* s, int what, int b, void* out, size_t bytes) {
    if (!s || !out || b < 0 || b >= s->B) return set_err(Q3_INVALID_ARG, "bad argument");
    const q3_config& c = s->m->cfg;
    HIPC(hipSetDevice(s->m->device));
    HIPC(sync_frames(s));
    const void* src = nullptr; size_t need = 0;
    switch (what) {
        case Q3_GET_PREFILL_EMBEDS: src = s->embeds + (size_t)b * s->prefill_len * c.hidden; need = (size_t)s->prefill_len * c.hidden * 4; break;
        case Q3_GET_LAST_HIDDEN: src = s->LASTH + (size_t)b * c.hidden; need = (size_t)c.hidden * 4; break;
        case Q3_GET_LOGITS: src = s->LOGITS + (size_t)b * c.codec_vocab; need = (size_t)c.codec_vocab * 4; break;
        case Q3_GET_TRAILING: src = s->rows + (size_t)s->seq[b].trail_base * c.hidden; need = (size_t)s->seq[b].trailing_len * c.hidden * 4; break;
        case Q3_GET_PAD_EMBED: src = s->rows + (size_t)s->seq[b].pad_row * c.hidden; need = (size_t)c.hidden * 4; break;
        case Q3_GET_LOGITS_HIST:
            if (!s->logits_hist) return set_err(Q3_INVALID_ARG, "session has no debug capture");
            src = s->logits_hist + (size_t)b * (s->max_frames + 1) * c.codec_vocab; need = (size_t)(s->frames_run + 1) * c.codec_vocab * 4; break;
        case Q3_GET_TOKEN: src = s->tok + b; need = 4; break;
        case Q3_GET_CP_LOGITS: {
            need = (size_t)15 * c.cp_vocab * 4;
            if (bytes < need) return set_err(Q3_INVALID_ARG, "buffer too small");
            for (int g = 0; g < 15; ++g)
                HIPC(q3_hipMemcpy((char*)out + (size_t)g * c.cp_vocab * 4, s->CP_LOGITS + ((size_t)g * s->B + b) * c.cp_vocab, (size_t)c.cp_vocab * 4, hipMemcpyDeviceToHost));
            return Q3_OK;
        }
        case Q3_GET_CP_LOGITS_HIST: {
            if (!s->cp_logits_hist) return set_err(Q3_INVALID_ARG, "session has no debug capture");
            need = (size_t)s->frames_run * 15 * c.cp_vocab * 4;
            if (bytes < need) return set_err(Q3_INVALID_ARG, "buffer too small");
            for (int f = 0; f < s->frames_run; ++f)
                for (int g = 0; g < 15; ++g)
                    HIPC(q3_hipMemcpy((char*)out + ((size_t)f * 15 + g) * c.cp_vocab * 4,
                                   s->cp_logits_hist + (((size_t)f * 15 + g) * s->B + b) * c.cp_vocab, (size_t)c.cp_vocab * 4, hipMemcpyDeviceToHost));
            return Q3_OK;
        }
        default: return set_err(Q3_INVALID_ARG, "unknown item %d", what);
    }
    if (bytes < need) return set_err(Q3_INVALID_ARG, "buffer too small (%zu < %zu)", bytes, need);
    HIPC(q3_hipMemcpy(out, src, need, hipMemcpyDeviceToHost));
    return Q3_OK;
}
```

Baseline: 2886.

## Decode overlapped segments through a batched async codec stream instead of per-row jobs

Adds an asynchronous enqueue/wait path to the codec stream, using pinned descriptor slots and async copies, so several pushes can be in flight without host syncs. q3_session_run now groups per-row decode jobs into multi-row pushes (default 8 rows) and enqueues them on a persistent codec stream, replacing the one-job-at-a-time segment decode. The intent is fewer kernel launches and host synchronisations, plus better GPU utilisation from batching rows during the overlapped and tail decode. In exchange it adds more state, a pinned-memory cache and an in-flight limit, and stream state that is kept between runs.

```diff
diff --git a/include/q3tts.h b/include/q3tts.h
--- a/include/q3tts.h
+++ b/include/q3tts.h
@@ -385,6 +385,10 @@
 q3_status q3_codec_stream_pos(q3_codec_stream* cs, int row, int* n_frames);
 q3_status q3_codec_stream_push(q3_codec_stream* cs, int n_rows, const int* rows, const uint32_t* const* frames_host,
                                const int* n_frames, float* const* pcm_host, const size_t* cap);
+q3_status q3_codec_stream_enqueue(q3_codec_stream* cs, int n_rows, const int* rows, const uint32_t* const* frames_host,
+                                  const int* n_frames, float* const* pcm_host, const size_t* cap, int resident);
+q3_status q3_codec_stream_wait(q3_codec_stream* cs);
+q3_status q3_codec_stream_set_inflight(q3_codec_stream* cs, int max_pushes);
 q3_status q3_codec_stream_create_blocked(q3_model* m, int rows, int max_frames, int block_frames, int max_blocks, q3_codec_stream** out);
 q3_status q3_codec_stream_info(q3_codec_stream* cs, int* block_frames, size_t* block_bytes, int* blocks_total, int* blocks_in_use,
                                int* blocks_peak);
diff --git a/qwen3_tts_rs_amd/_lib.py b/qwen3_tts_rs_amd/_lib.py
--- a/qwen3_tts_rs_amd/_lib.py
+++ b/qwen3_tts_rs_amd/_lib.py
@@ -219,6 +219,9 @@
     "q3_codec_stream_reset": (c_int, [c_void_p, c_int]),
     "q3_codec_stream_pos": (c_int, [c_void_p, c_int, P(c_int)]),
     "q3_codec_stream_push": (c_int, [c_void_p, c_int, P(c_int), P(c_void_p), P(c_int), P(c_void_p), P(ctypes.c_size_t)]),
+    "q3_codec_stream_enqueue": (c_int, [c_void_p, c_int, P(c_int), P(c_void_p), P(c_int), P(c_void_p), P(ctypes.c_size_t), c_int]),
+    "q3_codec_stream_wait": (c_int, [c_void_p]),
+    "q3_codec_stream_set_inflight": (c_int, [c_void_p, c_int]),
     "q3_pcm_stage_create": (c_int, [c_int, c_int, ctypes.c_size_t, P(c_void_p)]),
     "q3_pcm_stage_free": (None, [c_void_p]),
     "q3_pcm_stage_set": (c_int, [c_void_p, c_int, ctypes.c_uint32, c_int]),
diff --git a/qwen3_tts_rs_amd/api.py b/qwen3_tts_rs_amd/api.py
--- a/qwen3_tts_rs_amd/api.py
+++ b/qwen3_tts_rs_amd/api.py
@@ -1168,6 +1168,28 @@
         cp = (ctypes.c_size_t * n)(*[int(x) for x in (cap if cap is not None else [o.size for o in outs])])
         check(lib.q3_codec_stream_push(self._h, n, r, fp, nf, op, cp))
         return {int(rows[i]): outs[i] for i in range(n)}
+
+    def enqueue(self, rows: Sequence[int], codes: Sequence[np.ndarray], resident: int = 0) -> dict:
+        n = len(rows); spf = self.model.config.samples_per_frame
+        cs = [np.ascontiguousarray(c, dtype=np.uint32).reshape(-1, 16) for c in codes]
+        outs = [np.zeros(c.shape[0] * spf, dtype=np.float32) for c in cs]
+        r = (ctypes.c_int * n)(*[int(x) for x in rows])
+        fp = (ctypes.c_void_p * n)(*[c.ctypes.data_as(ctypes.c_void_p) for c in cs])
+        nf = (ctypes.c_int * n)(*[c.shape[0] for c in cs])
+        op = (ctypes.c_void_p * n)(*[o.ctypes.data_as(ctypes.c_void_p) for o in outs])
+        cp = (ctypes.c_size_t * n)(*[o.size for o in outs])
+        check(lib.q3_codec_stream_enqueue(self._h, n, r, fp, nf, op, cp, int(resident)))
+        self._held = getattr(self, "_held", []) + [outs, cs]
+        return {int(rows[i]): outs[i] for i in range(n)}
+
+    def wait(self):
+        try:
+            check(lib.q3_codec_stream_wait(self._h))
+        finally:
+            self._held = []
+
+    def set_inflight(self, max_pushes: int):
+        check(lib.q3_codec_stream_set_inflight(self._h, int(max_pushes)))
 
     def reset(self, row: int):
         check(lib.q3_codec_stream_reset(self._h, int(row)))
diff --git a/qwen3_tts_rs_amd/csrc/q3_codec_stream.hip b/qwen3_tts_rs_amd/csrc/q3_codec_stream.hip
--- a/qwen3_tts_rs_amd/csrc/q3_codec_stream.hip
+++ b/qwen3_tts_rs_amd/csrc/q3_codec_stream.hip
@@ -1,4 +1,5 @@
 #include "q3_engine.h"
+#include <map>
 
 struct CsRow { int pos = 0; float* kv = nullptr; float* lat = nullptr; float* hist = nullptr; std::vector<float*> blocks; };
 struct q3_codec_stream {
@@ -11,6 +12,10 @@
     float *cs = nullptr, *sn = nullptr;
     char* desc = nullptr; size_t desc_cap = 0;
     float* stage = nullptr; float* stage_host = nullptr; size_t stage_cap = 0;
+    struct Slot { char* host = nullptr; size_t host_cap = 0; char* dev = nullptr; size_t dev_cap = 0; };
+    std::vector<Slot> slots; int inflight = 0, max_inflight = 64;
+    std::vector<int> pending;
+    long long front_cols = 0;
 };
 
 static size_t kv_floats(const q3_codec_stream* cs) {
@@ -69,6 +74,33 @@
     return Q3_OK;
 }
 
+namespace {
+struct PinCache {
+    std::mutex mu; std::multimap<size_t, char*> free_blocks;
+    static size_t size_class(size_t bytes) { size_t p2 = 64 << 10; while (p2 < bytes) p2 <<= 1; return p2; }
+    char* get(size_t* bytes) {
+        *bytes = size_class(*bytes);
+        {
+            std::lock_guard<std::mutex> g(mu);
+            auto it = free_blocks.find(*bytes);
+            if (it != free_blocks.end()) { char* p = it->second; free_blocks.erase(it); return p; }
+        }
+        char* p = nullptr;
+        if (hipHostMalloc((void**)&p, *bytes, hipHostMallocDefault) != hipSuccess) { (void)hipGetLastError(); return nullptr; }
+        return p;
+    }
+    void put(char* p, size_t bytes) {
+        if (!p) return;
+        {
+            std::lock_guard<std::mutex> g(mu);
+            if (free_blocks.size() < 64) { free_blocks.emplace(bytes, p); return; }
+        }
+        (void)hipHostFree(p);
+    }
+};
+PinCache& pin_cache() { static PinCache* c = new PinCache(); return *c; }
+}
+
 extern "C" void q3_codec_stream_free(q3_codec_stream* cs) {
     if (!cs) return;
     q3_model* m = cs->m;
@@ -79,6 +111,7 @@
     cs->ws.release();
     dev_free(cs->cs); dev_free(cs->sn); dev_free(cs->desc); dev_free(cs->stage);
     if (cs->stage_host) (void)hipHostFree(cs->stage_host);
+    for (auto& sl : cs->slots) { pin_cache().put(sl.host, sl.host_cap); dev_free(sl.dev); }
     if (cs->owns_stream && cs->st) (void)hipStreamDestroy(cs->st);
     delete cs;
     if (m->refs.fetch_sub(1) == 1) model_destroy(m);
@@ -121,9 +154,64 @@
 };
 }
 
-q3_status codec_stream_push(q3_codec_stream* cs, const std::vector<CsPush>& all) {
+q3_status codec_stream_wait(q3_codec_stream* cs) {
+    if (!cs->inflight && cs->pending.empty()) return Q3_OK;
+    HIPC(hipSetDevice(cs->m->device));
+    const hipError_t e = hipStreamSynchronize(cs->st);
+    cs->inflight = 0;
+    std::vector<int> rows; rows.swap(cs->pending);
+    if (e != hipSuccess) {
+        for (int r : rows) codec_stream_reset(cs, r);
+        return set_err(Q3_HIP_ERROR, "codec stream: enqueued pushes failed on the device: %s (their rows are back at frame 0)", hipGetErrorString(e));
+    }
+    return Q3_OK;
+}
+
+long long codec_stream_front_cols(q3_codec_stream* cs, bool clear) {
+    const long long n = cs->front_cols;
+    if (clear) cs->front_cols = 0;
+    return n;
+}
+
+q3_status codec_stream_reserve(q3_codec_stream* cs, int T, int Tf, int out_frames, bool state_rows) {
     q3_model* m = cs->m;
     const q3_config& c = m->cfg;
+    HIPC(hipSetDevice(m->device));
+    const int spf = samples_per_frame(c);
+    if (T > cs->ws.cap_frames || std::max(T, Tf) > cs->ws.cap_front) { Q3C(codec_stream_wait(cs)); Q3C(codec_reserve(m, cs->ws, T, Tf)); }
+    if ((size_t)out_frames * spf > cs->stage_cap) {
+        Q3C(codec_stream_wait(cs));
+        HIPC(hipStreamSynchronize(cs->st));
+        dev_free(cs->stage); cs->stage = nullptr;
+        if (cs->stage_host) { (void)hipHostFree(cs->stage_host); cs->stage_host = nullptr; }
+        cs->stage_cap = 0;
+        if (dev_malloc((void**)&cs->stage, (size_t)out_frames * spf * 4) != hipSuccess) { (void)hipGetLastError(); cs->stage = nullptr; return set_err(Q3_OOM, "codec stream: staging for %d frames", out_frames); }
+        cs->stage_cap = (size_t)out_frames * spf;
+    }
+    if (state_rows && !cs->bf)
+        for (int i = 0; i < cs->R; ++i) {
+            CsRow& r = cs->rows[i];
+            if (r.kv) continue;
+            if (dev_malloc((void**)&r.kv, kv_floats(cs) * 4) != hipSuccess || dev_malloc((void**)&r.lat, (size_t)c.dec_latent * cs->cap * 4) != hipSuccess ||
+                dev_malloc((void**)&r.hist, (size_t)c.dec_q_dim * 2 * 4) != hipSuccess) {
+                (void)hipGetLastError();
+                dev_free(r.kv); dev_free(r.lat); dev_free(r.hist); r.kv = r.lat = r.hist = nullptr;
+                return set_err(Q3_OOM, "codec stream: state of row %d (%zu MB)", i, (kv_floats(cs) + (size_t)c.dec_latent * cs->cap) * 4 >> 20);
+            }
+        }
+    return Q3_OK;
+}
+
+static q3_status push_run(q3_codec_stream* cs, const std::vector<CsPush>& all, const bool async, const int resident) {
+    q3_model* m = cs->m;
+    const q3_config& c = m->cfg;
+    if (!async) Q3C(codec_stream_wait(cs));
+    else {
+        if (cs->inflight >= cs->max_inflight)
+            return set_err(Q3_INVALID_ARG, "codec stream: descriptor block refused: %d pushes are in flight and the stream allows %d (q3_codec_stream_wait releases them)",
+                           cs->inflight, cs->max_inflight);
+        for (const CsPush& p : all) if (p.ps) return set_err(Q3_INVALID_ARG, "codec stream: an enqueued push takes no output stage");
+    }
     std::vector<CsPush> P;
     for (const CsPush& p : all) if (p.n > 0) P.push_back(p);
     q3_pcm_stage* ps = nullptr;
@@ -215,18 +303,21 @@
         int max_n = 0; for (const CsPush& p : P) max_n = std::max(max_n, p.n);
         const int T = std::max(1, std::max(Lc, solo_max));
         const long long Tw = (long long)cs->R * (max_n + CODEC_CTX_FRAMES), Fw = (long long)cs->R * (max_n + 2);
-        Q3C(codec_reserve(m, cs->ws, (int)std::max<long long>(T, std::min<long long>(Tw, CS_WIDE)),
-                          (int)std::max<long long>(Np, std::min<long long>(Fw, CS_WIDE))));
+        if (async) { if (T > cs->ws.cap_frames || std::max(T, Np) > cs->ws.cap_front) { Q3C(codec_stream_wait(cs)); Q3C(codec_reserve(m, cs->ws, T, Np)); } }
+        else Q3C(codec_reserve(m, cs->ws, (int)std::max<long long>(T, std::min<long long>(Tw, CS_WIDE)),
+                               (int)std::max<long long>(Np, std::min<long long>(Fw, CS_WIDE))));
     }
     CodecWS& ws = cs->ws;
-    if ((size_t)W * spf > cs->stage_cap) {
+    if ((size_t)W * spf > cs->stage_cap || (!async && W > 0 && !cs->stage_host)) {
+        if (async) Q3C(codec_stream_wait(cs));
         HIPC(hipStreamSynchronize(st));
         dev_free(cs->stage); cs->stage = nullptr;
         if (cs->stage_host) { (void)hipHostFree(cs->stage_host); cs->stage_host = nullptr; }
+        const size_t want = std::max((size_t)W * spf, cs->stage_cap);
         cs->stage_cap = 0;
-        HIPC(dev_malloc((void**)&cs->stage, (size_t)W * spf * 4));
-        HIPC(hipHostMalloc((void**)&cs->stage_host, (size_t)W * spf * 4, hipHostMallocDefault));
-        cs->stage_cap = (size_t)W * spf;
+        HIPC(dev_malloc((void**)&cs->stage, want * 4));
+        if (!async) HIPC(hipHostMalloc((void**)&cs->stage_host, want * 4, hipHostMallocDefault));
+        cs->stage_cap = want;
     }
     std::vector<PsSeg> psegs; std::vector<const CsPush*> pseg_of; std::vector<void*> pouts; PsPlan plan;
     if (ps) {
@@ -287,7 +378,26 @@
     const size_t o_pos = db.add(pos), o_arows = db.add(arows), o_xin = db.add(xin), o_hist = db.add(hist), o_compact = db.add(compact),
                  o_kvsc = db.add(kvsc), o_latsc = db.add(latsc), o_latg = db.add(latg), o_segs = db.add(segs), o_fsrc = db.add(fsrc),
                  o_brows = db.add(brows), o_tabs = db.add(tabs), o_solog = db.add(solog), o_ps = db.add(plan.desc);
-    if (db.host.size() > cs->desc_cap) {
+    const size_t o_fhost = async ? db.add(fhost) : 0;
+    char* desc = nullptr;
+    if (async) {
+        if ((int)cs->slots.size() <= cs->inflight) cs->slots.resize((size_t)cs->inflight + 1);
+        q3_codec_stream::Slot& sl = cs->slots[(size_t)cs->inflight];
+        if (sl.host_cap < db.host.size()) {
+            pin_cache().put(sl.host, sl.host_cap); sl.host = nullptr; sl.host_cap = 0;
+            size_t bytes = db.host.size();
+            sl.host = pin_cache().get(&bytes);
+            if (!sl.host) return set_err(Q3_OOM, "codec stream: pinned descriptor block of %zu bytes", db.host.size());
+            sl.host_cap = bytes;
+        }
+        if (sl.dev_cap < db.host.size()) {
+            dev_free(sl.dev); sl.dev = nullptr; sl.dev_cap = 0;
+            if (dev_malloc((void**)&sl.dev, sl.host_cap) != hipSuccess) { (void)hipGetLastError(); sl.dev = nullptr; return set_err(Q3_OOM, "codec stream: descriptor block of %zu bytes", sl.host_cap); }
+            sl.dev_cap = sl.host_cap;
+        }
+        memcpy(sl.host, db.host.data(), db.host.size());
+        desc = sl.dev;
+    } else if (db.host.size() > cs->desc_cap) {
         HIPC(hipStreamSynchronize(st));
         dev_free(cs->desc); cs->desc = nullptr; cs->desc_cap = 0;
         HIPC(dev_malloc((void**)&cs->desc, db.host.size() * 2));
@@ -301,12 +411,19 @@
             for (const CsPush& p : P) codec_stream_reset(cs, p.row);
         }
     } failed{cs, P};
-    HIPC(q3_hipMemcpy(cs->desc, db.host.data(), db.host.size(), hipMemcpyHostToDevice));
-    auto D = [&](size_t off) { return (const void*)(cs->desc + off); };
+    if (async) {
+        HIPC(hipMemcpyAsync(desc, cs->slots[(size_t)cs->inflight].host, db.host.size(), hipMemcpyHostToDevice, st));
+        cs->inflight++;
+    } else {
+        desc = cs->desc;
+        HIPC(q3_hipMemcpy(desc, db.host.data(), db.host.size(), hipMemcpyHostToDevice));
+    }
+    auto D = [&](size_t off) { return (const void*)(desc + off); };
     if (on_dev) HIPC(launch_gather_frames((const uint32_t* const*)D(o_fsrc), ws.frames, N, st));
+    else if (async) HIPC(hipMemcpyAsync(ws.frames, D(o_fhost), fhost.size() * 4, hipMemcpyDeviceToDevice, st));
     else HIPC(q3_hipMemcpy(ws.frames, fhost.data(), fhost.size() * 4, hipMemcpyHostToDevice));
 
-    const CodecScope scope(m);
+    const CodecScope scope(m, async ? resident : 0);
     Q3C(codec_front_quant(m, ws, N, st));
     HIPC(launch_copy_cols((const ColCopy*)D(o_xin), Np, Q, 0, 0, st));
     HIPC(launch_copy_cols((const ColCopy*)D(o_hist), 2 * nP, Q, 0, 0, st));
@@ -337,6 +454,16 @@
         Q3C(codec_stack_dev(m, ws, F, e, st, nullptr, scope));
         HIPC(launch_copy_segs(ws.pcm, cs->stage, dsegs + conc.size() + k, 1, (size_t)(P[i].n - P[i].skip) * spf, st));
     }
+    if (async) {
+        for (int i = 0; i < nP; ++i)
+            if (P[i].pcm_host && P[i].n > P[i].skip)
+                HIPC(hipMemcpyAsync(P[i].pcm_host, cs->stage + (size_t)out0[i] * spf, (size_t)(P[i].n - P[i].skip) * spf * 4, hipMemcpyDeviceToHost, st));
+        for (int i = 0; i < nP; ++i) { cs->rows[P[i].row].pos += P[i].n; cs->pending.push_back(P[i].row); }
+        cs->front_cols += N;
+        failed.armed = false; untake.armed = false;
+        cs->blocks_peak = std::max(cs->blocks_peak, cs->blocks_in_use);
+        return Q3_OK;
+    }
     bool raw = false;
     for (int i = 0; i < nP; ++i) raw = raw || !P[i].ps;
     if (W > 0 && raw) HIPC(hipMemcpyAsync(cs->stage_host, cs->stage, (size_t)W * spf * 4, hipMemcpyDeviceToHost, st));
@@ -348,8 +475,58 @@
         if (P[i].pcm_host && !P[i].ps) memcpy(P[i].pcm_host, cs->stage_host + (size_t)out0[i] * spf, (size_t)(P[i].n - P[i].skip) * spf * 4);
         cs->rows[P[i].row].pos += P[i].n;
     }
+    cs->front_cols += N;
     failed.armed = false; untake.armed = false;
     cs->blocks_peak = std::max(cs->blocks_peak, cs->blocks_in_use);
+    return Q3_OK;
+}
+
+q3_status codec_stream_push(q3_codec_stream* cs, const std::vector<CsPush>& pushes) { return push_run(cs, pushes, false, 0); }
+q3_status codec_stream_enqueue(q3_codec_stream* cs, const std::vector<CsPush>& pushes, int resident) { return push_run(cs, pushes, true, resident); }
+
+static q3_status check_push_rows(q3_codec_stream* cs, const char* who, int n_rows, const int* rows, const uint32_t* const* frames_host, const int* n_frames,
+                                 float* const* pcm_host, const size_t* cap, std::vector<CsPush>& P) {
+    const int spf = samples_per_frame(cs->m->cfg);
+    std::vector<char> seen(cs->R, 0);
+    for (int i = 0; i < n_rows; ++i) {
+        const int r = rows[i], n = n_frames[i];
+        if (r < 0 || r >= cs->R) return set_err(Q3_INVALID_ARG, "%s: row %d out of range (%d rows)", who, r, cs->R);
+        if (seen[r]) return set_err(Q3_INVALID_ARG, "%s: row %d listed twice", who, r);
+        seen[r] = 1;
+        if (n < 0) return set_err(Q3_INVALID_ARG, "%s: negative frame count for row %d", who, r);
+        if (n == 0) continue;
+        if (cs->rows[r].pos + n > cs->cap)
+            return set_err(Q3_INVALID_ARG, "%s: row %d would reach %d frames, the stream holds %d", who, r, cs->rows[r].pos + n, cs->cap);
+        if (!frames_host[i] || !pcm_host[i]) return set_err(Q3_INVALID_ARG, "%s: null frames or pcm pointer for row %d", who, r);
+        if (cap[i] < (size_t)n * spf) return set_err(Q3_INVALID_ARG, "%s: pcm buffer of row %d too small (%zu < %zu samples)", who, r, cap[i], (size_t)n * spf);
+        for (int f = 0; f < n; ++f)
+            for (int g = 1; g < 16; ++g)
+                if (frames_host[i][(size_t)f * 16 + g] >= (uint32_t)cs->m->cfg.dec_cb_size)
+                    return set_err(Q3_INVALID_ARG, "code %u out of range for codebook %d (row %d, frame %d)", frames_host[i][(size_t)f * 16 + g], g, r, f);
+        P.push_back({r, n, 0, frames_host[i], nullptr, pcm_host[i]});
+    }
+    return Q3_OK;
+}
+
+extern "C" q3_status q3_codec_stream_enqueue(q3_codec_stream* cs, int n_rows, const int* rows, const uint32_t* const* frames_host,
+                                             const int* n_frames, float* const* pcm_host, const size_t* cap, int resident) {
+    if (!cs) return set_err(Q3_INVALID_ARG, "q3_codec_stream_enqueue: null stream");
+    if (n_rows < 0 || (n_rows > 0 && (!rows || !frames_host || !n_frames || !pcm_host || !cap)))
+        return set_err(Q3_INVALID_ARG, "q3_codec_stream_enqueue: null argument");
+    if (resident < 0 || resident > 2) return set_err(Q3_INVALID_ARG, "q3_codec_stream_enqueue: resident must be 0, 1 or 2");
+    std::vector<CsPush> P;
+    Q3C(check_push_rows(cs, "q3_codec_stream_enqueue", n_rows, rows, frames_host, n_frames, pcm_host, cap, P));
+    return codec_stream_enqueue(cs, P, resident);
+}
+
+extern "C" q3_status q3_codec_stream_wait(q3_codec_stream* cs) {
+    if (!cs) return set_err(Q3_INVALID_ARG, "q3_codec_stream_wait: null stream");
+    return codec_stream_wait(cs);
+}
+
+extern "C" q3_status q3_codec_stream_set_inflight(q3_codec_stream* cs, int max_pushes) {
+    if (!cs || max_pushes < 1) return set_err(Q3_INVALID_ARG, "q3_codec_stream_set_inflight: the stream holds at least one descriptor block");
+    cs->max_inflight = max_pushes;
     return Q3_OK;
 }
 
diff --git a/qwen3_tts_rs_amd/csrc/q3_engine.h b/qwen3_tts_rs_amd/csrc/q3_engine.h
--- a/qwen3_tts_rs_amd/csrc/q3_engine.h
+++ b/qwen3_tts_rs_amd/csrc/q3_engine.h
@@ -361,6 +361,7 @@
     hipStream_t dec_stream = nullptr; hipEvent_t dec_ev = nullptr;
     std::vector<CodecWS> par_ws; std::vector<hipStream_t> par_streams;
     CodecWS seg_ws;
+    q3_codec_stream* run_cs = nullptr;
     std::vector<uint32_t> codes_host; bool codes_host_valid = false;
     int stream_pos = 0;
     int stream_mode = 0;
@@ -407,6 +408,10 @@
 Q3_HIDDEN q3_status codec_stream_create(q3_model* m, int rows, int max_frames, hipStream_t st, q3_codec_stream** out, int block_frames = 0,
                                         int max_blocks = 0);
 Q3_HIDDEN q3_status codec_stream_push(q3_codec_stream* cs, const std::vector<CsPush>& pushes);
+Q3_HIDDEN q3_status codec_stream_enqueue(q3_codec_stream* cs, const std::vector<CsPush>& pushes, int resident);
+Q3_HIDDEN q3_status codec_stream_wait(q3_codec_stream* cs);
+Q3_HIDDEN q3_status codec_stream_reserve(q3_codec_stream* cs, int T, int Tf, int out_frames, bool state_rows);
+Q3_HIDDEN long long codec_stream_front_cols(q3_codec_stream* cs, bool clear);
 Q3_HIDDEN int codec_stream_pos(const q3_codec_stream* cs, int row);
 Q3_HIDDEN void codec_stream_blocks(const q3_codec_stream* cs, int row, int upto, int* held, int* need);
 Q3_HIDDEN void codec_stream_reset(q3_codec_stream* cs, int row);
diff --git a/qwen3_tts_rs_amd/csrc/q3_session.hip b/qwen3_tts_rs_amd/csrc/q3_session.hip
--- a/qwen3_tts_rs_amd/csrc/q3_session.hip
+++ b/qwen3_tts_rs_amd/csrc/q3_session.hip
@@ -637,6 +637,7 @@
     for (auto st : par_streams) (void)hipStreamDestroy(st);
     if (ostage) q3_pcm_stage_free(ostage);
     if (cstream) q3_codec_stream_free(cstream);
+    if (run_cs) q3_codec_stream_free(run_cs);
     cws.release(); seg_ws.release();
     for (auto& w : par_ws) w.release();
     if (dec_ev) (void)hipEventDestroy(dec_ev);
@@ -1906,6 +1907,8 @@
 }
 
 static constexpr bool DECODE_OVERLAP_DEFAULT = true;
+static constexpr bool DECODE_STREAM_DEFAULT = true;
+static constexpr int DECODE_ROWS_DEFAULT = 8;
 extern "C" q3_status q3_session_run(q3_session* s, int use_graph, float** pcm_host, const size_t* cap, size_t* n_samples, q3_timing* timing) {
     if (!s) return set_err(Q3_INVALID_ARG, "null session");
     if (any_open_text(s)) return set_err(Q3_UNSUPPORTED, "q3_session_run: a row's text is still open (q3_session_append_text with last != 0 closes it; or drive the session with q3_session_generate)");
@@ -1981,7 +1984,27 @@
             HIPC(hipStreamCreateWithPriority(&s->dec_stream, hipStreamNonBlocking, least));
         }
     }
-    Q3C(codec_reserve(s->m, s->seg_ws, seg_env + CODEC_CTX_FRAMES, s->max_frames));
+    const bool stream_env = [] { const char* e = getenv("Q3_DECODE_STREAM"); return e ? atoi(e) != 0 : DECODE_STREAM_DEFAULT; }();
+    const int rows_env = [s] { const char* e = getenv("Q3_DECODE_ROWS"); const int v = e ? atoi(e) : DECODE_ROWS_DEFAULT; return v < 1 ? 1 : (v > s->B ? s->B : v); }();
+    const int push_T = rows_env * (seg_env + CODEC_CTX_FRAMES);
+    bool use_stream = stream_env;
+    if (use_stream) {
+        q3_status cst = Q3_OK;
+        if (!s->run_cs) cst = codec_stream_create(s->m, s->B, s->max_frames, s->dec_stream, &s->run_cs);
+        if (cst == Q3_OK) cst = codec_stream_wait(s->run_cs);
+        if (cst == Q3_OK) {
+            for (int b = 0; b < s->B; ++b) codec_stream_reset(s->run_cs, b);
+            (void)codec_stream_front_cols(s->run_cs, true);
+            cst = codec_stream_reserve(s->run_cs, push_T, rows_env * (seg_env + 2), rows_env * seg_env, true);
+        }
+        if (cst != Q3_OK) { (void)hipGetLastError(); use_stream = false; }
+    }
+    if (!use_stream) Q3C(codec_reserve(s->m, s->seg_ws, seg_env + CODEC_CTX_FRAMES, s->max_frames));
+    struct Drain {
+        q3_codec_stream* cs = nullptr;
+        ~Drain() { if (cs) (void)codec_stream_wait(cs); }
+    } drain;
+    if (use_stream) drain.cs = s->run_cs;
     struct Split {
         q3::AqlProgram* p = nullptr;
         void release() { if (p) { std::string why; q3::aql_restrict_cus(p, 0, &why); p = nullptr; } }
@@ -1991,6 +2014,7 @@
     std::vector<int> dec_pos((size_t)s->B, 0);
     std::thread worker; q3_status wst = Q3_OK; std::string werr;
     double join_wait_ms = 0.0; int n_dispatch = 0;
+    long long front_cols = 0;
     auto join = [&]() -> q3_status {
         if (worker.joinable()) worker.join();
         if (wst != Q3_OK) return set_err(wst, "%s", werr.c_str());
@@ -2018,6 +2042,21 @@
         }
         return jobs;
     };
+    auto group = [s, spf, pcm_host, cap, rows_env, push_T](const std::vector<Job>& jobs, std::vector<std::vector<CsPush>>& out) -> q3_status {
+        int T = 0;
+        std::vector<char> in_push((size_t)s->B, 0);
+        for (const Job& j : jobs) {
+            if (pcm_host && pcm_host[j.b] && (!cap || cap[j.b] < (size_t)j.e * spf)) return set_err(Q3_INVALID_ARG, "pcm buffer too small");
+            const int t = j.e - j.a + CODEC_CTX_FRAMES;
+            if (out.empty() || (int)out.back().size() >= rows_env || T + t > push_T || in_push[(size_t)j.b]) {
+                out.emplace_back(); T = 0; std::fill(in_push.begin(), in_push.end(), 0);
+            }
+            out.back().push_back(CsPush{j.b, j.e - j.a, 0, nullptr, s->codes + ((size_t)j.b * s->max_frames + j.a) * 16,
+                                        pcm_host && pcm_host[j.b] ? pcm_host[j.b] + (size_t)j.a * spf : nullptr});
+            T += t; in_push[(size_t)j.b] = 1;
+        }
+        return Q3_OK;
+    };
     auto dispatch = [&]() -> q3_status {
         std::vector<Job> jobs = collect(false);
         if (jobs.empty()) return Q3_OK;
@@ -2026,6 +2065,19 @@
             Q3C(join());
             join_wait_ms += ms(j0, clk::now()); ++n_dispatch;
         }
+        if (use_stream) {
+            std::vector<std::vector<CsPush>> pushes;
+            Q3C(group(jobs, pushes));
+            worker = std::thread([s, pushes, resident_env, &wst, &werr]() {
+                if (hipSetDevice(s->m->device) != hipSuccess) { wst = Q3_HIP_ERROR; werr = "hipSetDevice failed in the decode thread"; return; }
+                for (const auto& P : pushes) {
+                    const q3_status st = codec_stream_enqueue(s->run_cs, P, resident_env);
+                    if (st != Q3_OK) { wst = st; werr = q3_last_error(); return; }
+                }
+            });
+            return Q3_OK;
+        }
+        for (const Job& j : jobs) front_cols += j.e;
         worker = std::thread([s, jobs, seg_enqueue, resident_env, &wst, &werr]() {
             if (hipSetDevice(s->m->device) != hipSuccess) { wst = Q3_HIP_ERROR; werr = "hipSetDevice failed in the decode thread"; return; }
             for (const Job& j : jobs) {
@@ -2055,6 +2107,13 @@
         auto st_of = [&](int k) { return k == 0 ? s->stream : s->par_streams[(size_t)k - 1]; };
         auto tail = [&]() -> q3_status {
             std::vector<Job> jobs = collect(true);
+            if (use_stream) {
+                std::vector<std::vector<CsPush>> pushes;
+                Q3C(group(jobs, pushes));
+                for (const auto& P : pushes) Q3C(codec_stream_enqueue(s->run_cs, P, 0));
+                return Q3_OK;
+            }
+            for (const Job& j : jobs) front_cols += j.e;
             while ((int)s->par_ws.size() < conc - 1) {
                 hipStream_t pst = nullptr;
                 HIPC(hipStreamCreateWithFlags(&pst, hipStreamNonBlocking));
@@ -2065,6 +2124,7 @@
             return Q3_OK;
         };
         st = tail();
+        if (use_stream) { const q3_status ws = codec_stream_wait(s->run_cs); if (st == Q3_OK) st = ws; front_cols = codec_stream_front_cols(s->run_cs, true); }
         hipError_t he = hipStreamSynchronize(s->dec_stream);
         for (int k = 0; k < conc && k <= (int)s->par_streams.size(); ++k) { const hipError_t e2 = hipStreamSynchronize(st_of(k)); if (he == hipSuccess) he = e2; }
         if (st != Q3_OK) return st;
@@ -2079,8 +2139,9 @@
     if (timing) { timing->prefill_ms = ms(t0, t1); timing->generation_ms = ms(t1, t2); timing->decode_ms = ms(t2, t3); timing->generation_frames = total; }
     const bool log_env = getenv("Q3_DECODE_LOG") != nullptr;
     if (log_env)
-        fprintf(stderr, "q3_session_run overlap: resident %d seg %d tail %d, %d dispatches, frame loop waited %.3f ms for the enqueue thread, frames %.1f ms, exposed decode %.1f ms\n",
-                resident_env, seg_env, tail_env, n_dispatch, join_wait_ms, ms(t1, t2), ms(t2, t3));
+        fprintf(stderr, "q3_session_run overlap: resident %d seg %d tail %d, %d dispatches, frame loop waited %.3f ms for the enqueue thread, frames %.1f ms, exposed decode %.1f ms, "
+                        "path %s, rows per push %d, front columns %lld\n",
+                resident_env, seg_env, tail_env, n_dispatch, join_wait_ms, ms(t1, t2), ms(t2, t3), use_stream ? "stream" : "rows", use_stream ? rows_env : 1, front_cols);
     return Q3_OK;
 }
 
```

Result: no change. 2904 (median of 6 runs) (+0.6%).
